# mit-han-lab/pvcnn

Hardware: AMD Instinct MI355X
Metric: point-clouds/sec fwd+bwd, PVCNN S3DIS N=4096 R=32 (higher is better)
Workload: dtype f32 (fp32 tensors, fp32 accumulate; Conv3d fwd / bwd-data / bwd-weight and the large SharedMLP fwd / bwd-data / bwd-weight products as power-of-two scaled fp16 hi+lo splits, 3 partial products on fp16 MFMA, max rel err vs fp64 1e-6 <= the fp32-MFMA kernels'; PVCNN_CONV_MATH=fp32 PVCNN_PW_MATH=fp32 s; 1 GPU; PVCNN (1xC) S3DIS fwd+bwd+Adam, B=16/GPU N=4096 R=32/16 fp32; global_batch=16, points=4096, parallelism=dp1, gradient_bytes=10289972, step_mode=graph, rccl_ranks=0, gradient_buckets=2

## Files before the change

include/pvcnn_hip.h:

```cpp
#ifndef PVCNN_HIP_H_
#define PVCNN_HIP_H_

#include <stddef.h>
#include <stdint.h>

#ifdef __cplusplus
extern "C" {
#endif

#if defined(__GNUC__)
#define PVCNN_API __attribute__((visibility("default")))
#else
#define PVCNN_API
#endif

#define PVCNN_ABI_VERSION 17
#define PVCNN_OK 0
#define PVCNN_ERR_INVALID_ARGUMENT (-1)

PVCNN_API int pvcnn_version(void);
PVCNN_API const char *pvcnn_last_error_string(void);

PVCNN_API int pvcnn_voxel_coords(const float *coords, int B, int N, int R, int normalize, float eps, float *norm_coords,
                       int32_t *vox_coords, void *stream);

PVCNN_API int pvcnn_voxel_coords_tail(const float *coords, long coords_batch_stride, const float *mean, const float *radius,
                            int B, int N, int R, float eps, float *norm_coords, int32_t *vox_coords, void *stream);

PVCNN_API size_t pvcnn_avg_voxelize_fwd_workspace_bytes(int B, int C, int N, int R);
PVCNN_API int pvcnn_avg_voxelize_fwd(const float *feat, const int32_t *coords, int B, int C, int N, int R,
                           float *out, int32_t *ind, int32_t *cnt, void *workspace,
                           size_t workspace_bytes, void *stream);
PVCNN_API int pvcnn_avg_voxelize_bwd(const float *grad_y, const int32_t *ind, const int32_t *cnt, int B,
                           int C, int N, int S, float *grad_x, void *stream);

PVCNN_API int pvcnn_trilinear_devox_fwd(const float *coords, const float *feat, int B, int C, int N, int R,
                              int is_training, int32_t *inds, float *wgts, float *outs,
                              void *stream);
PVCNN_API size_t pvcnn_trilinear_devox_bwd_workspace_bytes(int B, int C, int N, int R);
PVCNN_API int pvcnn_trilinear_devox_bwd(const float *grad_y, const int32_t *inds, const float *wgts, int B,
                              int C, int N, int R, float *grad_x, void *workspace,
                              size_t workspace_bytes, void *stream);

PVCNN_API size_t pvcnn_avg_voxelize_plan_bytes(int B, int N, int R);
PVCNN_API size_t pvcnn_avg_voxelize_plan_scratch_bytes(int B, int N, int R);
PVCNN_API int pvcnn_avg_voxelize_plan(const int32_t *coords, int B, int N, int R, int32_t *ind, int32_t *cnt, void *plan,
                            size_t plan_bytes, void *scratch, size_t scratch_bytes, void *stream);
PVCNN_API size_t pvcnn_pvconv_plans_scratch_bytes(int B, int N, int R);
PVCNN_API int pvcnn_pvconv_plans(const int32_t *vox_coords, const float *norm_coords, int B, int N, int R, int32_t *ind, int32_t *cnt,
                                 void *vox_plan, size_t vox_plan_bytes, void *devox_bwd_plan, size_t devox_bwd_plan_bytes,
                                 void *scratch, size_t scratch_bytes, void *stream);
PVCNN_API int pvcnn_avg_voxelize_apply(const float *feat, const void *plan, size_t plan_bytes, int B, int C, int N, int R,
                             float *out, void *stream);
PVCNN_API size_t pvcnn_trilinear_devox_bwd_plan_bytes(int B, int N, int R);
PVCNN_API size_t pvcnn_trilinear_devox_bwd_plan_scratch_bytes(int B, int N, int R);
PVCNN_API int pvcnn_trilinear_devox_bwd_plan(const int32_t *inds, const float *wgts, int B, int N, int R, void *plan,
                                   size_t plan_bytes, void *scratch, size_t scratch_bytes, void *stream);
PVCNN_API int pvcnn_trilinear_devox_bwd_apply(const float *grad_y, long grad_y_batch_stride, const void *plan, size_t plan_bytes,
                                    int B, int C, int N, int R, float *grad_x, void *stream);

PVCNN_API int pvcnn_ball_query(const float *centers, const float *points, int B, int N, int M, float radius,
                     int U, int32_t *out, void *stream);

PVCNN_API int pvcnn_grouping_fwd(const float *features, const int32_t *indices, int B, int C, int N, int M,
                       int U, float *out, void *stream);
PVCNN_API size_t pvcnn_grouping_bwd_workspace_bytes(int B, int C, int N, int M, int U);
PVCNN_API int pvcnn_grouping_bwd(const float *grad_y, const int32_t *indices, int B, int C, int N, int M,
                       int U, float *grad_x, void *workspace, size_t workspace_bytes, void *stream);
PVCNN_API int pvcnn_gather_fwd(const float *features, const int32_t *indices, int B, int C, int N, int M,
                     float *out, void *stream);
PVCNN_API size_t pvcnn_gather_bwd_workspace_bytes(int B, int C, int N, int M);
PVCNN_API int pvcnn_gather_bwd(const float *grad_y, const int32_t *indices, int B, int C, int N, int M,
                     float *grad_x, void *workspace, size_t workspace_bytes, void *stream);

#define PVCNN_FPS_MAX_RESIDENT_POINTS 16384
PVCNN_API int pvcnn_fps(const float *coords, int B, int N, int M, float *distances, int32_t *indices,
              void *stream);

PVCNN_API int pvcnn_mask_select(const uint8_t *mask, int B, int N, int M, const int32_t *choices, const int64_t *seed,
                      int32_t *selected, int32_t *count, void *stream);

PVCNN_API size_t pvcnn_batch_lds_bytes(int N, int max_n);
PVCNN_API int pvcnn_batch_s3dis(const float *rows, const void *labels, int label_bytes, const int64_t *offsets, long long W, int max_n,
                      const int64_t *order, long long order_len, const int64_t *cursor, int B, int N, int C_out,
                      const int32_t *choices, const int64_t *seed, float *features, int64_t *targets, void *stream);
PVCNN_API int pvcnn_batch_shapenet(const float *rows, const void *labels, int label_bytes, const int64_t *offsets, long long W,
                         const int32_t *shape_ids, const int64_t *order, long long order_len, const int64_t *cursor, int B, int N,
                         int with_normal, int num_shapes, int jitter_on, const int32_t *choices, const double *jitter,
                         const int64_t *seed, float *features, int64_t *targets, void *stream);
PVCNN_API int pvcnn_batch_frustum(const float *rows, const void *labels, int label_bytes, const int64_t *offsets, long long W,
                        const double *item_f64, const float *item_f32, const int64_t *item_i64, int K, int random_flip,
                        int random_shift, const int64_t *order, long long order_len, const int64_t *cursor, int B, int N,
                        const int32_t *choices, const double *flip, const double *shift, const int64_t *seed, float *features,
                        float *one_hot_vectors, int64_t *mask_logits, float *center, int64_t *heading_bin_id,
                        float *heading_residual, int64_t *size_template_id, float *size_residual, int64_t *class_id, void *stream);
PVCNN_API int pvcnn_batch_frustum_rgb(const float *rows, const int64_t *offsets, long long W, const double *item_f64,
                            const float *item_f32, int K, const int64_t *order, long long order_len, const int64_t *cursor, int B,
                            int N, const int32_t *choices, const int64_t *seed, float *features, float *one_hot_vectors,
                            float *rotation_angle, double *rgb_score, void *stream);

PVCNN_API int pvcnn_three_nn_interp_fwd(const float *points_coords, const float *centers_coords,
                              const float *centers_features, int B, int C, int M, int N,
                              int32_t *indices, float *weights, float *out, void *stream);
PVCNN_API size_t pvcnn_three_nn_interp_bwd_workspace_bytes(int B, int C, int N, int M);
PVCNN_API int pvcnn_three_nn_interp_bwd(const float *grad_y, const int32_t *indices, const float *weights,
                              int B, int C, int N, int M, float *grad_x, void *workspace,
                              size_t workspace_bytes, void *stream);

PVCNN_API int pvcnn_conv3d_weight_transform(const float *w, int Co, int Ci, int for_bwd_data, float *wt,
                                            void *stream);
PVCNN_API int pvcnn_conv3d_fwd(const float *x, const float *wt, const float *bias, int B, int Ci, int Co,
                               int R, float *y, void *stream);
PVCNN_API size_t pvcnn_conv3d_bwd_weight_workspace_bytes(int B, int Ci, int Co, int R);
PVCNN_API int pvcnn_conv3d_bwd_weight(const float *x, const float *grad_y, int B, int Ci, int Co, int R,
                                      float *grad_w, float *grad_bias, void *workspace, size_t workspace_bytes,
                                      void *stream);

PVCNN_API size_t pvcnn_conv3d_weight_split_bytes(int Co, int Ci, int for_bwd_data, int nsplit);
PVCNN_API int pvcnn_conv3d_weight_split(const float *w, int Co, int Ci, int for_bwd_data, int nsplit, void *wts, void *stream);
PVCNN_API int pvcnn_conv3d_weight_split_pair(const float *w, int Co, int Ci, void *wts_fwd, void *wts_bwd, void *stream);
PVCNN_API size_t pvcnn_conv3d_fwd_split_stats_parts(int B, int Co, int R, int nsplit);
PVCNN_API int pvcnn_conv3d_fwd_split_route(int B, int Ci, int Co, int R, int nsplit);
PVCNN_API int pvcnn_absmax_bits(const float *x, size_t n, void *out, void *stream);
PVCNN_API size_t pvcnn_absmax_tiles_count(int B, long L, int seg);
#define PVCNN_TABLE_ONLY ((void *)1)
PVCNN_API int pvcnn_absmax_tiles(const float *x, int B, int C, long L, int seg, void *out, void *ticket, void *stream);
PVCNN_API int pvcnn_conv3d_fwd_split(const float *x, const void *wts, const float *bias, int B, int Ci, int Co, int R, int nsplit,
                           const void *x_absmax, int amax_seg , float *y, float *stats_part, void *stream);
PVCNN_API int pvcnn_conv3d_fwd_split_act(const float *x, const void *wts, const float *bias, int B, int Ci, int Co, int R, int nsplit,
                           const void *x_absmax, int amax_seg , float *y, float *stats_part, float slope, void *y_amax,
                           int y_amax_seg , void *stream);
PVCNN_API int pvcnn_conv3d_fwd_act(const float *x, const float *wt, const float *bias, int B, int Ci, int Co, int R, float *y,
                           float slope, void *y_amax, int y_amax_seg , void *stream);

PVCNN_API size_t pvcnn_conv3d_bwd_weight_f16_workspace_bytes(int B, int Ci, int Co, int R);
PVCNN_API int pvcnn_conv3d_bwd_weight_f16(const float *x, const float *grad_y, const void *x_absmax, int x_amax_seg, const void *gy_absmax,
                                int gy_amax_seg, int B, int Ci, int Co, int R, float *grad_w, float *grad_bias, void *workspace,
                                size_t workspace_bytes, void *stream);

PVCNN_API int pvcnn_pwconv_transpose(const float *w, int M, int K, float *wt, void *stream);
PVCNN_API int pvcnn_pwconv_fwd(const float *x, const float *wt, int wt_rows, const float *bias, int B, int K, int M,
                     int N, float *y, void *stream);
PVCNN_API size_t pvcnn_pwconv_bwd_weight_workspace_bytes(int B, int K, int M, int N);
PVCNN_API int pvcnn_pwconv_bwd_weight(const float *x, const float *grad_y, int B, int K, int M, int N,
                            float *grad_w, float *grad_bias, void *workspace, size_t workspace_bytes,
                            void *stream);

PVCNN_API size_t pvcnn_pwconv_weight_split_bytes(int Co, int Ci, int for_bwd_data, int nsplit);
PVCNN_API int pvcnn_pwconv_weight_split(const float *w, int Co, int Ci, int for_bwd_data, int nsplit, void *wts, void *stream);
PVCNN_API int pvcnn_pwconv_weight_split_pair(const float *w, int Co, int Ci, void *wts_fwd, void *wts_bwd, void *stream);
PVCNN_API size_t pvcnn_pwconv_fwd_split_stats_parts(int B, int N);
PVCNN_API int pvcnn_pwconv_fwd_split_route(int B, int K, int M, int N, int nsplit);
PVCNN_API int pvcnn_pwconv_fwd_split(const float *x, const void *wts, const float *bias, int B, int K, int M, int N, int nsplit,
                           const void *x_absmax, int amax_seg , float *y, float *stats_part, void *stream);
PVCNN_API int pvcnn_pwconv_fwd_split_act(const float *x, const void *wts, const float *bias, int B, int K, int M, int N, int nsplit,
                           const void *x_absmax, int amax_seg , float *y, float *stats_part, float slope, void *y_amax,
                           int y_amax_seg , void *stream);
PVCNN_API int pvcnn_pwconv_fwd_act(const float *x, const float *wt, int wt_rows, const float *bias, int B, int K, int M, int N,
                           float *y, float slope, void *y_amax, int y_amax_seg , void *stream);
PVCNN_API size_t pvcnn_pwconv_bwd_weight_f16_workspace_bytes(int B, int K, int M, int N);
PVCNN_API int pvcnn_pwconv_bwd_weight_f16(const float *x, const float *grad_y, const void *x_absmax, int x_amax_seg, const void *gy_absmax,
                                int gy_amax_seg, int B, int K, int M, int N, float *grad_w, float *grad_bias, void *workspace,
                                size_t workspace_bytes, void *stream);

PVCNN_API int pvcnn_dropout_keep_mask(const void *drop_seed, float drop_p, long numel, unsigned char *keep, void *stream);
PVCNN_API size_t pvcnn_bnact_workspace_bytes(int B, int C, int S);
PVCNN_API int pvcnn_bnact_fwd(const float *x, const float *gamma, const float *beta, float *running_mean,
                              float *running_var, int B, int C, int S, float eps, float momentum, float slope,
                              int training, float *mean, float *rstd, float *y, void *y_amax, int amax_seg, int amax_zeroed,
                              void *workspace, size_t workspace_bytes, const void *drop_seed, float drop_p, void *stream);
PVCNN_API size_t pvcnn_conv3d_fwd_stats_parts(int B, int Co, int R);
PVCNN_API int pvcnn_conv3d_fwd_stats(const float *x, const float *wt, const float *bias, int B, int Ci, int Co, int R,
                           float *y, float *stats_part, void *stream);
PVCNN_API size_t pvcnn_pwconv_fwd_stats_parts(int B, int N);
PVCNN_API int pvcnn_pwconv_fwd_stats(const float *x, const float *wt, int wt_rows, const float *bias, int B, int K, int M,
                           int N, float *y, float *stats_part, void *stream);
PVCNN_API int pvcnn_bn_finalize(const float *part, int C, long nparts, double count, float eps, float momentum, const float *shift,
                      float *running_mean, float *running_var, float *mean, float *rstd,
                      void *zero_words , long zero_count ,
                      void *num_batches_tracked , void *stream);
PVCNN_API int pvcnn_bn_stats(const float *x, float *running_mean, float *running_var, int B, int C, int S,
                   float eps, float momentum, float *mean, float *rstd, void *workspace,
                   size_t workspace_bytes, void *stream);
PVCNN_API int pvcnn_trilinear_devox_bnact_fwd(const float *coords, const float *feat, const float *gamma,
                                    const float *beta, const float *mean, const float *rstd, float slope,
                                    int B, int C, int N, int R, int is_training, int32_t *inds, float *wgts,
                                    const float *addend, const float *se_scale, float *outs, void *stream);
PVCNN_API int pvcnn_trilinear_devox_bnact_addbn_fwd(const float *coords, const float *feat, const float *gamma,
                                    const float *beta, const float *mean, const float *rstd, float slope,
                                    int B, int C, int N, int R, int is_training, int32_t *inds, float *wgts,
                                    const float *addend, const float *add_gamma, const float *add_beta,
                                    const float *add_mean, const float *add_rstd, float add_slope, float *outs, void *stream);
PVCNN_API int pvcnn_bnact_bwd(const float *x, const float *grad_y, const float *gamma, const float *beta,
                              const float *mean, const float *rstd, int B, int C, int S, float slope, int training,
                              float *grad_x, float *grad_gamma, float *grad_beta, void *workspace,
                              size_t workspace_bytes, void *stream);
PVCNN_API int pvcnn_bnact_bwd_strided(const float *x, const float *grad_y, long grad_y_batch_stride, const float *gamma,
                            const float *beta, const float *mean, const float *rstd, int B, int C, int S,
                            float slope, int training, float *grad_x, float *grad_gamma, float *grad_beta,
                            void *gx_amax, int amax_seg, void *workspace, size_t workspace_bytes, const void *drop_seed,
                            float drop_p, void *tickets, void *stream);
PVCNN_API int pvcnn_bnact_slices(int S);
PVCNN_API long pvcnn_conv3d_weight_split_pair_entry(const float *w, int Co, int Ci, void *wts_fwd, void *wts_bwd, long long *entry);
PVCNN_API int pvcnn_conv3d_weight_split_pair_batch(const void *table, int n, long total_rows, void *stream);
PVCNN_API long pvcnn_pwconv_weight_split_pair_entry(const float *w, int Co, int Ci, void *wts_fwd, void *wts_bwd, long long *entry);
PVCNN_API int pvcnn_pwconv_weight_split_pair_batch(const void *table, int n, long total_rows, void *stream);
PVCNN_API long pvcnn_conv3d_weight_split_pair_entry_bf16(const float *w, int Co, int Ci, void *wts_fwd, void *wts_bwd, long long *entry);
PVCNN_API int pvcnn_conv3d_weight_split_pair_batch_bf16(const void *table, int n, long total_rows, void *stream);
PVCNN_API long pvcnn_pwconv_weight_split_pair_entry_bf16(const float *w, int Co, int Ci, void *wts_fwd, void *wts_bwd, long long *entry);
PVCNN_API int pvcnn_pwconv_weight_split_pair_batch_bf16(const void *table, int n, long total_rows, void *stream);

PVCNN_API int pvcnn_neighbor_max_supported(int K);
PVCNN_API int pvcnn_neighbor_max_fwd(const float *x, long rows, int K, float *out, unsigned char *winners, void *stream);
PVCNN_API int pvcnn_neighbor_max_bwd(const float *grad_out, const unsigned char *winners, long rows, int K, float *grad_x, void *stream);

PVCNN_API int pvcnn_row_argmax(const float *x, long rows, int K, long long *winners, float *values, void *stream);

PVCNN_API int pvcnn_bnact_apply_rowmax(const float *x, const float *gamma, const float *beta, const float *mean, const float *rstd, int B,
                                       int C, int S, float slope, float *y, long y_batch_stride, void *y_amax, int amax_seg,
                                       void *row_keys, void *stream);
PVCNN_API int pvcnn_row_keys_decode(const void *row_keys, const float *y, long rows, int S, long long *winners, float *values,
                                    int C, long y_batch_stride, void *stream);

PVCNN_API size_t pvcnn_frustum_box_loss_grad_floats(int B, int NH, int NS);
PVCNN_API int pvcnn_frustum_box_loss(const float *center, const float *center_reg, const float *heading_scores, const float *size_scores,
                                     const float *heading_residuals_normalized, const float *size_residuals_normalized,
                                     const float *heading_residuals, const float *size_residuals, const long long *heading_bin_id,
                                     const long long *size_template_id, const float *heading_residual_t, const float *size_residual_t,
                                     const float *center_t, const float *size_templates, const float *heading_bin_centers, int B, int NH,
                                     int NS, float heading_bin_width, float w_heading_residual, float w_size_residual, float w_corners,
                                     float *loss, float *grads, void *stream);

PVCNN_API int pvcnn_se_excite_fwd(const float *part, int slices, const float *gamma, const float *beta, const float *w1, const float *w2,
                        int B, int C, int H, float inv_s, float *a_sum, float *ax_sum, float *squeezed, float *hidden, float *excite,
                        void *stream);
PVCNN_API int pvcnn_se_excite_bwd(const float *part, int slices, const float *a_sum, const float *ax_sum, const float *gamma,
                        const float *beta, const float *squeezed, const float *hidden, const float *excite, const float *w1,
                        const float *w2, int B, int C, int H, float inv_s, float *g_w1, float *g_w2, float *g_mean, float *sum_beta,
                        float *sum_gamma, float *workspace, void *stream);
PVCNN_API int pvcnn_bnact_partial_sums(const float *x, const float *grad_y, long grad_y_batch_stride, const float *gamma, const float *beta,
                             const float *mean, const float *rstd, int B, int C, int S, float slope, float *part, void *stream);
PVCNN_API int pvcnn_bnact_bwd_apply(const float *x, const float *grad_y, long grad_y_batch_stride, const float *gamma, const float *beta,
                          const float *mean, const float *rstd, const float *sum_gamma, const float *sum_beta, const float *bc_mul,
                          const float *bc_add, int B, int C, int S, float slope, int training, float *grad_x, void *gx_amax,
                          int amax_seg, void *stream);
PVCNN_API int pvcnn_trilinear_devox_bwd_strided(const float *grad_y, long grad_y_batch_stride, const int32_t *inds,
                                      const float *wgts, int B, int C, int N, int R, float *grad_x,
                                      void *workspace, size_t workspace_bytes, void *stream);

PVCNN_API int pvcnn_concat_points(const float *const *srcs, const long *bstrides, const int *channels, const int *pstrides,
                        const void *const *src_amax ,
                        int nsrc, int B, int N, float *out, void *out_amax,
                        void *ticket , void *stream);

PVCNN_API int pvcnn_dense_bn_relu_supported(int rows, int Cin, int Cout);
PVCNN_API int pvcnn_dense_bn_relu_fwd(const float *x, const float *weight, const float *bias, const float *gamma, const float *beta,
                                      float *running_mean, float *running_var, void *num_batches_tracked, int rows, int Cin, int Cout,
                                      float eps, float momentum, float *z, float *y, float *mean, float *rstd, void *stream);
PVCNN_API int pvcnn_dense_bn_relu_bwd(const float *x, const float *grad_y, const float *z, const float *mean, const float *rstd,
                                      const float *gamma, const float *beta, int rows, int Cin, int Cout, float *grad_z,
                                      float *grad_weight, float *grad_bias, float *grad_gamma, float *grad_beta, void *stream);

PVCNN_API int pvcnn_adam_step(float *p, const float *g, float *m, float *v, size_t n, float *step, const float *hyper, int inc_step,
                    void *stream);
PVCNN_API int pvcnn_grad_sqsum(const float *g, size_t n, float *partials, int nparts, void *stream);
PVCNN_API int pvcnn_grad_norm_finalize(const float *partials, int nparts, float *status, void *stream);
PVCNN_API int pvcnn_adam_step_grouped(float *p, const float *g, float *m, float *v, float *vmax, size_t n, float *step,
                                      const float *hyper, int ngroups, const int *runs, int nruns, const float *status,
                                      int decoupled, int inc_step, void *stream);

PVCNN_API int pvcnn_eval_tile(const float *src, long long batch_stride, long long point_stride, long long chan_stride, long long src_points,
                              const long long *shuffled, int B, int V, int num_points, int C, float *out, void *stream);
PVCNN_API int pvcnn_vote_confidence(const float *logits, int B, int C, int N, int c0, int c1, const int *ranges, float *conf, int *pred,
                                    void *stream);
PVCNN_API size_t pvcnn_vote_merge_workspace_bytes(long long P);
PVCNN_API int pvcnn_vote_merge(const float *conf, const int *pred, const long long *shuffled, const long long *mapping, long long map_stride,
                               int B, int V, long long P, float *scene_conf, long long *scene_pred, void *workspace, size_t workspace_bytes,
                               void *stream);
PVCNN_API int pvcnn_seg_counts(const long long *gt, const long long *pred, long long P, int C, int wrap_negative, long long *counts,
                               void *stream);
PVCNN_API int pvcnn_seg_meter_update(const float *logits, const long long *targets, int B, int C, int N, const int *part_ranges,
                                     int num_part_classes, int max_parts, long long *counts, int *rows, const long long *row_cursor,
                                     long long row_capacity, void *stream);

// ... 102 lines not shown
```

pvcnn_amd/_lib.py:

```python
import ctypes
import functools
import os

import torch

_CSRC = os.path.join(os.path.dirname(os.path.abspath(__file__)), 'csrc')
LIB_PATH = os.path.join(_CSRC, 'libpvcnn_hip.so')
ABI_VERSION = 17

_vp, _i, _f, _sz, _l = ctypes.c_void_p, ctypes.c_int, ctypes.c_float, ctypes.c_size_t, ctypes.c_long
_ll = ctypes.c_longlong
_d = ctypes.c_double

SIGNATURES = {
    'pvcnn_version': (_i, []),
    'pvcnn_last_error_string': (ctypes.c_char_p, []),
    'pvcnn_voxel_coords': (_i, [_vp, _i, _i, _i, _i, _f, _vp, _vp, _vp]),
    'pvcnn_voxel_coords_tail': (_i, [_vp, ctypes.c_long, _vp, _vp, _i, _i, _i, _f, _vp, _vp, _vp]),
    'pvcnn_avg_voxelize_fwd_workspace_bytes': (_sz, [_i, _i, _i, _i]),
    'pvcnn_avg_voxelize_fwd': (_i, [_vp, _vp, _i, _i, _i, _i, _vp, _vp, _vp, _vp, _sz, _vp]),
    'pvcnn_avg_voxelize_bwd': (_i, [_vp, _vp, _vp, _i, _i, _i, _i, _vp, _vp]),
    'pvcnn_trilinear_devox_fwd': (_i, [_vp, _vp, _i, _i, _i, _i, _i, _vp, _vp, _vp, _vp]),
    'pvcnn_trilinear_devox_bwd_workspace_bytes': (_sz, [_i, _i, _i, _i]),
    'pvcnn_trilinear_devox_bwd': (_i, [_vp, _vp, _vp, _i, _i, _i, _i, _vp, _vp, _sz, _vp]),
    'pvcnn_avg_voxelize_plan_bytes': (_sz, [_i, _i, _i]),
    'pvcnn_avg_voxelize_plan_scratch_bytes': (_sz, [_i, _i, _i]),
    'pvcnn_avg_voxelize_plan': (_i, [_vp, _i, _i, _i, _vp, _vp, _vp, _sz, _vp, _sz, _vp]),
    'pvcnn_avg_voxelize_apply': (_i, [_vp, _vp, _sz, _i, _i, _i, _i, _vp, _vp]),
    'pvcnn_pvconv_plans_scratch_bytes': (_sz, [_i, _i, _i]),
    'pvcnn_pvconv_plans': (_i, [_vp, _vp, _i, _i, _i, _vp, _vp, _vp, _sz, _vp, _sz, _vp, _sz, _vp]),
    'pvcnn_trilinear_devox_bwd_plan_bytes': (_sz, [_i, _i, _i]),
    'pvcnn_trilinear_devox_bwd_plan_scratch_bytes': (_sz, [_i, _i, _i]),
    'pvcnn_trilinear_devox_bwd_plan': (_i, [_vp, _vp, _i, _i, _i, _vp, _sz, _vp, _sz, _vp]),
    'pvcnn_trilinear_devox_bwd_apply': (_i, [_vp, ctypes.c_long, _vp, _sz, _i, _i, _i, _i, _vp, _vp]),
    'pvcnn_ball_query': (_i, [_vp, _vp, _i, _i, _i, _f, _i, _vp, _vp]),
    'pvcnn_grouping_fwd': (_i, [_vp, _vp, _i, _i, _i, _i, _i, _vp, _vp]),
    'pvcnn_grouping_bwd_workspace_bytes': (_sz, [_i, _i, _i, _i, _i]),
    'pvcnn_grouping_bwd': (_i, [_vp, _vp, _i, _i, _i, _i, _i, _vp, _vp, _sz, _vp]),
    'pvcnn_gather_fwd': (_i, [_vp, _vp, _i, _i, _i, _i, _vp, _vp]),
    'pvcnn_gather_bwd_workspace_bytes': (_sz, [_i, _i, _i, _i]),
    'pvcnn_gather_bwd': (_i, [_vp, _vp, _i, _i, _i, _i, _vp, _vp, _sz, _vp]),
    'pvcnn_fps': (_i, [_vp, _i, _i, _i, _vp, _vp, _vp]),
    'pvcnn_mask_select': (_i, [_vp, _i, _i, _i, _vp, _vp, _vp, _vp, _vp]),
    'pvcnn_three_nn_interp_fwd': (_i, [_vp, _vp, _vp, _i, _i, _i, _i, _vp, _vp, _vp, _vp]),
    'pvcnn_three_nn_interp_bwd_workspace_bytes': (_sz, [_i, _i, _i, _i]),
    'pvcnn_three_nn_interp_bwd': (_i, [_vp, _vp, _vp, _i, _i, _i, _i, _vp, _vp, _sz, _vp]),
    'pvcnn_conv3d_weight_transform': (_i, [_vp, _i, _i, _i, _vp, _vp]),
    'pvcnn_conv3d_fwd': (_i, [_vp, _vp, _vp, _i, _i, _i, _i, _vp, _vp]),
    'pvcnn_conv3d_bwd_weight_workspace_bytes': (_sz, [_i, _i, _i, _i]),
    'pvcnn_conv3d_bwd_weight': (_i, [_vp, _vp, _i, _i, _i, _i, _vp, _vp, _vp, _sz, _vp]),
    'pvcnn_conv3d_weight_split_bytes': (_sz, [_i, _i, _i, _i]),
    'pvcnn_conv3d_weight_split': (_i, [_vp, _i, _i, _i, _i, _vp, _vp]),
    'pvcnn_conv3d_weight_split_pair': (_i, [_vp, _i, _i, _vp, _vp, _vp]),
    'pvcnn_conv3d_fwd_split_stats_parts': (_sz, [_i, _i, _i, _i]),
    'pvcnn_conv3d_fwd_split_route': (_i, [_i, _i, _i, _i, _i]),
    'pvcnn_absmax_bits': (_i, [_vp, _sz, _vp, _vp]),
    'pvcnn_absmax_tiles_count': (_sz, [_i, ctypes.c_long, _i]),
    'pvcnn_absmax_tiles': (_i, [_vp, _i, _i, ctypes.c_long, _i, _vp, _vp, _vp]),
    'pvcnn_conv3d_bwd_weight_f16_workspace_bytes': (_sz, [_i, _i, _i, _i]),
    'pvcnn_conv3d_bwd_weight_f16': (_i, [_vp, _vp, _vp, _i, _vp, _i, _i, _i, _i, _i, _vp, _vp, _vp, _sz, _vp]),
    'pvcnn_conv3d_fwd_split': (_i, [_vp, _vp, _vp, _i, _i, _i, _i, _i, _vp, _i, _vp, _vp, _vp]),
    'pvcnn_pwconv_transpose': (_i, [_vp, _i, _i, _vp, _vp]),
    'pvcnn_pwconv_fwd': (_i, [_vp, _vp, _i, _vp, _i, _i, _i, _i, _vp, _vp]),
    'pvcnn_pwconv_weight_split_bytes': (_sz, [_i, _i, _i, _i]),
    'pvcnn_pwconv_weight_split': (_i, [_vp, _i, _i, _i, _i, _vp, _vp]),
    'pvcnn_pwconv_weight_split_pair': (_i, [_vp, _i, _i, _vp, _vp, _vp]),
    'pvcnn_pwconv_fwd_split_stats_parts': (_sz, [_i, _i]),
    'pvcnn_pwconv_fwd_split_route': (_i, [_i, _i, _i, _i, _i]),
    'pvcnn_pwconv_fwd_split': (_i, [_vp, _vp, _vp, _i, _i, _i, _i, _i, _vp, _i, _vp, _vp, _vp]),
    'pvcnn_pwconv_bwd_weight_f16_workspace_bytes': (_sz, [_i, _i, _i, _i]),
    'pvcnn_pwconv_bwd_weight_f16': (_i, [_vp, _vp, _vp, _i, _vp, _i, _i, _i, _i, _i, _vp, _vp, _vp, _sz, _vp]),
    'pvcnn_pwconv_bwd_weight_workspace_bytes': (_sz, [_i, _i, _i, _i]),
    'pvcnn_pwconv_bwd_weight': (_i, [_vp, _vp, _i, _i, _i, _i, _vp, _vp, _vp, _sz, _vp]),
    'pvcnn_bnact_workspace_bytes': (_sz, [_i, _i, _i]),
    'pvcnn_bnact_fwd': (_i, [_vp, _vp, _vp, _vp, _vp, _i, _i, _i, _f, _f, _f, _i, _vp, _vp, _vp, _vp, _i, _i, _vp, _sz, _vp, _f, _vp]),
    'pvcnn_dropout_keep_mask': (_i, [_vp, _f, _l, _vp, _vp]),
    'pvcnn_conv3d_fwd_stats_parts': (_sz, [_i, _i, _i]),
    'pvcnn_conv3d_fwd_stats': (_i, [_vp, _vp, _vp, _i, _i, _i, _i, _vp, _vp, _vp]),
    'pvcnn_pwconv_fwd_stats_parts': (_sz, [_i, _i]),
    'pvcnn_pwconv_fwd_stats': (_i, [_vp, _vp, _i, _vp, _i, _i, _i, _i, _vp, _vp, _vp]),
    'pvcnn_bn_finalize': (_i, [_vp, _i, ctypes.c_long, ctypes.c_double, _f, _f, _vp, _vp, _vp, _vp, _vp, _vp, ctypes.c_long, _vp, _vp]),
    'pvcnn_bn_stats': (_i, [_vp, _vp, _vp, _i, _i, _i, _f, _f, _vp, _vp, _vp, _sz, _vp]),
    'pvcnn_trilinear_devox_bnact_fwd': (_i, [_vp, _vp, _vp, _vp, _vp, _vp, _f, _i, _i, _i, _i, _i, _vp, _vp, _vp, _vp, _vp, _vp]),
    'pvcnn_trilinear_devox_bnact_addbn_fwd': (_i, [_vp, _vp, _vp, _vp, _vp, _vp, _f, _i, _i, _i, _i, _i, _vp, _vp, _vp, _vp, _vp, _vp, _vp, _f, _vp, _vp]),
    'pvcnn_bnact_slices': (_i, [_i]),
    'pvcnn_conv3d_weight_split_pair_entry': (_l, [_vp, _i, _i, _vp, _vp, _vp]),
    'pvcnn_conv3d_weight_split_pair_batch': (_i, [_vp, _i, _l, _vp]),
    'pvcnn_pwconv_weight_split_pair_entry': (_l, [_vp, _i, _i, _vp, _vp, _vp]),
    'pvcnn_pwconv_weight_split_pair_batch': (_i, [_vp, _i, _l, _vp]),
    'pvcnn_conv3d_weight_split_pair_entry_bf16': (_l, [_vp, _i, _i, _vp, _vp, _vp]),
    'pvcnn_conv3d_weight_split_pair_batch_bf16': (_i, [_vp, _i, _l, _vp]),
    'pvcnn_pwconv_weight_split_pair_entry_bf16': (_l, [_vp, _i, _i, _vp, _vp, _vp]),
    'pvcnn_pwconv_weight_split_pair_batch_bf16': (_i, [_vp, _i, _l, _vp]),
    'pvcnn_neighbor_max_supported': (_i, [_i]),
    'pvcnn_neighbor_max_fwd': (_i, [_vp, _l, _i, _vp, _vp, _vp]),
    'pvcnn_neighbor_max_bwd': (_i, [_vp, _vp, _l, _i, _vp, _vp]),
    'pvcnn_row_argmax': (_i, [_vp, _l, _i, _vp, _vp, _vp]),
    'pvcnn_bnact_apply_rowmax': (_i, [_vp, _vp, _vp, _vp, _vp, _i, _i, _i, _f, _vp, _l, _vp, _i, _vp, _vp]),
    'pvcnn_row_keys_decode': (_i, [_vp, _vp, _l, _i, _vp, _vp, _i, _l, _vp]),
    'pvcnn_frustum_box_loss_grad_floats': (_sz, [_i, _i, _i]),
    'pvcnn_frustum_box_loss': (_i, [_vp] * 15 + [_i, _i, _i, _f, _f, _f, _f, _vp, _vp, _vp]),
    'pvcnn_se_excite_fwd': (_i, [_vp, _i, _vp, _vp, _vp, _vp, _i, _i, _i, _f, _vp, _vp, _vp, _vp, _vp, _vp]),
    'pvcnn_se_excite_bwd': (_i, [_vp, _i] + [_vp] * 9 + [_i, _i, _i, _f] + [_vp] * 7),
    'pvcnn_bnact_partial_sums': (_i, [_vp, _vp, ctypes.c_long, _vp, _vp, _vp, _vp, _i, _i, _i, _f, _vp, _vp]),
    'pvcnn_bnact_bwd_apply': (_i, [_vp, _vp, ctypes.c_long, _vp, _vp, _vp, _vp, _vp, _vp, _vp, _vp, _i, _i, _i, _f, _i, _vp, _vp, _i, _vp]),
    'pvcnn_bnact_bwd': (_i, [_vp, _vp, _vp, _vp, _vp, _vp, _i, _i, _i, _f, _i, _vp, _vp, _vp, _vp, _sz, _vp]),
    'pvcnn_bnact_bwd_strided': (_i, [_vp, _vp, ctypes.c_long, _vp, _vp, _vp, _vp, _i, _i, _i, _f, _i, _vp, _vp, _vp, _vp, _i, _vp, _sz, _vp, _f, _vp, _vp]),
    'pvcnn_concat_points': (_i, [_vp, _vp, _vp, _vp, _vp, _i, _i, _i, _vp, _vp, _vp, _vp]),
    'pvcnn_dense_bn_relu_supported': (_i, [_i, _i, _i]),
    'pvcnn_dense_bn_relu_fwd': (_i, [_vp] * 8 + [_i, _i, _i, _f, _f, _vp, _vp, _vp, _vp, _vp]),
    'pvcnn_dense_bn_relu_bwd': (_i, [_vp] * 7 + [_i, _i, _i] + [_vp] * 6),
    'pvcnn_adam_step': (_i, [_vp, _vp, _vp, _vp, _sz, _vp, _vp, _i, _vp]),
    'pvcnn_grad_sqsum': (_i, [_vp, _sz, _vp, _i, _vp]),
    'pvcnn_grad_norm_finalize': (_i, [_vp, _i, _vp, _vp]),
    'pvcnn_adam_step_grouped': (_i, [_vp, _vp, _vp, _vp, _vp, _sz, _vp, _vp, _i, _vp, _i, _vp, _i, _i, _vp]),
    'pvcnn_trilinear_devox_bwd_strided': (_i, [_vp, ctypes.c_long, _vp, _vp, _i, _i, _i, _i, _vp, _vp, _sz, _vp]),
    'pvcnn_eval_tile': (_i, [_vp, _ll, _ll, _ll, _ll, _vp, _i, _i, _i, _i, _vp, _vp]),
    'pvcnn_vote_confidence': (_i, [_vp, _i, _i, _i, _i, _i, _vp, _vp, _vp, _vp]),
    'pvcnn_vote_merge_workspace_bytes': (_sz, [_ll]),
    'pvcnn_vote_merge': (_i, [_vp, _vp, _vp, _vp, _ll, _i, _i, _ll, _vp, _vp, _vp, _sz, _vp]),
    'pvcnn_seg_counts': (_i, [_vp, _vp, _ll, _i, _i, _vp, _vp]),
    'pvcnn_seg_meter_update': (_i, [_vp, _vp, _i, _i, _i, _vp, _i, _i, _vp, _vp, _vp, _ll, _vp]),
    'pvcnn_frustum_meter_update': (_i, [_vp] * 11 + [_i, _i, _i, _vp, _vp, _vp, _vp, _i, _vp, _vp, _i, _i, _vp, _vp, _vp]),
    'pvcnn_box_iou_3d': (_i, [_vp, _vp, _i, _vp, _vp, _vp]),
    'pvcnn_rotate_iou': (_i, [_vp, _ll, _vp, _ll, _i, _vp, _vp]),
    'pvcnn_box3d_overlap': (_i, [_vp, _vp, _ll, _vp, _vp, _ll, _i, _i, ctypes.c_double, _vp, _vp]),
    'pvcnn_batch_lds_bytes': (_sz, [_i, _i]),
    'pvcnn_batch_s3dis': (_i, [_vp, _vp, _i, _vp, _ll, _i, _vp, _ll, _vp, _i, _i, _i, _vp, _vp, _vp, _vp, _vp]),
    'pvcnn_batch_shapenet': (_i, [_vp, _vp, _i, _vp, _ll, _vp, _vp, _ll, _vp, _i, _i, _i, _i, _i, _vp, _vp, _vp, _vp, _vp, _vp]),
    'pvcnn_batch_frustum': (_i, [_vp, _vp, _i, _vp, _ll, _vp, _vp, _vp, _i, _i, _i, _vp, _ll, _vp, _i, _i] + [_vp] * 14),
    'pvcnn_batch_frustum_rgb': (_i, [_vp, _vp, _ll, _vp, _vp, _i, _vp, _ll, _vp, _i, _i] + [_vp] * 7),
    'pvcnn_frustum_predictions': (_i, [_vp] * 5 + [_i, _i, _i] + [_vp] * 5 + [_ll, _ll, _vp]),
    'pvcnn_room_workspace_bytes': (_sz, [_ll, _ll]),
    'pvcnn_room_extent': (_i, [_vp, _ll, _vp, _vp, _sz, _vp]),
    'pvcnn_room_blocks': (_i, [_vp, _ll, _vp, _d, _d, _i, _i, _i, _vp, _vp, _vp, _vp, _vp, _vp, _sz, _vp]),
    'pvcnn_room_cells': (_i, [_vp, _ll, _vp, _d, _ll, _vp, _vp, _vp, _vp, _vp, _vp]),
    'pvcnn_room_plan': (_i, [_vp, _vp, _ll, _ll, _i] + [_vp] * 6 + [_vp, _sz, _vp]),
    'pvcnn_room_fill': (_i, [_vp] * 7 + [_ll, _ll, _ll] + [_vp] * 5),
    'pvcnn_room_pack': (_i, [_vp, _vp, _ll, _vp, _d, _vp, _vp, _ll, _ll, _i, _ll] + [_vp] * 9),
    'pvcnn_image_box_overlap': (_i, [_vp, _ll, _vp, _ll, _i, _vp, _vp]),
    'pvcnn_kitti_ap_bbox_overlaps': (_i, [_vp] * 5 + [_ll, _ll, _vp, _vp]),
    'pvcnn_kitti_ap_box_overlaps': (_i, [_vp] * 7 + [_ll, _ll, _i, _i, _d, _vp, _vp]),
    'pvcnn_kitti_ap_clean': (_i, [_vp, _vp, _vp, _vp, _ll, _vp, _vp, _ll, _vp, _vp, _ll, _vp, _i, _vp, _i] + [_vp] * 5),
    'pvcnn_kitti_ap_match': (_i, [_vp] * 5 + [_ll, _ll, _ll, _i, _i] + [_vp] * 9 + [_i, _i, _i] + [_vp, _vp]),
    'pvcnn_kitti_ap_thresholds': (_i, [_vp, _ll, _vp, _i, _i, _vp, _vp, _vp]),
    'pvcnn_kitti_ap_workspace_bytes': (_sz, [_ll, _i]),
    'pvcnn_conv3d_fwd_split_act': (_i, [_vp, _vp, _vp, _i, _i, _i, _i, _i, _vp, _i, _vp, _vp, _f, _vp, _i, _vp]),
    'pvcnn_conv3d_fwd_act': (_i, [_vp, _vp, _vp, _i, _i, _i, _i, _vp, _f, _vp, _i, _vp]),
    'pvcnn_pwconv_fwd_split_act': (_i, [_vp, _vp, _vp, _i, _i, _i, _i, _i, _vp, _i, _vp, _vp, _f, _vp, _i, _vp]),
    'pvcnn_pwconv_fwd_act': (_i, [_vp, _vp, _i, _vp, _i, _i, _i, _i, _vp, _f, _vp, _i, _vp]),
    'pvcnn_kitti_ap_stats': (_i, [_vp] * 5 + [_ll, _ll, _ll, _i, _i] + [_vp] * 9 + [_i, _i, _i] + [_vp, _vp, _i, _i, _vp, _vp, _sz, _vp]),
    'pvcnn_xent_parts': (_sz, [_ll, _ll]),
    'pvcnn_xent_workspace_bytes': (_sz, [_ll, _ll]),
    'pvcnn_xent_partials': (_i, [_vp, _ll, _vp, _ll, _vp, _ll, _i, _ll, _ll, _i, _vp, _vp]),
    'pvcnn_xent_finalize': (_i, [_vp, _ll, _i, _ll, _d, _i, _vp, _vp, _vp, _vp]),
    'pvcnn_xent_bwd': (_i, [_vp, _ll, _vp, _ll, _vp, _vp, _ll, _i, _ll, _ll, _f, _i, _vp, _vp, _vp]),
    'pvcnn_kl_workspace_bytes': (_sz, [_ll, _ll]),
    'pvcnn_kl_partials': (_i, [_vp, _ll, _vp, _ll, _ll, _i, _ll, _vp, _vp]),
    'pvcnn_kl_finalize': (_i, [_ll, _i, _ll, _vp, _vp, _vp]),
    'pvcnn_kl_bwd': (_i, [_vp, _ll, _vp, _ll, _vp, _ll, _i, _ll, _vp, _vp, _vp]),
    'pvcnn_dml_pair_workspace_bytes': (_sz, [_ll, _ll]),
    'pvcnn_dml_pair_partials': (_i, [_vp, _ll, _vp, _ll, _vp, _ll, _vp, _ll, _i, _ll, _ll, _vp, _vp]),
    'pvcnn_dml_pair_finalize': (_i, [_ll, _i, _ll, _vp, _vp, _vp, _vp]),
    'pvcnn_dml_pair_bwd': (_i, [_vp, _ll, _vp, _ll, _vp, _ll, _vp, _vp, _ll, _i, _ll, _ll, _i, _vp, _vp, _vp]),
}

_lib = None


class PvcnnHipError(RuntimeError):
    pass


def load():
    global _lib
    if _lib is not None:
        return _lib
    if not os.path.exists(LIB_PATH):
        raise PvcnnHipError(
            f'{LIB_PATH} not found: build it with `python -c "import __graft_entry__ as g; g.build()"` '
            f'or `make -C {_CSRC}`.  There is no CPU fallback for the PVConv hot path.')
    lib = ctypes.CDLL(LIB_PATH)
    for name, (res, args) in SIGNATURES.items():
        fn = getattr(lib, name)
        fn.restype, fn.argtypes = res, args
    got = lib.pvcnn_version()
    if got != ABI_VERSION:
        raise PvcnnHipError(f'libpvcnn_hip.so ABI version {got}, binding expects {ABI_VERSION}: rebuild')
    for name, (res, _args) in SIGNATURES.items():
        if res is _sz:
# ... 23 lines not shown
```

pvcnn_amd/csrc/bnact.hip:

```cpp
#include <algorithm>

#include "common.h"

namespace pvcnn {

constexpr int kBnThreads = 256;
constexpr int kBnSlice = 8192;

__device__ __forceinline__ float wave_sum(float v) {
#pragma unroll
  for (int d = 32; d >= 1; d >>= 1) v += __shfl_xor(v, d);
  return v;
}

__device__ __forceinline__ void block_sum2(float &a, float &b, float *sm) {
  a = wave_sum(a);
  b = wave_sum(b);
  const int wave = threadIdx.x >> 6, lane = threadIdx.x & 63;
  if (lane == 0) { sm[wave] = a; sm[8 + wave] = b; }
  __syncthreads();
  if (threadIdx.x == 0) {
    a = sm[0] + sm[1] + sm[2] + sm[3];
    b = sm[8] + sm[9] + sm[10] + sm[11];
  }
// ... 32 lines not shown
                                                        float *__restrict__ running_var, uint32_t *__restrict__ zero_word,
                                                        long zero_count, long long *__restrict__ counter) {
  const int c = blockIdx.x;
  if (zero_word != nullptr)
    for (long i = (long)c * 64 + threadIdx.x; i < zero_count; i += (long)gridDim.x * 64) zero_word[i] = 0u;
  if (counter != nullptr && c == 0 && threadIdx.x == 0) *counter += 1;
  double s = 0.0, q = 0.0;
  for (int i = threadIdx.x; i < nparts; i += 64) { const float2 p = part[(size_t)c * nparts + i]; s += p.x; q += p.y; }
#pragma unroll
  for (int d = 32; d >= 1; d >>= 1) { s += __shfl_xor(s, d); q += __shfl_xor(q, d); }
  if (threadIdx.x == 0) {
    const double ms = s / count;
    const double m = ms + (shift ? (double)shift[c] : 0.0);
    double var = q / count - ms * ms;
    var = var < 0.0 ? 0.0 : var;
    mean[c] = (float)m;
    rstd[c] = (float)(1.0 / sqrt(var + (double)eps));
    if (running_mean) {
      const double unbiased = count > 1.0 ? var * count / (count - 1.0) : var;
      running_mean[c] = (float)((1.0 - momentum) * running_mean[c] + momentum * m);
      running_var[c] = (float)((1.0 - momentum) * running_var[c] + momentum * unbiased);
    }
  }
}

__global__ __launch_bounds__(kBnThreads) void bnact_apply_kernel(const float *__restrict__ x, const float *__restrict__ mean,
                                                                const float *__restrict__ rstd,
                                                                const float *__restrict__ gamma,
                                                                const float *__restrict__ beta, float slope, int C, int S,
                                                                float *__restrict__ y) {
  const int sl = blockIdx.x, b = blockIdx.y, c = blockIdx.z;
  const float scale = (gamma ? gamma[c] : 1.0f) * rstd[c];
  const float shift = (beta ? beta[c] : 0.0f) - mean[c] * scale;
  const size_t off = ((size_t)b * C + c) * S;
  const int lo = sl * kBnSlice, hi = min(S, lo + kBnSlice);
  if ((S & 3) == 0 && aligned16(x + off) && aligned16(y + off)) {
    for (int i = lo + threadIdx.x * 4; i < hi; i += kBnThreads * 4) {
      float4 v = *reinterpret_cast<const float4 *>(x + off + i);
      v.x = fmaf(v.x, scale, shift); v.y = fmaf(v.y, scale, shift); v.z = fmaf(v.z, scale, shift); v.w = fmaf(v.w, scale, shift);
      v.x = v.x > 0.f ? v.x : v.x * slope; v.y = v.y > 0.f ? v.y : v.y * slope;
      v.z = v.z > 0.f ? v.z : v.z * slope; v.w = v.w > 0.f ? v.w : v.w * slope;
      using v4f = __attribute__((ext_vector_type(4))) float;
      v4f o = {v.x, v.y, v.z, v.w};
      __builtin_nontemporal_store(o, reinterpret_cast<v4f *>(y + off + i));
    }
  } else {
    for (int i = lo + threadIdx.x; i < hi; i += kBnThreads) {
      const float v = fmaf(x[off + i], scale, shift);
      y[off + i] = v > 0.f ? v : v * slope;
    }
  }
}

struct Drop { const unsigned long long *key; uint32_t thr; float scale; };

__device__ __forceinline__ uint32_t drop_mix(uint32_t pair, uint32_t k0, uint32_t k1) {
  uint32_t x = pair ^ k0;
  x ^= x >> 16; x *= 0x7feb352dU; x ^= x >> 15; x += k1; x *= 0x846ca68bU; x ^= x >> 16;
  return x;
}
__device__ __forceinline__ void drop_factors4(size_t e0, uint32_t k0, uint32_t k1, uint32_t thr, float scale, float (&f)[4]) {
  const uint32_t h0 = drop_mix((uint32_t)(e0 >> 1), k0, k1), h1 = drop_mix((uint32_t)(e0 >> 1) + 1u, k0, k1);
  f[0] = (h0 & 0xffffu) >= thr ? scale : 0.0f; f[1] = (h0 >> 16) >= thr ? scale : 0.0f;
  f[2] = (h1 & 0xffffu) >= thr ? scale : 0.0f; f[3] = (h1 >> 16) >= thr ? scale : 0.0f;
}
__device__ __forceinline__ float drop_factor1(size_t e, uint32_t k0, uint32_t k1, uint32_t thr, float scale) {
  const uint32_t h = drop_mix((uint32_t)(e >> 1), k0, k1);
  return ((e & 1) ? (h >> 16) : (h & 0xffffu)) >= thr ? scale : 0.0f;
}

__global__ __launch_bounds__(256) void dropout_keep_mask_kernel(Drop d, long numel, unsigned char *__restrict__ keep) {
  const long e = (long)blockIdx.x * 256 + threadIdx.x;
  const unsigned long long key = *d.key;
  if (e < numel) keep[e] = drop_factor1((size_t)e, (uint32_t)key, (uint32_t)(key >> 32), d.thr, 1.0f) != 0.0f;
}

struct BwdFold {
  unsigned *tickets;
  float *dgamma, *dbeta;
  uint32_t *zero_word;
  long zero_count;
};

template <bool DROP = false>
__global__ __launch_bounds__(kBnThreads) void bnact_bwd_reduce_kernel(const float *__restrict__ x, const float *__restrict__ gy,
                                                                     const float *__restrict__ mean,
                                                                     const float *__restrict__ rstd,
                                                                     const float *__restrict__ gamma,
                                                                     const float *__restrict__ beta, float slope, int C,
                                                                     int S, int slices, float2 *__restrict__ part,
                                                                     long gy_bstride, Drop drop = Drop{nullptr, 0u, 1.0f},
                                                                     BwdFold fold = BwdFold{nullptr, nullptr, nullptr, nullptr, 0L}) {
  __shared__ float sm[16];
  uint32_t k0 = 0u, k1 = 0u;
  if constexpr (DROP) { const unsigned long long key = *drop.key; k0 = (uint32_t)key; k1 = (uint32_t)(key >> 32); }
  int lin = blockIdx.x + (int)gridDim.x * (blockIdx.y + (int)gridDim.y * blockIdx.z);
  const int sl = lin % (int)gridDim.x; lin /= (int)gridDim.x;
  const int c = lin % (int)gridDim.z, b = lin / (int)gridDim.z;
  const float m = mean[c], r = rstd[c];
  const float scale = (gamma ? gamma[c] : 1.0f) * r;
  const float shift = (beta ? beta[c] : 0.0f) - m * scale;
  const size_t off = ((size_t)b * C + c) * S;
  const size_t goff = (size_t)b * gy_bstride + (size_t)c * S;
  const int lo = sl * kBnSlice, hi = min(S, lo + kBnSlice);
  float s = 0.f, q = 0.f;
  auto quad = [&](int i, const float4 xv, const float4 gv) {
    const float xs_[4] = {xv.x, xv.y, xv.z, xv.w};
    float gs_[4] = {gv.x, gv.y, gv.z, gv.w};
    if constexpr (DROP) {
      float f[4];
      drop_factors4(off + i, k0, k1, drop.thr, drop.scale, f);
#pragma unroll
      for (int u = 0; u < 4; ++u) gs_[u] *= f[u];
    }
#pragma unroll
    for (int u = 0; u < 4; ++u) {
      const float z = fmaf(xs_[u], scale, shift);
      const float g = gs_[u] * (z > 0.f ? 1.0f : slope);
      s += g;
      q += g * ((xs_[u] - m) * r);
    }
  };
  const float4 ones = make_float4(1.0f, 1.0f, 1.0f, 1.0f);
  if ((S & 3) == 0 && aligned16(x + off) && (!gy || aligned16(gy + goff))) {
    for (int i = lo + threadIdx.x * 4; i < hi; i += kBnThreads * 4)
      quad(i, *reinterpret_cast<const float4 *>(x + off + i), gy ? *reinterpret_cast<const float4 *>(gy + goff + i) : ones);
  } else if ((S & 3) == 0) {
    for (int i = lo + threadIdx.x * 4; i < hi; i += kBnThreads * 4)
      quad(i, ld4_unaligned(x + off + i), gy ? ld4_unaligned(gy + goff + i) : ones);
  } else {
    for (int i = lo + threadIdx.x; i < hi; i += kBnThreads) {
      const float xv = x[off + i];
      const float z = fmaf(xv, scale, shift);
      float gin = gy ? gy[goff + i] : 1.0f;
      if constexpr (DROP) gin *= drop_factor1(off + i, k0, k1, drop.thr, drop.scale);
      const float g = gin * (z > 0.f ? 1.0f : slope);
      s += g;
      q += g * ((xv - m) * r);
    }
  }
  block_sum2(s, q, sm);
  float2 *mine = part + ((size_t)c * gridDim.y + b) * slices + sl;
  if (fold.tickets == nullptr) {
    if (threadIdx.x == 0) *mine = make_float2(s, q);
    return;
  }
  if (fold.zero_word != nullptr) {
    const long wgs = (long)gridDim.x * gridDim.y * gridDim.z;
    const long me = blockIdx.x + (long)gridDim.x * (blockIdx.y + (long)gridDim.y * blockIdx.z);
    for (long i = me * kBnThreads + threadIdx.x; i < fold.zero_count; i += wgs * kBnThreads) fold.zero_word[i] = 0u;
  }
  if (threadIdx.x >= 64) return;
  if (threadIdx.x == 0)
    publish64(reinterpret_cast<unsigned long long *>(mine), ((unsigned long long)__float_as_uint(q) << 32) | __float_as_uint(s));
  if (!ticket_take_wave(fold.tickets + c, (unsigned)(gridDim.x * gridDim.y))) return;
  {
    const int nparts = (int)(gridDim.x * gridDim.y);
    double ds = 0.0, dq = 0.0;
    for (int i = threadIdx.x; i < nparts; i += 64) {
      const unsigned long long w = peek64(reinterpret_cast<const unsigned long long *>(part + (size_t)c * nparts + i));
      ds += __uint_as_float((uint32_t)w); dq += __uint_as_float((uint32_t)(w >> 32));
    }
#pragma unroll
    for (int d = 32; d >= 1; d >>= 1) { ds += __shfl_xor(ds, d); dq += __shfl_xor(dq, d); }
    if (threadIdx.x == 0) { fold.dbeta[c] = (float)ds; fold.dgamma[c] = (float)dq; }
  }
}

__global__ __launch_bounds__(64) void bnact_bwd_finalize_kernel(const float2 *__restrict__ part, int nparts,
                                                               float *__restrict__ dgamma, float *__restrict__ dbeta,
                                                               uint32_t *__restrict__ zero_word, long zero_count) {
  const int c = blockIdx.x;
  if (zero_word != nullptr)
    for (long i = (long)c * 64 + threadIdx.x; i < zero_count; i += (long)gridDim.x * 64) zero_word[i] = 0u;
  double s = 0.0, q = 0.0;
  for (int i = threadIdx.x; i < nparts; i += 64) { const float2 p = part[(size_t)c * nparts + i]; s += p.x; q += p.y; }
#pragma unroll
  for (int d = 32; d >= 1; d >>= 1) { s += __shfl_xor(s, d); q += __shfl_xor(q, d); }
  if (threadIdx.x == 0) { dbeta[c] = (float)s; dgamma[c] = (float)q; }
}

__global__ __launch_bounds__(kBnThreads) void bnact_bwd_apply_kernel(const float *__restrict__ x, const float *__restrict__ gy,
                                                                    const float *__restrict__ mean,
                                                                    const float *__restrict__ rstd,
                                                                    const float *__restrict__ gamma,
                                                                    const float *__restrict__ beta,
                                                                    const float *__restrict__ dgamma,
                                                                    const float *__restrict__ dbeta, float slope,
                                                                    float inv_count, int training, int C, int S,
                                                                    float *__restrict__ gx, long gy_bstride) {
  const int sl = blockIdx.x, b = blockIdx.y, c = blockIdx.z;
  const float m = mean[c], r = rstd[c];
  const float gmm = gamma ? gamma[c] : 1.0f;
  const float scale = gmm * r;
  const float shift = (beta ? beta[c] : 0.0f) - m * scale;
  const float db = training ? dbeta[c] * inv_count : 0.0f, dg = training ? dgamma[c] * inv_count : 0.0f;
  const size_t off = ((size_t)b * C + c) * S;
  const size_t goff = (size_t)b * gy_bstride + (size_t)c * S;
  const int lo = sl * kBnSlice, hi = min(S, lo + kBnSlice);
  if ((S & 3) == 0 && aligned16(x + off) && aligned16(gy + goff) && aligned16(gx + off)) {
    for (int i = lo + threadIdx.x * 4; i < hi; i += kBnThreads * 4) {
      const float4 xv = *reinterpret_cast<const float4 *>(x + off + i);
      const float4 gv = *reinterpret_cast<const float4 *>(gy + goff + i);
      const float xs_[4] = {xv.x, xv.y, xv.z, xv.w}, gs_[4] = {gv.x, gv.y, gv.z, gv.w};
      float o[4];
#pragma unroll
      for (int u = 0; u < 4; ++u) {
        const float z = fmaf(xs_[u], scale, shift);
        const float g = gs_[u] * (z > 0.f ? 1.0f : slope);
        o[u] = scale * (g - db - ((xs_[u] - m) * r) * dg);
      }
      using v4f = __attribute__((ext_vector_type(4))) float;
      v4f ov = {o[0], o[1], o[2], o[3]};
      __builtin_nontemporal_store(ov, reinterpret_cast<v4f *>(gx + off + i));
    }
  } else {
    for (int i = lo + threadIdx.x; i < hi; i += kBnThreads) {
      const float xv = x[off + i];
      const float z = fmaf(xv, scale, shift);
      const float g = gy[goff + i] * (z > 0.f ? 1.0f : slope);
      const float xhat = (xv - m) * r;
      gx[off + i] = scale * (g - db - xhat * dg);
    }
  }
}

__device__ __forceinline__ uint32_t max_order_bits(float v) {
  uint32_t u = __float_as_uint(v);
  if (u == 0x80000000u) u = 0u;
  return v != v ? 0xffffffffu : (u ^ ((uint32_t)((int32_t)u >> 31) | 0x80000000u));
}

__global__ __launch_bounds__(256) void row_keys_decode_kernel(const unsigned long long *__restrict__ keys, const float *__restrict__ y, long rows,
                                                              int S, long long *__restrict__ winners, float *__restrict__ values, int C,
                                                              long y_bstride) {
  const long row = (long)blockIdx.x * 256 + threadIdx.x;
  if (row >= rows) return;
  const uint32_t k = ~(uint32_t)keys[row];
  winners[row] = (long long)k;
  if (values) values[row] = y[(size_t)(row / C) * y_bstride + (size_t)(row % C) * S + k];
}

template <bool BWD, bool DROP = false, bool ROWMAX = false>
__global__ __launch_bounds__(256) void bnact_apply_pb_kernel(const float *__restrict__ x, const float *__restrict__ gy, long gy_bstride,
                                                             const float *__restrict__ mean, const float *__restrict__ rstd,
                                                             const float *__restrict__ gamma, const float *__restrict__ beta,
                                                             const float *__restrict__ dgamma, const float *__restrict__ dbeta,
                                                             float slope, float inv_count, int training, int C, int S, int seg,
                                                             int nseg, int vec, float *__restrict__ out, uint32_t *__restrict__ amax,
                                                             int global_by_atomic, const float *__restrict__ bc_mul = nullptr,
                                                             const float *__restrict__ bc_add = nullptr, int cgroup = 0x7fffffff,
                                                             int table_by_atomic = 0, Drop drop = Drop{nullptr, 0u, 1.0f},
                                                             unsigned long long *__restrict__ row_keys = nullptr, long out_bstride = 0) {
  static_assert(!ROWMAX || (!BWD && !DROP), "row maxima: plain forward pass only");
  __shared__ uint32_t seg_max[256];
  int lin = blockIdx.x + (int)gridDim.x * (blockIdx.y + (int)gridDim.y * blockIdx.z);
  const int bz = lin % (int)gridDim.z; lin /= (int)gridDim.z;
  const int bx = lin % (int)gridDim.x, by = lin / (int)gridDim.x;
  uint32_t k0 = 0u, k1 = 0u;
  if constexpr (DROP) { const unsigned long long key = *drop.key; k0 = (uint32_t)key; k1 = (uint32_t)(key >> 32); }
  const int spb = seg >= 256 ? 1 : 256 / seg;
  const int b = by, s0 = bx * spb;
  const int p0 = s0 * seg, span = min(spb * seg, S - p0);
  const int tid = threadIdx.x, wave = __builtin_amdgcn_readfirstlane(tid >> 6), lane = tid & 63, pos = 4 * lane;
  const int cbeg = bz * min(cgroup, C), cend = min(C, cbeg + min(cgroup, C));
  if (tid < spb) seg_max[tid] = 0u;
  __syncthreads();
  const float *xb = x + (size_t)b * C * S + p0;
  const float *gb = BWD ? gy + (size_t)b * gy_bstride + p0 : nullptr;
  float *ob = out + (size_t)b * (out_bstride > 0 ? (size_t)out_bstride : (size_t)C * S) + p0;
  uint32_t mx[4] = {0u, 0u, 0u, 0u};
  struct Par { float scale, shift, m, r, db, dg, gmul, gadd; };
  auto par_of = [&](int c) {
    Par p;
    p.m = mean[c]; p.r = rstd[c];
    p.gmul = (BWD && bc_mul) ? bc_mul[(size_t)b * C + c] : 1.0f;
    p.gadd = (BWD && bc_add) ? bc_add[(size_t)b * C + c] : 0.0f;
    p.scale = (gamma ? gamma[c] : 1.0f) * p.r;
    p.shift = (beta ? beta[c] : 0.0f) - p.m * p.scale;
    p.db = (BWD && training) ? dbeta[c] * inv_count : 0.0f;
    p.dg = (BWD && training) ? dgamma[c] * inv_count : 0.0f;
    return p;
  };
  auto one = [&](float xv, float gv, const Par &p, float kf) {
    if constexpr (BWD) {
      const float z = fmaf(xv, p.scale, p.shift);
      float gin = (bc_mul || bc_add) ? fmaf(gv, p.gmul, p.gadd) : gv;
      if constexpr (DROP) gin *= kf;
      const float g = gin * (z > 0.f ? 1.0f : slope);
      return p.scale * (g - p.db - ((xv - p.m) * p.r) * p.dg);
    } else {
      const float v = fmaf(xv, p.scale, p.shift);
      const float a = v > 0.f ? v : v * slope;
      if constexpr (DROP) return a * kf; else return a;
    }
  };
  const size_t ebase = (size_t)b * C * S + p0;
  if (pos < span) {
    if (vec) {
      using v4f = __attribute__((ext_vector_type(4))) float;
      constexpr int RF = 8;
      for (int c0 = cbeg + wave; c0 < cend; c0 += 4 * RF) {
        float4 xv[RF], gv[RF];
#pragma unroll
        for (int u = 0; u < RF; ++u) {
          const int c = c0 + 4 * u;
          xv[u] = gv[u] = make_float4(0.f, 0.f, 0.f, 0.f);
          if (c < cend) {
            xv[u] = *reinterpret_cast<const float4 *>(xb + (size_t)c * S + pos);
            if constexpr (BWD) gv[u] = *reinterpret_cast<const float4 *>(gb + (size_t)c * S + pos);
          }
        }
#pragma unroll
        for (int u = 0; u < RF; ++u) {
          const int c = c0 + 4 * u;
          if (c < cend) {
            const Par p = par_of(c);
            float kf[4] = {1.0f, 1.0f, 1.0f, 1.0f};
            if constexpr (DROP) drop_factors4(ebase + (size_t)c * S + pos, k0, k1, drop.thr, drop.scale, kf);
            const float o0 = one(xv[u].x, gv[u].x, p, kf[0]), o1 = one(xv[u].y, gv[u].y, p, kf[1]), o2 = one(xv[u].z, gv[u].z, p, kf[2]),
                        o3 = one(xv[u].w, gv[u].w, p, kf[3]);
            mx[0] = max(mx[0], __float_as_uint(fabsf(o0))); mx[1] = max(mx[1], __float_as_uint(fabsf(o1)));
            mx[2] = max(mx[2], __float_as_uint(fabsf(o2))); mx[3] = max(mx[3], __float_as_uint(fabsf(o3)));
            v4f ov = {o0, o1, o2, o3};
            __builtin_nontemporal_store(ov, reinterpret_cast<v4f *>(ob + (size_t)c * S + pos));
            if constexpr (ROWMAX) {
              const uint32_t e0 = max_order_bits(o0), e1 = max_order_bits(o1), e2 = max_order_bits(o2), e3 = max_order_bits(o3);
              uint32_t bv = e0;
              int bi = 0;
              if (e1 > bv) { bv = e1; bi = 1; }
              if (e2 > bv) { bv = e2; bi = 2; }
              if (e3 > bv) { bv = e3; bi = 3; }
              uint32_t wv = bv;
#pragma unroll
              for (int o = 32; o > 0; o >>= 1) wv = max(wv, (uint32_t)__shfl_xor((int)wv, o));
              const unsigned long long holders = __ballot(bv == wv);
              if (lane == __ffsll((long long)holders) - 1)
                atomicMax(&row_keys[(size_t)b * C + c], ((unsigned long long)wv << 32) | (unsigned long long)(~(uint32_t)(p0 + pos + bi)));
            }
          }
        }
      }
    } else {
      for (int c = cbeg + wave; c < cend; c += 4) {
        const Par p = par_of(c);
#pragma unroll
        for (int i = 0; i < 4; ++i)
          if (pos + i < span) {
            const float kf = DROP ? drop_factor1(ebase + (size_t)c * S + pos + i, k0, k1, drop.thr, drop.scale) : 1.0f;
            const float o = one(xb[(size_t)c * S + pos + i], BWD ? gb[(size_t)c * S + pos + i] : 0.0f, p, kf);
            ob[(size_t)c * S + pos + i] = o;
            mx[i] = max(mx[i], __float_as_uint(fabsf(o)));
          }
      }
    }
#pragma unroll
    for (int i = 0; i < 4; ++i)
      if (pos + i < span) atomicMax(&seg_max[(pos + i) / seg], mx[i]);
  }
  lds_barrier();
  if (tid < spb && s0 + tid < nseg) {
    if (table_by_atomic) { if (seg_max[tid] != 0u) atomicMax(&amax[1 + (size_t)b * nseg + s0 + tid], seg_max[tid]); }
    else amax[1 + (size_t)b * nseg + s0 + tid] = seg_max[tid];
  }
  if (global_by_atomic && tid == 0) {
    uint32_t m = 0;
    for (int i = 0; i < spb; ++i) m = max(m, seg_max[i]);
    if (m != 0) atomicMax(amax, m);
  }
}

}

using namespace pvcnn;

static const char kAmaxSegRange[] = "amax_seg must be in 1..256";
static bool amax_seg_in_range(int seg) { return seg > 0 && seg <= 256; }

static int pb_channel_groups(long position_blocks, int C) {
  int g = 1;
  while (position_blocks * g < 4 * kNumCU && C / (2 * g) >= 32) g *= 2;
  return g;
}

static bool make_drop(const void *drop_seed, float drop_p, Drop *d) {
  if (drop_seed == nullptr || !(drop_p > 0.0f)) return false;
  long t = lrintf(drop_p * 65536.0f);
  d->key = static_cast<const unsigned long long *>(drop_seed);
  d->thr = (uint32_t)(t < 0 ? 0 : t > 65536 ? 65536 : t);
  d->scale = 1.0f / (1.0f - drop_p);
  return true;
}

// ... 38 lines not shown
    amax_zeroed = 1;
  }
  if (y_amax != nullptr) {
    const int nseg = ceil_div(S, amax_seg), spb = amax_seg >= 256 ? 1 : 256 / amax_seg;
    const int vec = (S % 4 == 0) && (amax_seg % 4 == 0) && aligned16(x) && aligned16(y);
    uint32_t *am = static_cast<uint32_t *>(y_amax);
    const int groups = amax_zeroed ? pb_channel_groups((long)ceil_div(nseg, spb) * B, C) : 1;
    if (dropping)
      hipLaunchKernelGGL((bnact_apply_pb_kernel<false, true>), dim3(ceil_div(nseg, spb), B, groups), dim3(256), 0, s, x, nullptr, 0L, mean, rstd,
                         gamma, beta, nullptr, nullptr, slope, 0.0f, 0, C, S, amax_seg, nseg, vec, y, am, amax_zeroed ? 1 : 0, nullptr, nullptr,
                         ceil_div(C, groups), groups > 1 ? 1 : 0, drop);
    else
      hipLaunchKernelGGL(bnact_apply_pb_kernel<false>, dim3(ceil_div(nseg, spb), B, groups), dim3(256), 0, s, x, nullptr, 0L, mean, rstd, gamma,
                         beta, nullptr, nullptr, slope, 0.0f, 0, C, S, amax_seg, nseg, vec, y, am, amax_zeroed ? 1 : 0, nullptr, nullptr,
                         ceil_div(C, groups), groups > 1 ? 1 : 0);
    if (int e = check_launch("bnact_apply_pb")) return e;
    return amax_zeroed ? 0 : launch_amax_reduce(am, (long)B * nseg, s);
  }
  hipLaunchKernelGGL(bnact_apply_kernel, grid, dim3(kBnThreads), 0, s, x, mean, rstd, gamma, beta, slope, C, S, y);
  return check_launch("bnact_apply");
}

extern "C" int pvcnn_bnact_apply_rowmax(const float *x, const float *gamma, const float *beta, const float *mean, const float *rstd, int B,
                                        int C, int S, float slope, float *y, long y_batch_stride, void *y_amax, int amax_seg, void *row_keys,
                                        void *stream) {
  PVCNN_REQUIRE(B > 0 && C > 0 && S > 0 && x && y && mean && rstd && y_amax && row_keys, "bad argument");
  PVCNN_REQUIRE(y_batch_stride == 0 || (y_batch_stride >= (long)C * S && y_batch_stride % 4 == 0), "y_batch_stride: 0, or >= C * S and a multiple of 4");
  PVCNN_REQUIRE(B <= 65535 && C <= 65535, "batch or channel count > 65535");
  PVCNN_REQUIRE(amax_seg_in_range(amax_seg), kAmaxSegRange);
  PVCNN_REQUIRE(amax_seg % 4 == 0 && 256 % amax_seg == 0 && S % 256 == 0,
                "the row-maximum pass additionally needs S % 256 == 0 and amax_seg a multiple of 4 that divides 256");
  PVCNN_REQUIRE(aligned16(x) && aligned16(y) && ((uintptr_t)row_keys & 7) == 0, "x / y must be 16-byte aligned, row_keys 8-byte aligned");
  hipStream_t s = static_cast<hipStream_t>(stream);
  const int nseg = ceil_div(S, amax_seg), spb = amax_seg >= 256 ? 1 : 256 / amax_seg;
  const int groups = pb_channel_groups((long)ceil_div(nseg, spb) * B, C);
  hipLaunchKernelGGL((bnact_apply_pb_kernel<false, false, true>), dim3(ceil_div(nseg, spb), B, groups), dim3(256), 0, s, x, nullptr, 0L, mean, rstd,
                     gamma, beta, nullptr, nullptr, slope, 0.0f, 0, C, S, amax_seg, nseg, 1, y, static_cast<uint32_t *>(y_amax), 1, nullptr, nullptr,
                     ceil_div(C, groups), groups > 1 ? 1 : 0, Drop{nullptr, 0u, 1.0f}, static_cast<unsigned long long *>(row_keys), y_batch_stride);
  return check_launch("bnact_apply_rowmax");
}

extern "C" int pvcnn_row_keys_decode(const void *row_keys, const float *y, long rows, int S, long long *winners, float *values, int C,
                                     long y_batch_stride, void *stream) {
  PVCNN_REQUIRE(rows >= 0 && S > 0, "negative size");
  if (rows == 0) return 0;
  PVCNN_REQUIRE(row_keys && y && winners, "null pointer");
  if (C <= 0 || y_batch_stride <= 0) { C = 1; y_batch_stride = S; }
  hipLaunchKernelGGL(row_keys_decode_kernel, dim3((unsigned)((rows + 255) / 256)), dim3(256), 0, static_cast<hipStream_t>(stream),
                     static_cast<const unsigned long long *>(row_keys), y, rows, S, winners, values, C, y_batch_stride);
  return check_launch("row_keys_decode");
}

extern "C" int pvcnn_bn_finalize(const float *part, int C, long nparts, double count, float eps, float momentum, const float *shift,
                                 float *running_mean, float *running_var, float *mean, float *rstd, void *zero_words, long zero_count,
                                 void *num_batches_tracked, void *stream) {
  PVCNN_REQUIRE(C > 0 && nparts > 0 && nparts <= 0x7fffffffL && count > 0 && part && mean && rstd, "bad argument");
  hipLaunchKernelGGL(bn_finalize_kernel, dim3(C), dim3(64), 0, static_cast<hipStream_t>(stream),
                     reinterpret_cast<const float2 *>(part), (int)nparts, count, eps, momentum, shift, mean, rstd, running_mean,
                     running_var, static_cast<uint32_t *>(zero_words), zero_words ? zero_count : 0L,
                     static_cast<long long *>(num_batches_tracked));
  return check_launch("bn_finalize");
}

extern "C" int pvcnn_bn_stats(const float *x, float *running_mean, float *running_var, int B, int C, int S, float eps,
                              float momentum, float *mean, float *rstd, void *workspace, size_t workspace_bytes, void *stream) {
  PVCNN_REQUIRE(B > 0 && C > 0 && S > 0 && x && mean && rstd, "bad argument");
  PVCNN_REQUIRE(B <= 65535 && C <= 65535, "batch or channel count > 65535");
  PVCNN_REQUIRE(workspace && workspace_bytes >= pvcnn_bnact_workspace_bytes(B, C, S), "workspace too small");
  hipStream_t s = static_cast<hipStream_t>(stream);
  const int slices = ceil_div(S, kBnSlice);
  float2 *part = static_cast<float2 *>(workspace);
  float *shift = reinterpret_cast<float *>(part + (size_t)C * B * slices);
  hipLaunchKernelGGL(bn_stats_kernel, dim3(slices, B, C), dim3(kBnThreads), 0, s, x, C, S, slices, part, shift);
  if (int e = check_launch("bn_stats")) return e;
  hipLaunchKernelGGL(bn_finalize_kernel, dim3(C), dim3(64), 0, s, part, B * slices, (double)B * S, eps, momentum, shift, mean, rstd,
                     running_mean, running_var, static_cast<uint32_t *>(nullptr), 0L, static_cast<long long *>(nullptr));
  return check_launch("bn_finalize");
}

static int bnact_bwd_impl(const float *x, const float *grad_y, long gy_bstride, const float *gamma, const float *beta,
                          const float *mean, const float *rstd, int B, int C, int S, float slope, int training, float *grad_x,
                          float *grad_gamma, float *grad_beta, void *workspace, size_t workspace_bytes, void *stream,
                          void *gx_amax = nullptr, int amax_seg = 0, const void *drop_seed = nullptr, float drop_p = 0.0f,
                          void *tickets = nullptr) {
  PVCNN_REQUIRE(drop_p >= 0.0f && drop_p < 1.0f, "drop_p must be in [0, 1)");
  Drop drop{nullptr, 0u, 1.0f};
  const bool dropping = make_drop(drop_seed, drop_p, &drop);
  PVCNN_REQUIRE(!dropping || (gx_amax && (size_t)B * C * S < ((size_t)1 << 33)), "fused dropout needs the amax-emitting pass (gx_amax) and < 2^33 elements");
  PVCNN_REQUIRE(B > 0 && C > 0 && S > 0 && x && grad_y && mean && rstd && grad_x && grad_gamma && grad_beta, "bad argument");
  PVCNN_REQUIRE(B <= 65535 && C <= 65535, "batch or channel count > 65535");
  PVCNN_REQUIRE(gy_bstride >= (long)C * S, "grad_y batch stride smaller than one sample");
  PVCNN_REQUIRE(workspace && workspace_bytes >= pvcnn_bnact_workspace_bytes(B, C, S), "workspace too small");
  PVCNN_REQUIRE(!gx_amax || amax_seg_in_range(amax_seg), kAmaxSegRange);
  hipStream_t s = static_cast<hipStream_t>(stream);
  const int slices = ceil_div(S, kBnSlice);
  const dim3 grid(slices, B, C);
  float2 *part = static_cast<float2 *>(workspace);
  const long zero_count = gx_amax ? 1 + (long)B * ceil_div(S, amax_seg) : 0L;
  PVCNN_REQUIRE(!tickets || (reinterpret_cast<uintptr_t>(tickets) & 3) == 0, "tickets must be 4-byte aligned");
  const BwdFold fold{static_cast<unsigned *>(tickets), grad_gamma, grad_beta, static_cast<uint32_t *>(gx_amax), zero_count};
  if (dropping)
    hipLaunchKernelGGL(bnact_bwd_reduce_kernel<true>, grid, dim3(kBnThreads), 0, s, x, grad_y, mean, rstd, gamma, beta, slope, C, S, slices, part,
                       gy_bstride, drop, fold);
  else
    hipLaunchKernelGGL(bnact_bwd_reduce_kernel<false>, grid, dim3(kBnThreads), 0, s, x, grad_y, mean, rstd, gamma, beta, slope, C, S, slices, part,
                       gy_bstride, Drop{nullptr, 0u, 1.0f}, fold);
  if (int e = check_launch("bnact_bwd_reduce")) return e;
  if (tickets == nullptr) {
    hipLaunchKernelGGL(bnact_bwd_finalize_kernel, dim3(C), dim3(64), 0, s, part, B * slices, grad_gamma, grad_beta,
                       static_cast<uint32_t *>(gx_amax), zero_count);
    if (int e = check_launch("bnact_bwd_finalize")) return e;
  }
  const float inv_count = (float)(1.0 / ((double)B * S));
  if (gx_amax != nullptr) {
    const int nseg = ceil_div(S, amax_seg), spb = amax_seg >= 256 ? 1 : 256 / amax_seg;
    const int vec = (S % 4 == 0) && (amax_seg % 4 == 0) && (gy_bstride % 4 == 0) && aligned16(x) && aligned16(grad_y) && aligned16(grad_x);
    uint32_t *am = static_cast<uint32_t *>(gx_amax);
    const int groups = pb_channel_groups((long)ceil_div(nseg, spb) * B, C);
    if (dropping)
      hipLaunchKernelGGL((bnact_apply_pb_kernel<true, true>), dim3(ceil_div(nseg, spb), B, groups), dim3(256), 0, s, x, grad_y, gy_bstride, mean,
                         rstd, gamma, beta, grad_gamma, grad_beta, slope, inv_count, training, C, S, amax_seg, nseg, vec, grad_x, am, 1, nullptr,
                         nullptr, ceil_div(C, groups), groups > 1 ? 1 : 0, drop);
    else
      hipLaunchKernelGGL(bnact_apply_pb_kernel<true>, dim3(ceil_div(nseg, spb), B, groups), dim3(256), 0, s, x, grad_y, gy_bstride, mean, rstd,
                         gamma, beta, grad_gamma, grad_beta, slope, inv_count, training, C, S, amax_seg, nseg, vec, grad_x, am, 1, nullptr,
                         nullptr, ceil_div(C, groups), groups > 1 ? 1 : 0);
    return check_launch("bnact_bwd_apply_pb");
  }
  hipLaunchKernelGGL(bnact_bwd_apply_kernel, grid, dim3(kBnThreads), 0, s, x, grad_y, mean, rstd, gamma, beta, grad_gamma,
                     grad_beta, slope, inv_count, training, C, S, grad_x, gy_bstride);
  return check_launch("bnact_bwd_apply");
}

extern "C" int pvcnn_bnact_bwd(const float *x, const float *grad_y, const float *gamma, const float *beta, const float *mean,
                               const float *rstd, int B, int C, int S, float slope, int training, float *grad_x,
                               float *grad_gamma, float *grad_beta, void *workspace, size_t workspace_bytes, void *stream) {
  return bnact_bwd_impl(x, grad_y, (long)C * S, gamma, beta, mean, rstd, B, C, S, slope, training, grad_x, grad_gamma, grad_beta,
                        workspace, workspace_bytes, stream);
}

extern "C" int pvcnn_bnact_bwd_strided(const float *x, const float *grad_y, long grad_y_batch_stride, const float *gamma,
                                       const float *beta, const float *mean, const float *rstd, int B, int C, int S, float slope,
                                       int training, float *grad_x, float *grad_gamma, float *grad_beta, void *gx_amax, int amax_seg,
                                       void *workspace, size_t workspace_bytes, const void *drop_seed, float drop_p, void *tickets,
                                       void *stream) {
  return bnact_bwd_impl(x, grad_y, grad_y_batch_stride, gamma, beta, mean, rstd, B, C, S, slope, training, grad_x, grad_gamma,
                        grad_beta, workspace, workspace_bytes, stream, gx_amax, amax_seg, drop_seed, drop_p, tickets);
}

extern "C" int pvcnn_bnact_slices(int S) { return S > 0 ? ceil_div(S, kBnSlice) : 0; }

extern "C" int pvcnn_bnact_partial_sums(const float *x, const float *grad_y, long grad_y_batch_stride, const float *gamma, const float *beta,
                                        const float *mean, const float *rstd, int B, int C, int S, float slope, float *part, void *stream) {
  PVCNN_REQUIRE(B > 0 && C > 0 && S > 0 && x && mean && rstd && part, "bad argument");
  PVCNN_REQUIRE(B <= 65535 && C <= 65535, "batch or channel count > 65535");
  PVCNN_REQUIRE(!grad_y || grad_y_batch_stride >= (long)C * S, "grad_y batch stride smaller than one sample");
  PVCNN_REQUIRE((reinterpret_cast<uintptr_t>(part) & 7) == 0, "part must be 8-byte aligned");
  const int slices = ceil_div(S, kBnSlice);
  hipLaunchKernelGGL(bnact_bwd_reduce_kernel<false>, dim3(slices, B, C), dim3(kBnThreads), 0, static_cast<hipStream_t>(stream), x, grad_y, mean,
                     rstd, gamma, beta, slope, C, S, slices, reinterpret_cast<float2 *>(part), grad_y ? grad_y_batch_stride : (long)C * S);
  return check_launch("bnact_partial_sums");
}

extern "C" int pvcnn_bnact_bwd_apply(const float *x, const float *grad_y, long grad_y_batch_stride, const float *gamma, const float *beta,
                                     const float *mean, const float *rstd, const float *sum_gamma, const float *sum_beta, const float *bc_mul,
                                     const float *bc_add, int B, int C, int S, float slope, int training, float *grad_x, void *gx_amax,
                                     int amax_seg, void *stream) {
  PVCNN_REQUIRE(B > 0 && C > 0 && S > 0 && x && grad_y && mean && rstd && grad_x, "bad argument");
  PVCNN_REQUIRE(!training || (sum_gamma && sum_beta), "training mode needs the two per-channel sums");
  PVCNN_REQUIRE(B <= 65535 && C <= 65535, "batch or channel count > 65535");
  PVCNN_REQUIRE(grad_y_batch_stride >= (long)C * S, "grad_y batch stride smaller than one sample");
  PVCNN_REQUIRE(!gx_amax || amax_seg_in_range(amax_seg), kAmaxSegRange);
  hipStream_t s = static_cast<hipStream_t>(stream);
  PVCNN_REQUIRE(gx_amax, "pvcnn_bnact_bwd_apply needs an amax buffer (pvcnn_absmax_tiles_count words)");
  const int nseg = ceil_div(S, amax_seg), spb = amax_seg >= 256 ? 1 : 256 / amax_seg;
  const int vec = (S % 4 == 0) && (amax_seg % 4 == 0) && (grad_y_batch_stride % 4 == 0) && aligned16(x) && aligned16(grad_y) && aligned16(grad_x);
  uint32_t *am = static_cast<uint32_t *>(gx_amax);
  hipLaunchKernelGGL(bnact_apply_pb_kernel<true>, dim3(ceil_div(nseg, spb), B), dim3(256), 0, s, x, grad_y, grad_y_batch_stride, mean, rstd, gamma,
                     beta, sum_gamma, sum_beta, slope, (float)(1.0 / ((double)B * S)), training, C, S, amax_seg, nseg, vec, grad_x, am, 0, bc_mul,
                     bc_add);
  if (int e = check_launch("bnact_bwd_apply_pb")) return e;
  return launch_amax_reduce(am, (long)B * nseg, s);
}

namespace pvcnn {
constexpr int kCatMaxSrc = 8;
struct CatSources {
  const float *p[kCatMaxSrc];
  long bstride[kCatMaxSrc];
  int c0[kCatMaxSrc + 1];
  int pstride[kCatMaxSrc];
  const uint32_t *pre[kCatMaxSrc];
  int n;
};

__global__ __launch_bounds__(256) void concat_points_kernel(CatSources src, int N, int vec, float *__restrict__ out,
                                                            uint32_t *__restrict__ amax, unsigned *__restrict__ ticket) {
  __shared__ uint32_t wave_max[4];
  const int b = blockIdx.y, p0 = blockIdx.x * 256;
  const int tid = threadIdx.x, wave = __builtin_amdgcn_readfirstlane(tid >> 6), lane = tid & 63, pos = p0 + 4 * lane;
  const int Ctot = src.c0[src.n];
  const int cgroup = ceil_div(Ctot, (int)gridDim.z), gbeg = (int)blockIdx.z * cgroup, gend = min(Ctot, gbeg + cgroup);
  float *ob = out + (size_t)b * Ctot * N;
  uint32_t m = 0;
  using v4f = __attribute__((ext_vector_type(4))) float;
  for (int s = 0; s < src.n; ++s) {
    const int cb = src.c0[s], lo = max(gbeg, cb) - cb, cn = min(gend, src.c0[s + 1]) - cb;
    if (lo >= cn) continue;
    if (src.pre[s] != nullptr) {
      if (tid == 0 && amax != nullptr) m = max(m, src.pre[s][1 + (size_t)b * gridDim.x + blockIdx.x]);
      continue;
    }
    const float *sp = src.p[s] + (size_t)b * src.bstride[s];
    if (src.pstride[s] == 0) {
      for (int c = lo + wave; c < cn; c += 4) {
        const float v = sp[c];
        m = max(m, __float_as_uint(fabsf(v)));
        if (vec && pos < N) { v4f o = {v, v, v, v}; __builtin_nontemporal_store(o, reinterpret_cast<v4f *>(ob + (size_t)(cb + c) * N + pos)); }
        else for (int i = 0; i < 4; ++i) if (pos + i < N) ob[(size_t)(cb + c) * N + pos + i] = v;
      }
    } else if (vec) {
      if (pos < N)
        for (int c0 = lo + wave; c0 < cn; c0 += 32) {
          float4 v[8];
#pragma unroll
          for (int u = 0; u < 8; ++u)
            if (c0 + 4 * u < cn) v[u] = *reinterpret_cast<const float4 *>(sp + (size_t)(c0 + 4 * u) * N + pos);
#pragma unroll
          for (int u = 0; u < 8; ++u)
            if (c0 + 4 * u < cn) {
// ... 74 lines not shown
```

pvcnn_amd/csrc/common.h:

```cpp
#pragma once
#include <hip/hip_runtime.h>
#include <stdint.h>
#include <stddef.h>

#include "../../include/pvcnn_hip.h"
#include "switches.h"

namespace pvcnn {

constexpr int kWave = 64;
constexpr int kLdsBytesPerCU = 160 * 1024;
constexpr int kNumCU = 256;

void set_error(const char *fmt, ...);
int check_launch(const char *what);

__host__ __device__ inline int ceil_div(int a, int b) { return (a + b - 1) / b; }
inline int grid_pad_shift(int R) { int s = 0; while ((1 << s) < R) ++s; return ((1 << s) == R && R >= 4) ? s : 0; }
__host__ __device__ inline bool aligned16(const void *p) { return (reinterpret_cast<uintptr_t>(p) & 15) == 0; }

constexpr long kFoldTableMax = 1024;
int launch_amax_reduce(uint32_t *out, long T, hipStream_t s);

struct SplitEntry {
  const float *w;
  uint16_t *wts_f;
  int *wexp_f;
  uint16_t *wts_b;
  int *wexp_b;
  long long Co, Ci, rows_f, tm , row_begin;
};
static_assert(sizeof(SplitEntry) == 80, "ten 8-byte words");

#ifdef __HIPCC__
__device__ __forceinline__ SplitEntry split_entry_of(const SplitEntry *__restrict__ tab, int n, long long blk) {
  int i = 0;
  while (i + 1 < n && tab[i + 1].row_begin <= blk) ++i;
  return tab[i];
}

__device__ __forceinline__ void lds_barrier() { asm volatile("s_waitcnt lgkmcnt(0)\n\ts_barrier" ::: "memory"); }

__device__ __forceinline__ void publish32(uint32_t *p, uint32_t v) {
  const uint32_t old = atomicExch(p, v);
  asm volatile("" ::"v"(old) : "memory");
}
__device__ __forceinline__ void publish64(unsigned long long *p, unsigned long long v) {
  const unsigned long long old = atomicExch(p, v);
  asm volatile("" ::"v"(old) : "memory");
}
__device__ __forceinline__ uint32_t peek32(const uint32_t *p) {
  return __hip_atomic_load(p, __ATOMIC_RELAXED, __HIP_MEMORY_SCOPE_AGENT);
}
__device__ __forceinline__ unsigned long long peek64(const unsigned long long *p) {
  return __hip_atomic_load(p, __ATOMIC_RELAXED, __HIP_MEMORY_SCOPE_AGENT);
}
__device__ __forceinline__ bool ticket_take_wave(unsigned *ticket, unsigned total) {
  unsigned t = 0u;
  if ((threadIdx.x & 63) == 0) {
    t = atomicAdd(ticket, 1u);
    if (t == total - 1u) atomicExch(ticket, 0u);
  }
  return (unsigned)__builtin_amdgcn_readfirstlane((int)t) == total - 1u;
}
__device__ __forceinline__ bool ticket_take(unsigned *ticket, unsigned total) {
  __shared__ int s_last_workgroup;
  __syncthreads();
  if (threadIdx.x == 0) {
    const unsigned t = atomicAdd(ticket, 1u);
    s_last_workgroup = (t == total - 1u) ? 1 : 0;
    if (t == total - 1u) atomicExch(ticket, 0u);
  }
  __syncthreads();
  return s_last_workgroup != 0;
}

__device__ __forceinline__ void amax_table_max_wave(uint32_t *out, long T) {
  uint32_t m = 0;
  for (long i = threadIdx.x & 63; i < T; i += 64) m = max(m, peek32(out + 1 + i));
#pragma unroll
  for (int o = 32; o > 0; o >>= 1) m = max(m, (uint32_t)__shfl_xor((int)m, o));
  if ((threadIdx.x & 63) == 0) out[0] = m;
}
__device__ __forceinline__ void amax_table_max(uint32_t *out, long T) {
  __shared__ uint32_t s_amax_red[16];
  uint32_t m = 0;
  for (long i = threadIdx.x; i < T; i += blockDim.x) m = max(m, peek32(out + 1 + i));
#pragma unroll
  for (int o = 32; o > 0; o >>= 1) m = max(m, (uint32_t)__shfl_xor((int)m, o));
  if ((threadIdx.x & 63) == 0) s_amax_red[threadIdx.x >> 6] = m;
  __syncthreads();
  if (threadIdx.x == 0) {
    for (int w = 1; w < (int)((blockDim.x + 63) >> 6); ++w) m = max(m, s_amax_red[w]);
    out[0] = m;
  }
}

__device__ __forceinline__ uint32_t amax_table_value(const uint32_t *__restrict__ buf, long T) {
  if (T <= 0) return buf[0];
  __shared__ uint32_t s_amax_val[17];
  uint32_t m = 0;
  for (long i = threadIdx.x; i < T; i += blockDim.x) m = max(m, buf[1 + i]);
// ... 80 lines not shown
```

pvcnn_amd/csrc/csr.h:

```cpp
#pragma once
#include <algorithm>

#include "slab.h"

namespace pvcnn {

constexpr int kCsrThreads = 1024;
constexpr int kCsrMaxTargets = 1 << 20;
constexpr int kCsrMaxRange = 14336;

__host__ __device__ __forceinline__ int pad32(int v) { return v + (v >> 5); }
__host__ __device__ __forceinline__ int start_stride(int L) { return (L + 1 + 3) & ~3; }

constexpr int kTileTargets = 4096;
constexpr int kTileThreads = 1024;
__host__ __device__ inline int order_stride(int L) { return ceil_div(L, kTileTargets) * kTileTargets; }

constexpr int kGroupSlack = 256;
__host__ __device__ inline long entw_range_base(int start_t0, int r) { return 2L * start_t0 + (long)r * (kTileTargets / kWave) * kGroupSlack; }
__host__ __device__ inline long entw_stride(int L, long E) { return 2L * E + (long)ceil_div(L, kTileTargets) * (kTileTargets / kWave) * kGroupSlack; }

struct CsrPlan {
  int32_t *start;
  int2 *ent;
// ... 462 lines not shown
  int2 sg[kSlots];
#pragma unroll
  for (int k = 0; k < kSlots; ++k) {
    const int pos = k * kTileThreads + tid;
    sg[k] = l_seg[pos];
    out[pos] = l_lt[pos];
    sout[pos] = sg[k];
    int m = sg[k].y - sg[k].x, sum = m;
#pragma unroll
    for (int d = 32; d >= 1; d >>= 1) { m = max(m, __shfl_xor(m, d)); sum += __shfl_xor(sum, d); }
    if (lane == 0) gsz[pos >> 6] = (m > 0 && 64L * m <= 2L * sum + kGroupSlack) ? 64 * m : 0;
  }
  __syncthreads();
  if (tid < kGroups) {
    const int sz = gsz[tid];
    int inc = sz;
#pragma unroll
    for (int d = 1; d < kWave; d <<= 1) {
      const int up = __shfl_up(inc, d);
      if (lane >= d) inc += up;
    }
    const long base = entw_range_base(st[0], r) + (inc - sz);
    const int ofs = sz > 0 ? (int)base : -1;
    gsz[tid] = ofs;
    gofs[(size_t)b * (order_stride(L) / kWave) + (size_t)r * kGroups + tid] = ofs;
  }
}

static __global__ __launch_bounds__(kTileThreads) void csr_order_kernel(const int32_t *__restrict__ start, const int2 *__restrict__ ent,
                                                                        int L, int E, uint16_t *__restrict__ order,
                                                                        int2 *__restrict__ seg, int32_t *__restrict__ gofs,
                                                                        int2 *__restrict__ entw) {
  csr_order_body(start, ent, L, E, order, seg, gofs, entw, (int)blockIdx.x, (int)blockIdx.y);
}

struct CsrPlanRef {
  const int32_t *start;
  const int2 *ent;
  uint16_t *order;
  int2 *seg;
  int32_t *gofs;
  int2 *entw;
  int E;
};

[[maybe_unused]] static __global__ __launch_bounds__(kTileThreads) void csr_order_pair_kernel(CsrPlanRef a, CsrPlanRef c, int L, int nr) {
  const int r = (int)blockIdx.x;
  const bool f = r < nr;
  csr_order_body(f ? a.start : c.start, f ? a.ent : c.ent, L, f ? a.E : c.E, f ? a.order : c.order, f ? a.seg : c.seg,
                 f ? a.gofs : c.gofs, f ? a.entw : c.entw, f ? r : r - nr, (int)blockIdx.y);
}

static __device__ __forceinline__ void csr_interleave_body(const int2 *__restrict__ ent, const int2 *__restrict__ seg,
                                                           const int32_t *__restrict__ gofs, int L, int E, int2 *__restrict__ entw,
                                                           int blk, int b) {
  const int pos = blk * 256 + threadIdx.x, lane = threadIdx.x & 63;
  const int ofs = gofs[(size_t)b * (order_stride(L) / kWave) + (pos >> 6)];
  if (ofs < 0) return;
  const int2 sg = seg[(size_t)b * order_stride(L) + pos];
  const int2 *en = ent + (size_t)b * E + sg.x;
  int2 *ew = entw + (size_t)b * entw_stride(L, E) + ofs + lane;
  const int n = sg.y - sg.x;
  int i = 0;
  for (; i + 4 <= n; i += 4) {
    const int2 a = en[i], c = en[i + 1], d = en[i + 2], f = en[i + 3];
    ew[(size_t)i * 64] = a; ew[(size_t)(i + 1) * 64] = c; ew[(size_t)(i + 2) * 64] = d; ew[(size_t)(i + 3) * 64] = f;
  }
  for (; i < n; ++i) ew[(size_t)i * 64] = en[i];
}

static __global__ __launch_bounds__(256) void csr_interleave_kernel(const int2 *__restrict__ ent, const int2 *__restrict__ seg,
                                                                    const int32_t *__restrict__ gofs, int L, int E,
                                                                    int2 *__restrict__ entw) {
  csr_interleave_body(ent, seg, gofs, L, E, entw, (int)blockIdx.x, (int)blockIdx.y);
}

[[maybe_unused]] static __global__ __launch_bounds__(256) void csr_interleave_pair_kernel(CsrPlanRef a, CsrPlanRef c, int L, int nblk) {
  const int k = (int)blockIdx.x;
  const bool f = k < nblk;
  csr_interleave_body(f ? a.ent : c.ent, f ? a.seg : c.seg, f ? a.gofs : c.gofs, L, f ? a.E : c.E, f ? a.entw : c.entw, f ? k : k - nblk,
                      (int)blockIdx.y);
}

template <int G>
__global__ __launch_bounds__(kTileThreads) void segsum_tile_kernel(const float *__restrict__ src, const int2 *__restrict__ seg,
                                                                   const int2 *__restrict__ ent, const uint16_t *__restrict__ order,
                                                                   const int32_t *__restrict__ gofs, const int2 *__restrict__ entw,
                                                                   float *__restrict__ dst, int C, int L, int J, int E,
                                                                   long src_bstride, int nsplit, int JP) {
  extern __shared__ __attribute__((aligned(16))) float lds[];
  using vecG = __attribute__((ext_vector_type(G))) float;
  const int b = blockIdx.z, split = blockIdx.y, c0 = blockIdx.x * G, tid = threadIdx.x;
  const int g = min(G, C - c0);
  float *srcI = lds;
  float *tile = lds + (size_t)JP * G;
  const float *rows = src + (size_t)b * src_bstride + (size_t)c0 * J;
  if ((J & 3) == 0 && aligned16(rows) && ((src_bstride & 3) == 0)) {
    for (int j0 = tid * 4; j0 < J; j0 += kTileThreads * 4) {
      float4 v[G];
#pragma unroll
      for (int c = 0; c < G; ++c) v[c] = ld4(rows + (size_t)min(c, g - 1) * J + j0);
#pragma unroll
      for (int u = 0; u < 4; ++u) {
        vecG o;
#pragma unroll
        for (int c = 0; c < G; ++c) o[c] = (u == 0) ? v[c].x : (u == 1) ? v[c].y : (u == 2) ? v[c].z : v[c].w;
        *reinterpret_cast<vecG *>(srcI + (size_t)(j0 + u) * G) = o;
      }
    }
  } else {
    for (int j = tid; j < J; j += kTileThreads) {
      vecG o;
#pragma unroll
      for (int c = 0; c < G; ++c) o[c] = rows[(size_t)min(c, g - 1) * J + j];
      *reinterpret_cast<vecG *>(srcI + (size_t)j * G) = o;
    }
  }
  __syncthreads();
  const int2 *en = ent + (size_t)b * E;
  const int2 *ew = entw + (size_t)b * entw_stride(L, E) + (tid & 63);
  const uint16_t *ord = order + (size_t)b * order_stride(L);
  const int2 *sg = seg + (size_t)b * order_stride(L);
  const int32_t *go = gofs + (size_t)b * (order_stride(L) / kWave);
  const int nr = ceil_div(L, kTileTargets);
  constexpr int kSlots = kTileTargets / kTileThreads;
  int lt[kSlots], gb[kSlots];
  int2 sq[kSlots];
  auto fetch = [&](int r) {
#pragma unroll
    for (int k = 0; k < kSlots; ++k) {
      const int pos = r * kTileTargets + k * kTileThreads + tid;
      lt[k] = ord[pos];
      sq[k] = sg[pos];
      gb[k] = go[pos >> 6];
    }
  };
  if (split < nr) fetch(split);
  for (int r = split; r < nr; r += nsplit) {
    const int t0 = r * kTileTargets, nt = min(kTileTargets, L - t0);
    int clt[kSlots], cgb[kSlots];
    int2 csq[kSlots];
#pragma unroll
    for (int k = 0; k < kSlots; ++k) { clt[k] = lt[k]; csq[k] = sq[k]; cgb[k] = gb[k]; }
    if (r + nsplit < nr) fetch(r + nsplit);
#pragma unroll
    for (int k = 0; k < kSlots; ++k) {
      if (clt[k] == 0xFFFF) continue;
      const int n = csq[k].y - csq[k].x;
      const int2 *ep = cgb[k] >= 0 ? ew + cgb[k] : en + csq[k].x;
      const int estep = cgb[k] >= 0 ? 64 : 1;
      vecG acc;
#pragma unroll
      for (int c = 0; c < G; ++c) acc[c] = 0.0f;
      int i = 0;
      for (; i + 8 <= n; i += 8) {
        int2 t[8];
        vecG x[8];
#pragma unroll
        for (int u = 0; u < 8; ++u) t[u] = ep[(size_t)(i + u) * estep];
#pragma unroll
        for (int u = 0; u < 8; ++u) x[u] = *reinterpret_cast<const vecG *>(srcI + (size_t)t[u].x * G);
#pragma unroll
        for (int u = 0; u < 8; ++u) {
          const float w = __int_as_float(t[u].y);
#pragma unroll
          for (int c = 0; c < G; ++c) acc[c] = acc[c] + w * x[u][c];
        }
      }
#define PVCNN_TAIL(U)                                                                              \
      if ((n - i) & U) {                                                                           \
        int2 t[U];                                                                                 \
        vecG x[U];                                                                                 \
        _Pragma("unroll") for (int u = 0; u < U; ++u) t[u] = ep[(size_t)(i + u) * estep];          \
        _Pragma("unroll") for (int u = 0; u < U; ++u) x[u] = *reinterpret_cast<const vecG *>(srcI + (size_t)t[u].x * G); \
        _Pragma("unroll") for (int u = 0; u < U; ++u) {                                            \
          const float w = __int_as_float(t[u].y);                                                  \
          _Pragma("unroll") for (int c = 0; c < G; ++c) acc[c] = acc[c] + w * x[u][c];             \
        }                                                                                          \
        i += U;                                                                                    \
      }
      PVCNN_TAIL(4)
      PVCNN_TAIL(2)
      PVCNN_TAIL(1)
#undef PVCNN_TAIL
#pragma unroll
      for (int c = 0; c < G; ++c) tile[c * kTileTargets + clt[k]] = acc[c];
    }
    lds_barrier();
    float *out = dst + ((size_t)b * C + c0) * L + t0;
    if ((L & 3) == 0 && aligned16(dst)) {
      const int q_per_row = nt >> 2;
      for (int q = tid; q < g * q_per_row; q += kTileThreads) {
        const int c = q / q_per_row, i = (q - c * q_per_row) * 4;
        const float4 v = *reinterpret_cast<const float4 *>(tile + c * kTileTargets + i);
        using v4f = __attribute__((ext_vector_type(4))) float;
        v4f o = {v.x, v.y, v.z, v.w};
        __builtin_nontemporal_store(o, reinterpret_cast<v4f *>(out + (size_t)c * L + i));
      }
    } else {
      for (int q = tid; q < g * nt; q += kTileThreads) {
        const int c = q / nt, i = q - c * nt;
        out[(size_t)c * L + i] = tile[c * kTileTargets + i];
      }
    }
    lds_barrier();
  }
}

inline bool csr_supported(int L, long E) { return L <= kCsrMaxTargets && E <= 0x7fffffffL / 8; }

template <int G, bool STAGE>
int launch_segsum_g(const float *src, const CsrPlan &ws, float *dst, int B, int C, int L, int J, int E,
                    bool vec, int threads, hipStream_t s, const char *what, long src_bstride) {
  const size_t lds = STAGE ? (size_t)G * J * sizeof(float) : 0;
  const dim3 grid(ceil_div(C, G), B);
#define PVCNN_SEGSUM(VEC, T)                                                                          \
  do {                                                                                                \
    auto k = segsum_kernel<G, VEC, T, STAGE>;                                                         \
    if (int e = enable_big_lds(k, lds)) { set_error("%s: LDS attribute: %d", what, e); return e; }    \
    hipLaunchKernelGGL(k, grid, dim3(T), lds, s, src, ws.start, ws.ent, dst, C, L, J, E, src_bstride); \
  } while (0)
  if (threads == 1024) { if (vec) PVCNN_SEGSUM(4, 1024); else PVCNN_SEGSUM(1, 1024); }
  else                 { if (vec) PVCNN_SEGSUM(4, 256);  else PVCNN_SEGSUM(1, 256); }
#undef PVCNN_SEGSUM
  return check_launch(what);
}

template <class EP>
int launch_csr_prep(const EP &ep, int B, int L, long E_, int32_t *cnt_out, void *plan, size_t plan_bytes, void *scratch,
                    size_t scratch_bytes, hipStream_t s, const char *what) {
  const int E = (int)E_;
  if (B == 0) return 0;
  if (!plan || plan_bytes < CsrPlan::bytes(B, L, E) || !aligned16(plan) || !scratch || !aligned16(scratch) ||
      scratch_bytes < csr_prep_scratch_bytes(B, E)) {
    set_error("%s: plan / scratch missing, misaligned or too small (%zu + %zu bytes needed)", what, CsrPlan::bytes(B, L, E),
              csr_prep_scratch_bytes(B, E));
    return PVCNN_ERR_INVALID_ARGUMENT;
  }
  CsrPlan pl;
  pl.carve(plan, B, L, E);
  const CsrSplit sp = csr_split(B, L, E);
  const size_t prep_lds = ((size_t)kCsrCoarse * 2 + 4 + 32 + 4 + 3 * kCsrList + sp.HP) * sizeof(int);
  auto k = csr_prep_kernel<EP>;
  if (int e = enable_big_lds(k, prep_lds)) { set_error("%s: LDS attribute: %d", what, e); return e; }
  hipLaunchKernelGGL(k, dim3(sp.P, B), dim3(kCsrThreads), prep_lds, s, ep, E, L, sp, cnt_out, pl.start,
                     static_cast<int32_t *>(scratch), pl.ent);
  if (int e = check_launch(what)) return e;
  hipLaunchKernelGGL(csr_order_kernel, dim3(ceil_div(L, kTileTargets), B), dim3(kTileThreads), 0, s, pl.start, pl.ent, L, E, pl.order, pl.seg,
                     pl.gofs, pl.entw);
  if (int e = check_launch(what)) return e;
  hipLaunchKernelGGL(csr_interleave_kernel, dim3(order_stride(L) / 256, B), dim3(256), 0, s, pl.ent, pl.seg, pl.gofs, L, E, pl.entw);
  return check_launch(what);
}

template <class EP1, class EP2>
int launch_csr_prep_pair(const EP1 &ep1, long E1_, int32_t *cnt1, void *plan1, size_t plan1_bytes, const EP2 &ep2, long E2_, void *plan2,
                         size_t plan2_bytes, int B, int L, void *scratch, size_t scratch_bytes, hipStream_t s, const char *what) {
  const int E1 = (int)E1_, E2 = (int)E2_;
  if (B == 0) return 0;
  const size_t s1 = csr_prep_scratch_bytes(B, E1), s2 = csr_prep_scratch_bytes(B, E2);
  if (!plan1 || !plan2 || plan1_bytes < CsrPlan::bytes(B, L, E1) || plan2_bytes < CsrPlan::bytes(B, L, E2) || !aligned16(plan1) ||
      !aligned16(plan2) || !scratch || !aligned16(scratch) || scratch_bytes < s1 + s2) {
    set_error("%s: plans / scratch missing, misaligned or too small (%zu, %zu, %zu bytes needed)", what, CsrPlan::bytes(B, L, E1),
              CsrPlan::bytes(B, L, E2), s1 + s2);
    return PVCNN_ERR_INVALID_ARGUMENT;
  }
  CsrPlan p1, p2;
  p1.carve(plan1, B, L, E1);
  p2.carve(plan2, B, L, E2);
  const int total = std::max(2, std::min(16, kNumCU / std::max(B, 1)));
  const int cap1 = std::max(1, total / 4);
  const CsrSplit sp1 = csr_split(B, L, E1, cap1), sp2 = csr_split(B, L, E2, std::max(1, total - cap1));
  const size_t prep_lds = ((size_t)kCsrCoarse * 2 + 4 + 32 + 4 + 3 * kCsrList + std::max(sp1.HP, sp2.HP)) * sizeof(int);
  auto k = csr_prep_pair_kernel<EP1, EP2>;
  if (int e = enable_big_lds(k, prep_lds)) { set_error("%s: LDS attribute: %d", what, e); return e; }
  char *sc = static_cast<char *>(scratch);
  hipLaunchKernelGGL(k, dim3(sp1.P + sp2.P, B), dim3(kCsrThreads), prep_lds, s, ep1, E1, sp1, cnt1, p1.start, reinterpret_cast<int32_t *>(sc),
                     p1.ent, ep2, E2, sp2, p2.start, reinterpret_cast<int32_t *>(sc + s1), p2.ent, L);
  if (int e = check_launch(what)) return e;
  const CsrPlanRef r1{p1.start, p1.ent, p1.order, p1.seg, p1.gofs, p1.entw, E1}, r2{p2.start, p2.ent, p2.order, p2.seg, p2.gofs, p2.entw, E2};
  const int nr = ceil_div(L, kTileTargets), nblk = order_stride(L) / 256;
  hipLaunchKernelGGL(csr_order_pair_kernel, dim3(2 * nr, B), dim3(kTileThreads), 0, s, r1, r2, L, nr);
  if (int e = check_launch(what)) return e;
  hipLaunchKernelGGL(csr_interleave_pair_kernel, dim3(2 * nblk, B), dim3(256), 0, s, r1, r2, L, nblk);
  return check_launch(what);
}

inline int launch_csr_apply(const float *src, const void *plan, size_t plan_bytes, float *dst, int B, int C, int L, int J, long E_,
                            hipStream_t s, const char *what, long src_bstride = 0) {
  if (src_bstride <= 0) src_bstride = (long)C * J;
  const int E = (int)E_;
  if (B == 0 || C == 0) return 0;
  if (!plan || plan_bytes < CsrPlan::bytes(B, L, E) || !aligned16(plan)) {
    set_error("%s: plan missing, misaligned or too small (%zu bytes needed)", what, CsrPlan::bytes(B, L, E));
    return PVCNN_ERR_INVALID_ARGUMENT;
  }
  CsrPlan pl;
  pl.carve(const_cast<void *>(plan), B, L, E);
  const int JP = (J + 3) & ~3;
  int G = 0;
  for (int cand = 4; cand >= 1; cand >>= 1)
    if ((size_t)cand * (JP + kTileTargets) * sizeof(float) <= (size_t)kLdsBytesPerCU) { G = cand; break; }
  const size_t row = (size_t)J * sizeof(float);
  int GS = 1;
  if (row > 0 && row <= 64 * 1024) {
    GS = (int)std::min<size_t>(8, (64 * 1024) / row);
    while (GS > 1 && (long)B * ceil_div(C, GS) < 2L * kNumCU) GS >>= 1;
    if (GS >= 8) GS = 8; else if (GS >= 4) GS = 4; else if (GS >= 2) GS = 2; else GS = 1;
  }
  const bool very_sparse = (long)E * 4 <= (long)L && row > 0 && row <= (size_t)kLdsBytesPerCU && (long)B * ceil_div(C, GS) >= kNumCU;
  if (G > 0 && J > 0 && !very_sparse) {
    while (G > 1 && G / 2 >= C) G >>= 1;
    const int nr = ceil_div(L, kTileTargets), slabs = ceil_div(C, G);
    int nsplit = 1;
    while (nsplit < nr && (long)B * slabs * nsplit < kNumCU) nsplit <<= 1;
    nsplit = std::min(nsplit, nr);
    const size_t lds = (size_t)G * (JP + kTileTargets) * sizeof(float);
    const dim3 grid(slabs, nsplit, B);
#define PVCNN_TILE(GV)                                                                                                   \
  do {                                                                                                                   \
    auto k = segsum_tile_kernel<GV>;                                                                                     \
    if (int e = enable_big_lds(k, lds)) { set_error("%s: LDS attribute: %d", what, e); return e; }                       \
    hipLaunchKernelGGL(k, grid, dim3(kTileThreads), lds, s, src, pl.seg, pl.ent, pl.order, pl.gofs, pl.entw, dst, C, L, J, E,  \
                       src_bstride, nsplit, JP);                                                                                      \
  } while (0)
    if (G == 4) PVCNN_TILE(4); else if (G == 2) PVCNN_TILE(2); else PVCNN_TILE(1);
#undef PVCNN_TILE
    return check_launch(what);
  }
  const bool stage = row > 0 && row <= (size_t)kLdsBytesPerCU;
  const bool vec = (L % 4 == 0) && aligned16(dst);
  const int threads = (L >= 8192 || (size_t)GS * row > 48 * 1024) ? 1024 : 256;
  if (!stage) return launch_segsum_g<1, false>(src, pl, dst, B, C, L, J, E, vec, threads, s, what, src_bstride);
  switch (GS) {
    case 8: return launch_segsum_g<8, true>(src, pl, dst, B, C, L, J, E, vec, threads, s, what, src_bstride);
    case 4: return launch_segsum_g<4, true>(src, pl, dst, B, C, L, J, E, vec, threads, s, what, src_bstride);
    case 2: return launch_segsum_g<2, true>(src, pl, dst, B, C, L, J, E, vec, threads, s, what, src_bstride);
    default: return launch_segsum_g<1, true>(src, pl, dst, B, C, L, J, E, vec, threads, s, what, src_bstride);
  }
}

template <class EP>
int launch_csr_scatter(const EP &ep, const float *src, float *dst, int B, int C, int L, int J, long E,
                       int32_t *cnt_out, void *workspace, size_t workspace_bytes, hipStream_t s, const char *what,
                       long src_bstride = 0) {
  if (B == 0) return 0;
  const size_t pb = CsrPlan::bytes(B, L, E);
  if (!workspace || workspace_bytes < pb + csr_prep_scratch_bytes(B, E) || !aligned16(workspace)) {
    set_error("%s: workspace missing, misaligned or too small (%zu bytes needed)", what, pb + csr_prep_scratch_bytes(B, E));
    return PVCNN_ERR_INVALID_ARGUMENT;
  }
  char *w = static_cast<char *>(workspace);
  if (int e = launch_csr_prep(ep, B, L, E, cnt_out, w, pb, w + pb, workspace_bytes - pb, s, what)) return e;
  return launch_csr_apply(src, w, pb, dst, B, C, L, J, E, s, what, src_bstride);
}

}
```

pvcnn_amd/csrc/devoxelize.hip:

```cpp
#include "csr.h"

using namespace pvcnn;

__global__ __launch_bounds__(256) void trilinear_taps_only_kernel(TrilinearFromCoords p, int N) {
  const int b = blockIdx.y, j = blockIdx.x * 256 + threadIdx.x;
  if (j >= N) return;
  Taps<8> t;
  p.load1(b, j, t);
  p.post1(b, j, t);
}

extern "C" int pvcnn_trilinear_devox_fwd(const float *coords, const float *feat, int B, int C, int N, int R,
                                         int is_training, int32_t *inds, float *wgts, float *outs,
                                         void *stream) {
  PVCNN_REQUIRE(B >= 0 && C >= 0 && N >= 0 && R > 0, "negative size");
  PVCNN_REQUIRE((long)R * R * R <= 0x7fffffffL / 4, "resolution too large");
  if (B == 0 || N == 0) return 0;
  PVCNN_REQUIRE(coords && (outs || C == 0) && (feat || C == 0), "null pointer");
  PVCNN_REQUIRE(!is_training || (inds && wgts), "training mode needs inds and wgts");
  PVCNN_REQUIRE(B <= 65535, "batch > 65535");
  hipStream_t s = static_cast<hipStream_t>(stream);
  TrilinearFromCoords p{coords, is_training ? inds : nullptr, is_training ? wgts : nullptr, N, R, R * R};
  bool vec = (N % 4 == 0) && aligned16(coords) && aligned16(outs);
  if (is_training) vec = vec && aligned16(inds) && aligned16(wgts);
// ... 42 lines not shown
  if (is_training) vec = vec && aligned16(inds) && aligned16(wgts);
  const XfBnAct xf{gamma, beta, mean, rstd, slope, nullptr};
  const AddBnAct ax{add_gamma, add_beta, add_mean, add_rstd, add_slope};
  return launch_gather(p, feat, outs, B, C, R * R * R, N, vec, s, "trilinear_devox_bnact_addbn_fwd", xf, grid_pad_shift(R), addend, ax);
}

extern "C" size_t pvcnn_trilinear_devox_bwd_workspace_bytes(int B, int C, int N, int R) {
  if (B <= 0 || C < 0 || N < 0 || R <= 0) return 0;
  const long S = (long)R * R * R;
  if (S > 0x7fffffffL || !csr_supported((int)S, 8L * N)) return 16;
  return CsrWorkspace::bytes(B, C, (int)S, N, 8L * N);
}

static int devox_bwd_impl(const float *grad_y, long gy_bstride, const int32_t *inds, const float *wgts, int B, int C, int N,
                          int R, float *grad_x, void *workspace, size_t workspace_bytes, void *stream) {
  PVCNN_REQUIRE(B >= 0 && C >= 0 && N >= 0 && R > 0, "negative size");
  PVCNN_REQUIRE((long)R * R * R <= 0x7fffffffL / 4, "resolution too large");
  if (B == 0 || C == 0) return 0;
  PVCNN_REQUIRE(grad_x && (N == 0 || (grad_y && inds && wgts)), "null pointer");
  PVCNN_REQUIRE(B <= 65535, "batch > 65535");
  PVCNN_REQUIRE(gy_bstride >= (long)C * N, "grad_y batch stride smaller than one cloud");
  const int S = R * R * R;
  hipStream_t s = static_cast<hipStream_t>(stream);
  if (!csr_supported(S, 8L * N)) {
    PVCNN_REQUIRE(gy_bstride == (long)C * N, "the atomic fallback needs a contiguous grad_y");
    SavedTaps<8> p{inds, wgts, N};
    return launch_scatter_direct(p, grad_y, grad_x, B, C, S, N, s, "trilinear_devox_bwd(atomic)");
  }
  TapEntries<8> ep{inds, wgts, N, S};
  return launch_csr_scatter(ep, grad_y, grad_x, B, C, S, N, 8L * N, nullptr, workspace,
                            workspace_bytes, s, "trilinear_devox_bwd", gy_bstride);
}

extern "C" int pvcnn_trilinear_devox_bwd(const float *grad_y, const int32_t *inds, const float *wgts, int B,
                                         int C, int N, int R, float *grad_x, void *workspace,
                                         size_t workspace_bytes, void *stream) {
  return devox_bwd_impl(grad_y, (long)C * N, inds, wgts, B, C, N, R, grad_x, workspace, workspace_bytes, stream);
}

extern "C" int pvcnn_trilinear_devox_bwd_strided(const float *grad_y, long grad_y_batch_stride, const int32_t *inds,
                                                 const float *wgts, int B, int C, int N, int R, float *grad_x,
                                                 void *workspace, size_t workspace_bytes, void *stream) {
  return devox_bwd_impl(grad_y, grad_y_batch_stride, inds, wgts, B, C, N, R, grad_x, workspace, workspace_bytes, stream);
}

extern "C" size_t pvcnn_trilinear_devox_bwd_plan_bytes(int B, int N, int R) {
  if (B <= 0 || N < 0 || R <= 0) return 0;
  const long S = (long)R * R * R;
  if (S > 0x7fffffffL / 4 || !csr_supported((int)S, 8L * N)) return 0;
  return CsrPlan::bytes(B, (int)S, 8L * N);
}

extern "C" size_t pvcnn_trilinear_devox_bwd_plan_scratch_bytes(int B, int N, int R) {
  if (B <= 0 || N < 0 || R <= 0) return 0;
  return csr_prep_scratch_bytes(B, 8L * N);
}

extern "C" int pvcnn_trilinear_devox_bwd_plan(const int32_t *inds, const float *wgts, int B, int N, int R, void *plan,
                                              size_t plan_bytes, void *scratch, size_t scratch_bytes, void *stream) {
  PVCNN_REQUIRE(B >= 0 && N >= 0 && R > 0, "negative size");
  PVCNN_REQUIRE((long)R * R * R <= 0x7fffffffL / 4, "resolution too large");
  if (B == 0) return 0;
  const int S = R * R * R;
  PVCNN_REQUIRE(csr_supported(S, 8L * N), "grid too large for a plan: use pvcnn_trilinear_devox_bwd");
  PVCNN_REQUIRE(N == 0 || (inds && wgts), "null pointer");
  PVCNN_REQUIRE(B <= 65535, "batch > 65535");
  TapEntries<8> ep{inds, wgts, N, S};
  return launch_csr_prep(ep, B, S, 8L * N, nullptr, plan, plan_bytes, scratch, scratch_bytes,
                         static_cast<hipStream_t>(stream), "trilinear_devox_bwd_plan");
}

extern "C" int pvcnn_trilinear_devox_bwd_apply(const float *grad_y, long grad_y_batch_stride, const void *plan, size_t plan_bytes,
                                               int B, int C, int N, int R, float *grad_x, void *stream) {
  PVCNN_REQUIRE(B >= 0 && C >= 0 && N >= 0 && R > 0, "negative size");
  PVCNN_REQUIRE((long)R * R * R <= 0x7fffffffL / 4, "resolution too large");
  if (B == 0 || C == 0) return 0;
  PVCNN_REQUIRE(grad_x && (N == 0 || grad_y), "null pointer");
  PVCNN_REQUIRE(B <= 65535, "batch > 65535");
  PVCNN_REQUIRE(grad_y_batch_stride >= (long)C * N, "grad_y batch stride smaller than one cloud");
  const int S = R * R * R;
  return launch_csr_apply(grad_y, plan, plan_bytes, grad_x, B, C, S, N, 8L * N, static_cast<hipStream_t>(stream),
                          "trilinear_devox_bwd_apply", grad_y_batch_stride);
}
```

pvcnn_amd/modules/functional/backend.py:

```python
import ctypes
import os

import torch

from ... import _lib
from . import _cache
from ._align import aligned as _aligned
from ._product import CONV, PW

__all__ = ['_backend']


def _dev(t, name):
    if not t.is_cuda:
        raise RuntimeError(f'{name} must be a CUDA (HIP) tensor -- the PVConv hot path has no CPU implementation')


def _f32(t, name):
    _dev(t, name)
    if not t.is_contiguous():
        raise RuntimeError(f'{name} must be a contiguous tensor')
    if t.dtype != torch.float32:
        raise RuntimeError(f'{name} must be a float tensor')

# ... 313 lines not shown
    def _stamped_voxel_plan(self, coords, r):
        vp = self.avg_voxelize_plan(coords, r)
        return None if vp is None else (vp, (vp.ind._version, vp.cnt._version))

    def avg_voxelize_backward(self, grad_y, indices, cnt):
        _f32(grad_y, 'grad_y'); _i32(indices, 'indices'); _i32(cnt, 'cnt')
        _shape(grad_y.dim() == 3 and indices.dim() == 2 and tuple(cnt.shape) == (grad_y.shape[0], grad_y.shape[2])
               and indices.shape[0] == grad_y.shape[0],
               'avg_voxelize backward: grad_y (B,C,S), indices (B,N), cnt (B,S) expected')
        b, c, s3 = grad_y.shape
        n = indices.shape[1]
        grad_x = torch.empty((b, c, n), dtype=torch.float32, device=grad_y.device)
        _run(self.lib.pvcnn_avg_voxelize_bwd, 'avg_voxelize_backward', grad_y, grad_y, indices, cnt, b, c, n, s3, grad_x)
        return grad_x

    has_scatter_plans = True

    class VoxelPlan:
        __slots__ = ('ind', 'cnt', 'plan', 'r', 'n', 'b')

    def _voxel_plan(self, b, n, r, nbytes, dev):
        vp = self.VoxelPlan()
        vp.r, vp.n, vp.b = r, n, b
        vp.ind = torch.empty((b, n), dtype=torch.int32, device=dev)
        vp.cnt = torch.empty((b, r * r * r), dtype=torch.int32, device=dev)
        vp.plan = torch.empty((nbytes,), dtype=torch.uint8, device=dev)
        return vp

    def avg_voxelize_plan(self, coords, resolution):
        _i32(coords, 'coords')
        _shape(coords.dim() == 3 and coords.shape[1] == 3, 'avg_voxelize: coords (B,3,N) expected')
        b, _, n = coords.shape
        r = int(resolution)
        nbytes = self.lib.pvcnn_avg_voxelize_plan_bytes(b, n, r)
        if nbytes == 0:
            return None
        vp = self._voxel_plan(b, n, r, nbytes, coords.device)
        scratch = self._scratch(self.lib.pvcnn_avg_voxelize_plan_scratch_bytes(b, n, r), coords.device)
        _run(self.lib.pvcnn_avg_voxelize_plan, 'avg_voxelize_plan', coords, coords, b, n, r, vp.ind, vp.cnt, vp.plan, vp.plan.numel(),
             scratch, scratch.numel())
        return vp

    has_pvconv_plans = os.environ.get('PVCNN_PAIR_PLANS', '1') != '0'

    def pvconv_plans(self, vox_coords, norm_coords, resolution):
        _i32(vox_coords, 'vox_coords'); _f32(norm_coords, 'norm_coords')
        _shape(vox_coords.dim() == 3 and vox_coords.shape[1] == 3 and tuple(norm_coords.shape) == tuple(vox_coords.shape),
               'pvconv_plans: vox_coords / norm_coords (B,3,N) expected')
        b, _, n = vox_coords.shape
        r = int(resolution)
        vbytes, dbytes = self.lib.pvcnn_avg_voxelize_plan_bytes(b, n, r), self.lib.pvcnn_trilinear_devox_bwd_plan_bytes(b, n, r)
        if vbytes == 0 or dbytes == 0 or n == 0:
            return None
        dev = vox_coords.device
        vp = self._voxel_plan(b, n, r, vbytes, dev)
        dplan = torch.empty((dbytes,), dtype=torch.uint8, device=dev)
        scratch = self._scratch(self.lib.pvcnn_pvconv_plans_scratch_bytes(b, n, r), dev)
        _run(self.lib.pvcnn_pvconv_plans, 'pvconv_plans', vox_coords, vox_coords, norm_coords, b, n, r, vp.ind, vp.cnt, vp.plan, vp.plan.numel(),
             dplan, dplan.numel(), scratch, scratch.numel())
        return vp, dplan

    def avg_voxelize_apply(self, features, vp):
        _f32(features, 'features')
        _shape(features.dim() == 3 and features.shape[0] == vp.b and features.shape[2] == vp.n, 'avg_voxelize: features do not match the plan')
        b, c, n = features.shape
        out = torch.empty((b, c, vp.r ** 3), dtype=torch.float32, device=features.device)
        _run(self.lib.pvcnn_avg_voxelize_apply, 'avg_voxelize_apply', features, features, vp.plan, vp.plan.numel(), b, c, n, vp.r, out)
        return out

    def trilinear_devoxelize_backward_plan(self, indices, weights, r):
        _i32(indices, 'indices'); _f32(weights, 'weights')
        _shape(indices.dim() == 3 and indices.shape[1] == 8 and indices.shape == weights.shape, 'inds / wgts (B,8,N) expected')
        b, _, n = indices.shape
        r = int(r)
        nbytes = self.lib.pvcnn_trilinear_devox_bwd_plan_bytes(b, n, r)
        if nbytes == 0:
            return None
        plan = torch.empty((nbytes,), dtype=torch.uint8, device=indices.device)
        scratch = self._scratch(self.lib.pvcnn_trilinear_devox_bwd_plan_scratch_bytes(b, n, r), indices.device)
        _run(self.lib.pvcnn_trilinear_devox_bwd_plan, 'trilinear_devoxelize_backward_plan', indices, indices, weights, b, n, r,
             plan, plan.numel(), scratch, scratch.numel())
        return plan

    def trilinear_devoxelize_backward_apply(self, grad_y, plan, r):
        gy_bstride = _f32_rows(grad_y, 'grad_y')
        b, c, n = grad_y.shape
        r = int(r)
        grad_x = torch.empty((b, c, r * r * r), dtype=torch.float32, device=grad_y.device)
        _run(self.lib.pvcnn_trilinear_devox_bwd_apply, 'trilinear_devoxelize_backward_apply', grad_y, grad_y, gy_bstride, plan, plan.numel(),
             b, c, n, r, grad_x)
        return grad_x

    has_conv3d = True

    def _conv_wt(self, weight, for_bwd_data):
        co, ci = weight.shape[0], weight.shape[1]
        wt = torch.empty((ci * 27 * co,), dtype=torch.float32, device=weight.device)
        _run(self.lib.pvcnn_conv3d_weight_transform, 'conv3d_weight_transform', weight, weight, co, ci, int(for_bwd_data), wt)
        return wt

    def conv3d_forward(self, x, weight, bias, want_stats=False):
        _f32(x, 'x'); _f32(weight, 'weight')
        _shape(x.dim() == 5 and weight.dim() == 5 and tuple(weight.shape[2:]) == (3, 3, 3) and weight.shape[1] == x.shape[1]
               and x.shape[2] == x.shape[3] == x.shape[4], 'conv3d: x (B,Ci,R,R,R), weight (Co,Ci,3,3,3) expected')
        if bias is not None:
            _f32(bias, 'bias')
        b, ci, r = x.shape[0], x.shape[1], x.shape[2]
        co = weight.shape[0]
        wt = self._conv_wt(weight, False)
        y = torch.empty((b, co, r, r, r), dtype=torch.float32, device=x.device)
        if want_stats:
            part = torch.empty((co, self.lib.pvcnn_conv3d_fwd_stats_parts(b, co, r), 2), dtype=torch.float32, device=x.device)
            _run(self.lib.pvcnn_conv3d_fwd_stats, 'conv3d_forward', x, x, wt, bias, b, ci, co, r, y, part)
            return y, part
        _run(self.lib.pvcnn_conv3d_fwd, 'conv3d_forward', x, x, wt, bias, b, ci, co, r, y)
        return y

    def conv3d_backward_data(self, grad_y, weight):
        _f32(grad_y, 'grad_y'); _f32(weight, 'weight')
        b, co, r = grad_y.shape[0], grad_y.shape[1], grad_y.shape[2]
        ci = weight.shape[1]
        wt = self._conv_wt(weight, True)
        gx = torch.empty((b, ci, r, r, r), dtype=torch.float32, device=grad_y.device)
        _run(self.lib.pvcnn_conv3d_fwd, 'conv3d_backward_data', grad_y, grad_y, wt, None, b, co, ci, r, gx)
        return gx

    has_grad_out = True

    @staticmethod
    def _grad_out(dst, shape, device):
        if dst is None:
            return torch.empty(shape, dtype=torch.float32, device=device)
        _shape(tuple(dst.shape) == tuple(shape) and dst.dtype == torch.float32 and dst.is_contiguous() and dst.device == device,
               'gradient destination: contiguous float32 tensor of the gradient\'s shape expected')
        return dst

    def conv3d_backward_weight(self, x, grad_y, with_bias=False, out_w=None, out_b=None):
        _f32(x, 'x'); _f32(grad_y, 'grad_y')
        return self._backward_weight(CONV, x, grad_y, with_bias, out_w, out_b)

    has_conv3d_split = True
    conv_math = os.environ.get('PVCNN_CONV_MATH', 'f16x2')
    CONV_NSPLIT = {'f16x2': 2, 'bf16x3': 3, 'fp32': 0}

    def absmax_bits(self, x):
        _f32(x, 'x')
        x = _aligned(x)
        out = torch.empty((1,), dtype=torch.int32, device=x.device)
        _run(self.lib.pvcnn_absmax_bits, 'absmax_bits', x, x, x.numel(), out)
        return out

    PW_AMAX_SEG = 256
    _TABLE_ONLY = ctypes.c_void_p(1)
    amax_global = os.environ.get('PVCNN_AMAX_GLOBAL', '0') == '1'

    def absmax_tiles(self, x, seg, want_global=True):
        _f32(x, 'x')
        _shape(x.dim() == 3, 'absmax_tiles: x (B,C,L) expected')
        b, c, n = x.shape
        seg = int(seg)
        out = torch.empty((self.lib.pvcnn_absmax_tiles_count(b, n, seg),), dtype=torch.int32, device=x.device)
        ticket = self._tickets(1, x.device)
        want_global = want_global or self.amax_global
        _run(self.lib.pvcnn_absmax_tiles, 'absmax_tiles', x, x, b, c, n, seg, out, ticket if want_global else self._TABLE_ONLY)
        return out

    def conv_amax(self, x, want_global=True):
        return self.absmax_tiles(x.view(x.shape[0], x.shape[1], -1), x.shape[2], want_global)

    def pw_amax(self, x, want_global=True):
        return self.absmax_tiles(x, self.PW_AMAX_SEG, want_global)

    @staticmethod
    def _amax_seg(amax, tiles, seg):
# ... 446 lines not shown
        winners = torch.empty(x.shape[:-1], dtype=torch.int64, device=x.device)
        values = torch.empty(x.shape[:-1], dtype=torch.float32, device=x.device) if with_values else None
        _run(self.lib.pvcnn_row_argmax, 'row_argmax', x, x, x.numel() // k, k, winners, values)
        return (winners, values) if with_values else winners

    has_frustum_loss = True

    def frustum_box_loss(self, center, center_reg, heading_scores, size_scores, hrn, srn, hr, sr, heading_bin_id, size_template_id,
                         heading_residual, size_residual, center_t, templates, bin_centers, bin_width, w_heading, w_size, w_corners):
        outs = (center, center_reg, heading_scores, size_scores, hrn, srn, hr, sr)
        for t in outs + (heading_residual, size_residual, center_t, templates, bin_centers):
            _f32(t, 'frustum_box_loss input')
        b, nh, ns = center.shape[0], heading_scores.shape[1], size_scores.shape[1]
        _shape(tuple(center.shape) == (b, 3) and tuple(center_reg.shape) == (b, 3) and tuple(center_t.shape) == (b, 3)
               and tuple(heading_scores.shape) == (b, nh) and tuple(hrn.shape) == (b, nh) and tuple(hr.shape) == (b, nh)
               and tuple(size_scores.shape) == (b, ns) and tuple(srn.shape) == (b, ns, 3) and tuple(sr.shape) == (b, ns, 3)
               and tuple(heading_residual.shape) == (b,) and tuple(size_residual.shape) == (b, 3) and tuple(templates.shape) == (ns, 3)
               and tuple(bin_centers.shape) == (nh,) and tuple(heading_bin_id.shape) == (b,) and tuple(size_template_id.shape) == (b,)
               and heading_bin_id.dtype == torch.int64 and size_template_id.dtype == torch.int64
               and heading_bin_id.is_contiguous() and size_template_id.is_contiguous(), 'frustum_box_loss: shapes of modules/frustum.py:57-75 expected')
        loss = torch.empty((), dtype=torch.float32, device=center.device)
        grads = torch.empty((self.lib.pvcnn_frustum_box_loss_grad_floats(b, nh, ns),), dtype=torch.float32, device=center.device)
        _run(self.lib.pvcnn_frustum_box_loss, 'frustum_box_loss', center, *outs, heading_bin_id, size_template_id, heading_residual,
             size_residual, center_t, templates, bin_centers, b, nh, ns, float(bin_width), float(w_heading), float(w_size),
             float(w_corners), loss, grads)
        return loss, grads

    has_se_excite = True

    def se_excite_forward(self, part, gamma, beta, w1, w2, s3):
        c, b, slices, _ = part.shape
        h = w1.shape[0]
        _shape(tuple(w1.shape) == (h, c) and tuple(w2.shape) == (c, h) and c <= 2048 and h <= 256, 'se_excite: W1 (H,C), W2 (C,H), C <= 2048, H <= 256')
        dev = part.device
        a_sum, ax_sum, squeezed, excite = (torch.empty((b, c), dtype=torch.float32, device=dev) for _ in range(4))
        hidden = torch.empty((b, h), dtype=torch.float32, device=dev)
        _run(self.lib.pvcnn_se_excite_fwd, 'se_excite_fwd', part, part, slices, gamma, beta, w1, w2, b, c, h, 1.0 / float(s3),
             a_sum, ax_sum, squeezed, hidden, excite)
        return a_sum, ax_sum, squeezed, hidden, excite

    def se_excite_backward(self, part, a_sum, ax_sum, gamma, beta, squeezed, hidden, excite, w1, w2, s3):
        c, b, slices, _ = part.shape
        h = w1.shape[0]
        dev = part.device
        g_w1 = torch.empty((h, c), dtype=torch.float32, device=dev)
        g_w2 = torch.empty((c, h), dtype=torch.float32, device=dev)
        g_mean = torch.empty((b, c), dtype=torch.float32, device=dev)
        sum_beta = torch.empty((c,), dtype=torch.float32, device=dev)
        sum_gamma = torch.empty((c,), dtype=torch.float32, device=dev)
        ws = torch.empty((b * (3 * c + h),), dtype=torch.float32, device=dev)
        _run(self.lib.pvcnn_se_excite_bwd, 'se_excite_bwd', part, part, slices, a_sum, ax_sum, gamma, beta, squeezed, hidden, excite, w1, w2,
             b, c, h, 1.0 / float(s3), g_w1, g_w2, g_mean, sum_beta, sum_gamma, ws)
        return g_w1, g_w2, g_mean, sum_beta, sum_gamma

    def bnact_partial_sums_raw(self, x, grad_y, gamma, beta, mean, rstd, slope):
        _f32(x, 'x')
        b, c, s3 = x.shape
        gy_bstride = _f32_rows(grad_y, 'grad_y') if grad_y is not None else c * s3
        slices = self.lib.pvcnn_bnact_slices(s3)
        part = torch.empty((c, b, slices, 2), dtype=torch.float32, device=x.device)
        _run(self.lib.pvcnn_bnact_partial_sums, 'bnact_partial_sums', x, x, grad_y, gy_bstride, gamma, beta, mean, rstd, b, c, s3,
             float(slope), part)
        return part

    def bnact_partial_sums(self, x, grad_y, gamma, beta, mean, rstd, slope):
        sums = self.bnact_partial_sums_raw(x, grad_y, gamma, beta, mean, rstd, slope).sum(dim=2)
        return sums[..., 0].t().contiguous(), sums[..., 1].t().contiguous()

    def bnact_backward_apply(self, x, grad_y, gamma, beta, mean, rstd, sum_gamma, sum_beta, slope, training, bc_mul=None, bc_add=None,
                             amax_seg=256):
        _f32(x, 'x')
        gy_bstride = _f32_rows(grad_y, 'grad_y')
        b, c, s3 = x.shape
        for t, name in ((bc_mul, 'bc_mul'), (bc_add, 'bc_add')):
            if t is not None:
                _f32(t, name)
                _shape(tuple(t.shape) == (b, c), f'{name} (B,C) expected')
        gx = torch.empty_like(x)
        amax = self.amax_buffer(b, s3, amax_seg, x.device)
        _run(self.lib.pvcnn_bnact_bwd_apply, 'bnact_backward_apply', x, x, grad_y, gy_bstride, gamma, beta, mean, rstd, sum_gamma, sum_beta,
             bc_mul, bc_add, b, c, s3, float(slope), int(bool(training)), gx, amax, int(amax_seg))
        return gx, amax

    def bnact_backward(self, x, grad_y, gamma, beta, mean, rstd, slope, training, amax_seg=0, drop=None, out_w=None, out_b=None):
        _f32(x, 'x')
        gy_bstride = _f32_rows(grad_y, 'grad_y')
        b, c, s3 = x.shape
        dev = x.device
        gx = torch.empty_like(x)
        gg = self._grad_out(out_w, (c,), dev)
        gb = self._grad_out(out_b, (c,), dev)
        ws = self._scratch(self.lib.pvcnn_bnact_workspace_bytes(b, c, s3), dev)
        amax_seg = int(amax_seg)
        gx_amax = self.amax_buffer(b, s3, amax_seg, dev) if amax_seg > 0 else None
        tickets = self._tickets(c, dev)
        _run(self.lib.pvcnn_bnact_bwd_strided, 'bnact_backward', x, x, grad_y, gy_bstride, gamma, beta, mean, rstd, b, c, s3, float(slope),
             int(bool(training)), gx, gg, gb, gx_amax, amax_seg, ws, ws.numel(), drop[0] if drop else None,
             float(drop[1]) if drop else 0.0, tickets)
        return (gx, gg, gb, gx_amax) if amax_seg > 0 else (gx, gg, gb)

    def eval_tile(self, src, shuffled, num_points, channels, strides, src_points):
        _f32(src, 'src'); _dev(shuffled, 'shuffled')
        _shape(shuffled.dtype == torch.int64 and shuffled.dim() == 2 and shuffled.is_contiguous(), 'eval_tile: shuffled (B,V) int64 expected')
        b, v = shuffled.shape
        np_, c, (bs, ps, cs) = int(num_points), int(channels), (int(x) for x in strides)
        _shape(np_ > 0 and v % np_ == 0 and c > 0, 'eval_tile: V must be a multiple of num_points')
        _shape(min(bs, ps, cs) >= 0 and (b == 0 or (b - 1) * bs + (int(src_points) - 1) * ps + (c - 1) * cs < src.numel()),
               'eval_tile: strides reach beyond src')
        out = torch.empty((b * (v // np_), c, np_), dtype=torch.float32, device=src.device)
        _run(self.lib.pvcnn_eval_tile, 'eval_tile', src, src, bs, ps, cs, int(src_points), shuffled, b, v, np_, c, out)
        return out

    def vote_confidence(self, logits, class_range=None):
        _f32(logits, 'logits')
        _shape(logits.dim() == 3, 'vote_confidence: logits (B,C,N) expected')
        b, c, n = logits.shape
        table = None
        if class_range is None:
            c0, c1 = 0, c
        elif isinstance(class_range, torch.Tensor):
            _i32(class_range, 'class_range')
            _shape(tuple(class_range.shape) == (b, 2), 'vote_confidence: class_range table (B,2) expected')
            table, c0, c1 = class_range, 0, 0
        else:
            c0, c1 = int(class_range[0]), int(class_range[1])
            _shape(0 <= c0 < c1 <= c, 'vote_confidence: class range must satisfy 0 <= c0 < c1 <= C')
        conf = torch.empty((b, n), dtype=torch.float32, device=logits.device)
        pred = torch.empty((b, n), dtype=torch.int32, device=logits.device)
        _run(self.lib.pvcnn_vote_confidence, 'vote_confidence', logits, logits, b, c, n, c0, c1, table, conf, pred)
        return conf, pred

    def vote_merge(self, conf, pred, shuffled, scene_conf, scene_pred, keys, mapping=None):
        _f32(conf, 'conf'); _i32(pred, 'pred'); _f32(scene_conf, 'scene_conf')
        for t, name in ((shuffled, 'shuffled'), (scene_pred, 'scene_pred'), (keys, 'keys')):
            _dev(t, name)
            _shape(t.dtype == torch.int64 and t.is_contiguous(), f'vote_merge: {name} must be a contiguous int64 tensor')
        _shape(conf.dim() == 2 and conf.shape == pred.shape == shuffled.shape, 'vote_merge: conf, pred, shuffled (B,V) expected')
        b, v = conf.shape
        p = scene_conf.numel()
        _shape(scene_pred.numel() == p and keys.numel() == p, 'vote_merge: scene_pred (P) and a (P) key workspace expected')
        map_stride = 0
        if mapping is not None:
            _dev(mapping, 'mapping')
            _shape(mapping.dtype == torch.int64 and mapping.is_contiguous() and mapping.dim() == 2 and mapping.shape[0] >= b,
                   'vote_merge: mapping (>= B, M) contiguous int64 expected')
            map_stride = mapping.shape[1]
        _run(self.lib.pvcnn_vote_merge, 'vote_merge', conf, conf, pred, shuffled, mapping, map_stride, b, v, p, scene_conf, scene_pred,
             keys, keys.numel() * 8)

    def seg_counts(self, gt, pred, num_classes, counts=None, wrap_negative=True):
        for t, name in ((gt, 'gt'), (pred, 'pred')):
            _dev(t, name)
            _shape(t.dtype == torch.int64 and t.is_contiguous(), f'seg_counts: {name} must be a contiguous int64 tensor')
        _shape(gt.numel() == pred.numel(), 'seg_counts: gt and pred must have the same number of points')
        c = int(num_classes)
        if counts is None:
            counts = torch.zeros((3, c), dtype=torch.int64, device=gt.device)
        _shape(counts.dtype == torch.int64 and counts.is_contiguous() and counts.numel() == 3 * c, 'seg_counts: counts (3,C) int64')
        _run(self.lib.pvcnn_seg_counts, 'seg_counts', gt, gt, pred, gt.numel(), c, int(bool(wrap_negative)), counts)
        return counts

    def seg_meter_update(self, logits, targets, counts=None, part_ranges=None, max_parts=0, rows=None, row_cursor=None):
        _f32(logits, 'logits'); _dev(targets, 'targets')
        _shape(logits.dim() == 3 and targets.dtype == torch.int64 and targets.is_contiguous()
               and tuple(targets.shape) == (logits.shape[0], logits.shape[2]), 'seg_meter_update: logits (B,C,N), targets (B,N) int64')
        b, c, n = logits.shape
        if part_ranges is None:
            _shape(counts is not None and counts.dtype == torch.int64 and counts.is_contiguous() and counts.numel() == 3 * c + 2,
                   'seg_meter_update: counts (3C+2) int64 expected')
            tail = (None, 0, 0, counts, None, None, 0)
        else:
            _i32(part_ranges, 'part_ranges')
            _shape(part_ranges.dim() == 2 and part_ranges.shape[1] == 2, 'seg_meter_update: part_ranges (K,2) int32 expected')
            _i32(rows, 'rows')
            _shape(rows.dim() == 3 and rows.shape[1:] == (int(max_parts) + 1, 2), 'seg_meter_update: rows (capacity, max_parts+1, 2)')
            if row_cursor is not None:
                _dev(row_cursor, 'row_cursor')
                _shape(row_cursor.dtype == torch.int64 and row_cursor.numel() == 1, 'seg_meter_update: row_cursor: one int64')
            tail = (part_ranges, part_ranges.shape[0], int(max_parts), None, rows, row_cursor, rows.shape[0])
# ... 292 lines not shown
```

pvcnn_amd/modules/functional/bnact.py:

```python
import contextlib
import threading

import torch
import torch.nn as nn
from torch.autograd import Function

from . import _cache, _fold, _gradslots, _product
from ._align import aligned as _aligned
from ._autograd import native, amp_fwd, amp_bwd
from ._fold import folded_parameters
from .backend import batch_strided_ok
from .devoxelization import CornerTaps


def _rows(t, shape):
    if t.dim() == len(shape) and t.dim() >= 3:
        try:
            v = t.view(shape[0], shape[1], -1) if t.dim() > 3 else t
            if batch_strided_ok(v):
                return v
        except RuntimeError:
            pass
    return t.contiguous().view(shape[0], shape[1], -1)


def _servable(x):
    return x.dtype == torch.float32 or (torch.is_autocast_enabled() and x.dtype in (torch.bfloat16, torch.float16))


def _amax_seg_for(shape, is_cuda):
    be = native()
    if not is_cuda:
        return 0
    cap = getattr(be, 'BNACT_AMAX_MAX_SEG', 0)
    if len(shape) == 5 and shape[2] == shape[3] == shape[4]:
        ok = getattr(be, 'has_conv3d_split', False) and getattr(be, 'conv_math', '') == 'f16x2'
        return int(shape[2]) if ok and shape[2] <= cap else 0
    if len(shape) in (3, 4):
        ok = getattr(be, 'has_pwconv_split', False) and getattr(be, 'pw_math', '') == 'f16x2'
        seg = getattr(be, 'PW_AMAX_SEG', 0)
        return seg if ok and 0 < seg <= cap else 0
    return 0


def _bnact_backward(x3, g3, w, b, mean, rstd, slope, training, shape, drop=None):
    be = native()
    seg = _amax_seg_for(shape, x3.is_cuda)
    dst = _gradslots.destinations(be, w, b)
    if seg:
        gx, gw, gb, amax = be.bnact_backward(x3, g3, w, b, mean, rstd, slope, training, amax_seg=seg, **({'drop': drop} if drop else {}), **dst)
        return _cache.tag_amax(gx.view(shape), seg, amax), gw, gb
    assert drop is None, 'the fused dropout rides on the amax-emitting passes'
    gx, gw, gb = be.bnact_backward(x3, g3, w, b, mean, rstd, slope, training, **dst)
    return gx.view(shape), gw, gb


def _prologue(x, weight, bias):
    return (x.shape, x.contiguous().view(x.shape[0], x.shape[1], -1), weight.contiguous() if weight is not None else None,
            bias.contiguous() if bias is not None else None)


def _statistics(x3, use_batch_stats, stats_part, stats_shift, running_mean, running_var, momentum, eps, counter, zero_word=None):
    if use_batch_stats and stats_part is not None:
        return native().bn_finalize(stats_part, x3.shape[0] * x3.shape[2], running_mean, running_var, momentum, eps, stats_shift,
                                    **({'zero_word': zero_word} if zero_word is not None else {}), counter=counter)
    if use_batch_stats:
        return native().bn_stats(x3, running_mean, running_var, momentum, eps)
    return running_mean.contiguous(), torch.rsqrt(running_var + eps)


__all__ = ['batch_norm_act', 'batch_norm_act_devoxelize', 'batch_norm_act_se_devoxelize', 'batch_norm_act_devoxelize_point_bn',
           'point_bn_fusable', 'fusable_tail', 'run_layers', 'fused_dropout_ok',
           'folded_parameters', 'folded_snapshot']


class BatchNormAct(Function):
    @staticmethod
    @amp_fwd
    def forward(ctx, x, weight, bias, running_mean, running_var, training, momentum, eps, slope, stats_part=None, stats_shift=None,
                amax_seg=0, counter=None, drop_p=0.0, drop_seed=None, row_max=False):
        shape, x3, w, b = _prologue(x, weight, bias)
        stats = whole = armed = keys = None
        if training and stats_part is not None:
            if amax_seg and row_max:
                whole, armed, keys = native().amax_and_row_keys(x3.shape[0], x3.shape[1], x3.shape[2], amax_seg, x3.device)
            elif amax_seg:
                whole = armed = native().amax_buffer(x3.shape[0], x3.shape[2], amax_seg, x3.device)
            stats = _statistics(x3, True, stats_part, stats_shift, running_mean, running_var, momentum, eps, counter, zero_word=whole)
            if keys is not None:
                ctx.slope, ctx.training, ctx.shape, ctx.drop = slope, training, shape, None
                dest = getattr(_ROW_MAX, 'out', None)
                if dest is not None and not (dest.is_cuda and tuple(dest.shape) == tuple(x3.shape) and dest.dtype == torch.float32):
                    dest = None
                y, winners, values = native().bnact_apply_rowmax(x3, w, b, stats[0], stats[1], slope, amax_seg, armed, keys, out=dest)
                ctx.save_for_backward(x3, w, b, stats[0], stats[1])
                ctx.mark_non_differentiable(armed, winners, values)
                ctx.set_materialize_grads(False)
                return y.view(shape), armed, winners, values
        ctx.slope, ctx.training, ctx.shape = slope, training, shape
        ctx.drop = (drop_seed, float(drop_p)) if (drop_p and drop_seed is not None) else None
        if amax_seg:
            y, mean, rstd, amax = native().bnact_forward(x3, w, b, running_mean, running_var, training, momentum, eps, slope, stats=stats,
                                                         amax_seg=amax_seg, y_amax=armed, **({'drop': ctx.drop} if ctx.drop else {}))
            ctx.save_for_backward(x3, w, b, mean, rstd)
            ctx.mark_non_differentiable(amax)
            ctx.set_materialize_grads(False)
            return y.view(shape), amax
        y, mean, rstd = native().bnact_forward(x3, w, b, running_mean, running_var, training, momentum, eps, slope, stats=stats)
        ctx.save_for_backward(x3, w, b, mean, rstd)
        return y.view(shape)

    @staticmethod
    @amp_bwd
    def backward(ctx, grad_y, grad_amax=None, grad_winners=None, grad_values=None):
        if grad_y is None:
            return (None,) * 16
        x3, w, b, mean, rstd = ctx.saved_tensors
        g3 = _rows(grad_y, ctx.shape)
        gx, gw, gb = _bnact_backward(x3, g3, w, b, mean, rstd, ctx.slope, ctx.training, ctx.shape, drop=ctx.drop)
        return (gx, gw if w is not None else None, gb if b is not None else None) + (None,) * 13


_ROW_MAX = threading.local()


@contextlib.contextmanager
def emit_row_max(bn, out=None):
    prev = (getattr(_ROW_MAX, 'bn', None), getattr(_ROW_MAX, 'out', None))
    _ROW_MAX.bn, _ROW_MAX.out = bn, out
    try:
        yield
    finally:
        _ROW_MAX.bn, _ROW_MAX.out = prev


def _bn_mode(bn, finalize_counts=False):
    use_batch_stats = bn.training or bn.running_mean is None
    momentum = 0.0 if bn.momentum is None else bn.momentum
    counter = None
    if bn.training and bn.track_running_stats and bn.num_batches_tracked is not None:
        nbt = bn.num_batches_tracked
        if (finalize_counts and bn.momentum is not None and nbt.is_cuda and nbt.dtype == torch.int64 and nbt.numel() == 1):
            counter = nbt
        else:
            nbt.add_(1)
            if bn.momentum is None:
                momentum = 1.0 / float(nbt)
    rm = bn.running_mean if (bn.track_running_stats or not use_batch_stats) else None
    rv = bn.running_var if (bn.track_running_stats or not use_batch_stats) else None
    return use_batch_stats, momentum, rm, rv, counter


def _split(stats):
    if stats is None:
        return None, None
    part, shift = stats
    return part, (shift.detach().contiguous() if shift is not None else None)


def _module_call(bn, stats_part):
    return (*_bn_mode(bn, finalize_counts=stats_part is not None and bn.training), *_split(stats_part))


def fused_dropout_ok(x):
    return (x.is_cuda and x.dtype == torch.float32 and getattr(native(), 'has_bnact_dropout', False) and not torch.is_autocast_enabled()
            and _amax_seg_for(x.shape, True) > 0 and 0 < x.numel() < (1 << 33))


def batch_norm_act(x, bn, slope, stats_part=None, drop_p=0.0):
    use_batch_stats, momentum, rm, rv, counter, part, shift = _module_call(bn, stats_part)
    seg = _amax_seg_for(x.shape, x.is_cuda)
    if (seg and bn is getattr(_ROW_MAX, 'bn', None) and not drop_p and use_batch_stats and part is not None and x.dim() == 3
            and x.shape[2] % 256 == 0 and seg % 4 == 0 and x.dtype == torch.float32 and x.data_ptr() % 16 == 0 and x.is_contiguous()
            and getattr(native(), 'has_bnact_rowmax', False)):
        y, amax, winners, values = BatchNormAct.apply(x, bn.weight, bn.bias, rm, rv, use_batch_stats, momentum, bn.eps, slope, part, shift,
                                                      seg, counter, 0.0, None, True)
        y._pvcnn_row_max = (winners, values, y._version)
        return _cache.tag_amax(y, seg, amax)
    if seg:
        seed = torch.randint(-(1 << 62), 1 << 62, (1,), dtype=torch.int64, device=x.device) if drop_p else None
        y, amax = BatchNormAct.apply(x, bn.weight, bn.bias, rm, rv, use_batch_stats, momentum, bn.eps, slope, part, shift, seg, counter,
                                     float(drop_p), seed)
        return _cache.tag_amax(y, seg, amax)
    assert not drop_p, 'fused dropout: see fused_dropout_ok'
    return BatchNormAct.apply(x, bn.weight, bn.bias, rm, rv, use_batch_stats, momentum, bn.eps, slope, part, shift, 0, counter)


class BatchNormActDevoxelize(Function):

    @staticmethod
    @amp_fwd
    def forward(ctx, grid, coords, weight, bias, running_mean, running_var, use_batch_stats, momentum, eps, slope,
                resolution, is_training, stats_part=None, stats_shift=None, addend=None, counter=None):
        shape, x3, w, b = _prologue(grid, weight, bias)
        mean, rstd = _statistics(x3, use_batch_stats, stats_part, stats_shift, running_mean, running_var, momentum, eps, counter)
        r = int(resolution)
        pts = coords.contiguous()
        add = addend.contiguous() if addend is not None else None
        ctx.has_addend = add is not None
        if not is_training:
            return native().trilinear_devoxelize_bnact_forward(r, False, pts, x3, w, b, mean, rstd, slope, add)[0]
        taps = CornerTaps.of(coords, r)
        out = taps.forward(lambda emit: native().trilinear_devoxelize_bnact_forward(r, emit, pts, x3, w, b, mean, rstd, slope, add))
        ctx.save_for_backward(x3, w, b, mean, rstd, taps.inds, taps.wgts)
        ctx.taps = taps
        ctx.slope, ctx.use_batch_stats, ctx.shape = slope, use_batch_stats, shape
        return out

    @staticmethod
    @amp_bwd
    def backward(ctx, grad_out):
        x3, w, b, mean, rstd, _, _ = ctx.saved_tensors
        g_act = ctx.taps.backward(_rows(grad_out, grad_out.shape))
        gx, gw, gb = _bnact_backward(x3, g_act.view(x3.shape), w, b, mean, rstd, ctx.slope, ctx.use_batch_stats, ctx.shape)
        return (gx, None, gw if w is not None else None, gb if b is not None else None) + (None,) * 10 + (grad_out if ctx.has_addend else None, None)


def batch_norm_act_devoxelize(grid, coords, bn, slope, resolution, is_training, stats_part=None, addend=None):
    use_batch_stats, momentum, rm, rv, counter, part, shift = _module_call(bn, stats_part)
    return BatchNormActDevoxelize.apply(grid, coords, bn.weight, bn.bias, rm, rv, use_batch_stats, momentum, bn.eps, slope,
                                        resolution, is_training, part, shift, addend, counter)


class BatchNormActDevoxelizePointBN(Function):

    @staticmethod
    @amp_fwd
    def forward(ctx, grid, coords, weight, bias, running_mean, running_var, momentum, eps, slope, resolution, stats_part, stats_shift,
                counter, pre, p_weight, p_bias, p_running_mean, p_running_var, p_momentum, p_eps, p_slope, p_stats_part, p_stats_shift,
                p_counter):
        shape, x3, w, b = _prologue(grid, weight, bias)
        p_shape, pre3, pw, pb = _prologue(pre, p_weight, p_bias)
        p_mean, p_rstd = _statistics(pre3, True, p_stats_part, p_stats_shift, p_running_mean, p_running_var, p_momentum, p_eps, p_counter)
        mean, rstd = _statistics(x3, True, stats_part, stats_shift, running_mean, running_var, momentum, eps, counter)
        r = int(resolution)
        pts = coords.contiguous()
        taps = CornerTaps.of(coords, r)
        out = taps.forward(lambda emit: native().trilinear_devoxelize_bnact_forward(
            r, emit, pts, x3, w, b, mean, rstd, slope, pre3, addend_bn=(pw, pb, p_mean, p_rstd, p_slope)))
        ctx.save_for_backward(x3, w, b, mean, rstd, pre3, pw, pb, p_mean, p_rstd, taps.inds, taps.wgts)
        ctx.taps = taps
        ctx.slope, ctx.shape, ctx.p_slope, ctx.p_shape = slope, shape, p_slope, p_shape
        return out

    @staticmethod
    @amp_bwd
    def backward(ctx, grad_out):
        x3, w, b, mean, rstd, pre3, pw, pb, p_mean, p_rstd, _, _ = ctx.saved_tensors
        g_rows = _rows(grad_out, grad_out.shape)
        g_act = ctx.taps.backward(g_rows)
        gx, gw, gb = _bnact_backward(x3, g_act.view(x3.shape), w, b, mean, rstd, ctx.slope, True, ctx.shape)
        gp, gpw, gpb = _bnact_backward(pre3, g_rows, pw, pb, p_mean, p_rstd, ctx.p_slope, True, ctx.p_shape)
        return ((gx, None, gw if w is not None else None, gb if b is not None else None) + (None,) * 9
                + (gp, gpw if pw is not None else None, gpb if pb is not None else None) + (None,) * 8)


def point_bn_fusable(point_layers, features, training):
    be = native()
    if not (training and getattr(be, 'has_point_branch_fused', False) and getattr(be, 'has_pwconv', False)
            and getattr(be, 'has_bnact', False)):
        return None
    mods = list(point_layers)
    if len(mods) != 3 or _has_hooks(point_layers) or any(_has_hooks(m) for m in mods):
        return None
    conv, bn, act = mods
    if not (_is_pointwise(conv) and isinstance(conv, nn.Conv1d) and isinstance(bn, nn.BatchNorm1d) and _slope(act) is not None):
        return None
    if not (bn.training and conv.weight.dtype == torch.float32 and getattr(conv, _fold.ATTR, None) is None):
        return None
    if not (features.is_cuda and features.dtype == torch.float32 and features.dim() == 3 and features.numel() > 0
            and not torch.is_autocast_enabled() and torch.is_grad_enabled()):
        return None
    return conv, bn, _slope(act)


def batch_norm_act_devoxelize_point_bn(grid, coords, bn, slope, resolution, stats_part, pre, p_bn, p_slope, p_stats_part):
    _, momentum, rm, rv, counter, part, shift = _module_call(bn, stats_part)
    _, p_momentum, p_rm, p_rv, p_counter, p_part, p_shift = _module_call(p_bn, p_stats_part)
    return BatchNormActDevoxelizePointBN.apply(grid, coords, bn.weight, bn.bias, rm, rv, momentum, bn.eps, slope, resolution, part, shift,
                                               counter, pre, p_bn.weight, p_bn.bias, p_rm, p_rv, p_momentum, p_bn.eps, p_slope, p_part,
                                               p_shift, p_counter)


def _se_excite_forward(sums, gamma, beta, w1, w2, s3):
    a_sum, ax_sum = sums
    gam = gamma if gamma is not None else torch.ones_like(a_sum[0])
    bet = beta if beta is not None else torch.zeros_like(a_sum[0])
    squeezed = (gam * ax_sum + bet * a_sum) / float(s3)
    hidden = torch.relu(squeezed @ w1.t())
    excite = torch.sigmoid(hidden @ w2.t()).contiguous()
    return a_sum, ax_sum, squeezed, hidden, excite


def _se_excite_backward(sums, a_sum, ax_sum, gamma, beta, squeezed, hidden, excite, w1, w2, s3):
    p_sum, q_sum = sums
    gam = gamma if gamma is not None else torch.ones_like(p_sum[0])
    bet = beta if beta is not None else torch.zeros_like(p_sum[0])
    g_excite = gam * q_sum + bet * p_sum
    g_pre2 = g_excite * excite * (1.0 - excite)
    g_w2 = g_pre2.t() @ hidden
    g_pre1 = (g_pre2 @ w2) * (hidden > 0).to(hidden.dtype)
    g_w1 = g_pre1.t() @ squeezed
    g_mean = ((g_pre1 @ w1) / float(s3)).contiguous()
    sum_beta = (excite * p_sum + g_mean * a_sum).sum(dim=0).contiguous()
    sum_gamma = (excite * q_sum + g_mean * ax_sum).sum(dim=0).contiguous()
    return g_w1, g_w2, g_mean, sum_beta, sum_gamma


class BatchNormActSEDevoxelize(Function):

    @staticmethod
    @amp_fwd
    def forward(ctx, grid, coords, weight, bias, running_mean, running_var, use_batch_stats, momentum, eps, slope,
                resolution, is_training, stats_part, stats_shift, addend, counter, fc1, fc2):
        be = native()
        shape, x3, w, b = _prologue(grid, weight, bias)
        mean, rstd = _statistics(x3, use_batch_stats, stats_part, stats_shift, running_mean, running_var, momentum, eps, counter)
        w1, w2 = fc1.contiguous(), fc2.contiguous()
        fused = ctx.fused_se = getattr(be, 'has_se_excite', False) and x3.shape[1] <= 2048 and w1.shape[0] <= 256
        sums = (be.bnact_partial_sums_raw if fused else be.bnact_partial_sums)(x3, None, w, b, mean, rstd, slope)
        a_sum, ax_sum, squeezed, hidden, excite = (be.se_excite_forward if fused else _se_excite_forward)(sums, w, b, w1, w2, x3.shape[2])
        r = int(resolution)
        pts = coords.contiguous()
        add = addend.contiguous() if addend is not None else None
        ctx.has_addend = add is not None
        if not is_training:
            return be.trilinear_devoxelize_bnact_forward(r, False, pts, x3, w, b, mean, rstd, slope, add, se_scale=excite)[0]
        taps = CornerTaps.of(coords, r)
        out = taps.forward(lambda emit: be.trilinear_devoxelize_bnact_forward(r, emit, pts, x3, w, b, mean, rstd, slope, add, se_scale=excite))
        ctx.save_for_backward(x3, w, b, mean, rstd, a_sum, ax_sum, squeezed, hidden, excite, w1, w2, taps.inds, taps.wgts)
        ctx.taps = taps
        ctx.slope, ctx.use_batch_stats, ctx.shape = slope, use_batch_stats, shape
        return out

# ... 162 lines not shown
```

pvcnn_amd/modules/functional/devoxelization.py:

```python
from torch.autograd import Function

from . import _cache
from ._autograd import native, amp_fwd, amp_bwd

__all__ = ['trilinear_devoxelize', 'CornerTaps']


class CornerTaps:
    __slots__ = ('inds', 'wgts', 'plan', 'r')

    def __init__(self, r):
        self.inds = self.wgts = self.plan = None
        self.r = int(r)

    @staticmethod
    def of(coords, r):
        if coords.is_cuda and getattr(native(), 'has_scatter_plans', False):
            return _cache.memo(coords, ('corner_taps', int(r)), lambda: CornerTaps(r))
        return CornerTaps(r)

    def forward(self, run):
        if self.inds is None:
            outs, self.inds, self.wgts = run(True)
        else:
            outs = run(False)[0]
        return outs

    def backward(self, grad_points):
        be = native()
        if getattr(be, 'has_scatter_plans', False) and grad_points.is_cuda:
            if self.plan is None:
                made = be.trilinear_devoxelize_backward_plan(self.inds, self.wgts, self.r)
                self.plan = made if made is not None else False
            if self.plan is not False:
                return be.trilinear_devoxelize_backward_apply(grad_points, self.plan, self.r)
        return be.trilinear_devoxelize_backward(grad_points, self.inds, self.wgts, self.r)


class TrilinearDevoxelization(Function):

    @staticmethod
    @amp_fwd
    def forward(ctx, features, coords, resolution, is_training=True):
        nb, nc = features.shape[0], features.shape[1]
        grid = features.contiguous().view(nb, nc, -1)
        r = int(resolution)
        if not is_training:
            return native().trilinear_devoxelize_forward(r, False, coords.contiguous(), grid)[0]
        taps = CornerTaps.of(coords, r)
        pts = coords.contiguous()
        outs = taps.forward(lambda emit: native().trilinear_devoxelize_forward(r, emit, pts, grid))
        ctx.save_for_backward(taps.inds, taps.wgts)
        ctx.taps = taps
        return outs

    @staticmethod
    @amp_bwd
    def backward(ctx, grad_points):
        r = ctx.taps.r
        grad_grid = ctx.taps.backward(grad_points.contiguous())
        return grad_grid.view(grad_points.shape[0], grad_points.shape[1], r, r, r), None, None, None


trilinear_devoxelize = TrilinearDevoxelization.apply
```

Before: 2510 point-clouds/s.

## Skip untapped voxel rows in devoxelize backward and fused BN-act backward

Builds a per-sample bitmask of voxel rows (runs of length R along the grid) that any point's trilinear corner taps actually touch, cached alongside the scatter plan. The devoxelize backward scatter then writes only tapped rows, and the fused BN+activation backward reduce and apply kernels skip loading and processing grad_y for rows whose gradient is known to be zero. The aim is to cut memory traffic over the sparse R^3 grid at resolution 32. It adds a mask-building kernel and extra per-element mask checks, and it is restricted to aligned, non-dropout, amax-emitting paths with autocast disabled.

```diff
diff --git a/include/pvcnn_hip.h b/include/pvcnn_hip.h
--- a/include/pvcnn_hip.h
+++ b/include/pvcnn_hip.h
@@ -58,6 +58,10 @@
                                    size_t plan_bytes, void *scratch, size_t scratch_bytes, void *stream);
 PVCNN_API int pvcnn_trilinear_devox_bwd_apply(const float *grad_y, long grad_y_batch_stride, const void *plan, size_t plan_bytes,
                                     int B, int C, int N, int R, float *grad_x, void *stream);
+PVCNN_API int pvcnn_trilinear_devox_bwd_row_mask(const void *plan, size_t plan_bytes, int B, int N, int R, void *row_mask,
+                                    void *stream);
+PVCNN_API int pvcnn_trilinear_devox_bwd_apply_rows(const float *grad_y, long grad_y_batch_stride, const void *plan, size_t plan_bytes,
+                                    const void *row_mask, int B, int C, int N, int R, float *grad_x, void *stream);
 
 PVCNN_API int pvcnn_ball_query(const float *centers, const float *points, int B, int N, int M, float radius,
                      int U, int32_t *out, void *stream);
@@ -200,6 +204,11 @@
                             float slope, int training, float *grad_x, float *grad_gamma, float *grad_beta,
                             void *gx_amax, int amax_seg, void *workspace, size_t workspace_bytes, const void *drop_seed,
                             float drop_p, void *tickets, void *stream);
+PVCNN_API int pvcnn_bnact_bwd_strided_rows(const float *x, const float *grad_y, long grad_y_batch_stride, const float *gamma,
+                            const float *beta, const float *mean, const float *rstd, int B, int C, int S,
+                            float slope, int training, float *grad_x, float *grad_gamma, float *grad_beta,
+                            void *gx_amax, int amax_seg, void *workspace, size_t workspace_bytes, void *tickets,
+                            const void *row_mask, int row_len, void *stream);
 PVCNN_API int pvcnn_bnact_slices(int S);
 PVCNN_API long pvcnn_conv3d_weight_split_pair_entry(const float *w, int Co, int Ci, void *wts_fwd, void *wts_bwd, long long *entry);
 PVCNN_API int pvcnn_conv3d_weight_split_pair_batch(const void *table, int n, long total_rows, void *stream);
diff --git a/pvcnn_amd/_lib.py b/pvcnn_amd/_lib.py
--- a/pvcnn_amd/_lib.py
+++ b/pvcnn_amd/_lib.py
@@ -33,6 +33,8 @@
     'pvcnn_trilinear_devox_bwd_plan_scratch_bytes': (_sz, [_i, _i, _i]),
     'pvcnn_trilinear_devox_bwd_plan': (_i, [_vp, _vp, _i, _i, _i, _vp, _sz, _vp, _sz, _vp]),
     'pvcnn_trilinear_devox_bwd_apply': (_i, [_vp, ctypes.c_long, _vp, _sz, _i, _i, _i, _i, _vp, _vp]),
+    'pvcnn_trilinear_devox_bwd_row_mask': (_i, [_vp, _sz, _i, _i, _i, _vp, _vp]),
+    'pvcnn_trilinear_devox_bwd_apply_rows': (_i, [_vp, ctypes.c_long, _vp, _sz, _vp, _i, _i, _i, _i, _vp, _vp]),
     'pvcnn_ball_query': (_i, [_vp, _vp, _i, _i, _i, _f, _i, _vp, _vp]),
     'pvcnn_grouping_fwd': (_i, [_vp, _vp, _i, _i, _i, _i, _i, _vp, _vp]),
     'pvcnn_grouping_bwd_workspace_bytes': (_sz, [_i, _i, _i, _i, _i]),
@@ -106,6 +108,7 @@
     'pvcnn_bnact_bwd_apply': (_i, [_vp, _vp, ctypes.c_long, _vp, _vp, _vp, _vp, _vp, _vp, _vp, _vp, _i, _i, _i, _f, _i, _vp, _vp, _i, _vp]),
     'pvcnn_bnact_bwd': (_i, [_vp, _vp, _vp, _vp, _vp, _vp, _i, _i, _i, _f, _i, _vp, _vp, _vp, _vp, _sz, _vp]),
     'pvcnn_bnact_bwd_strided': (_i, [_vp, _vp, ctypes.c_long, _vp, _vp, _vp, _vp, _i, _i, _i, _f, _i, _vp, _vp, _vp, _vp, _i, _vp, _sz, _vp, _f, _vp, _vp]),
+    'pvcnn_bnact_bwd_strided_rows': (_i, [_vp, _vp, ctypes.c_long, _vp, _vp, _vp, _vp, _i, _i, _i, _f, _i, _vp, _vp, _vp, _vp, _i, _vp, _sz, _vp, _vp, _i, _vp]),
     'pvcnn_concat_points': (_i, [_vp, _vp, _vp, _vp, _vp, _i, _i, _i, _vp, _vp, _vp, _vp]),
     'pvcnn_dense_bn_relu_supported': (_i, [_i, _i, _i]),
     'pvcnn_dense_bn_relu_fwd': (_i, [_vp] * 8 + [_i, _i, _i, _f, _f, _vp, _vp, _vp, _vp, _vp]),
diff --git a/pvcnn_amd/csrc/bnact.hip b/pvcnn_amd/csrc/bnact.hip
--- a/pvcnn_amd/csrc/bnact.hip
+++ b/pvcnn_amd/csrc/bnact.hip
@@ -138,7 +138,7 @@
   long zero_count;
 };
 
-template <bool DROP = false>
+template <bool DROP = false, bool ROWS = false>
 __global__ __launch_bounds__(kBnThreads) void bnact_bwd_reduce_kernel(const float *__restrict__ x, const float *__restrict__ gy,
                                                                      const float *__restrict__ mean,
                                                                      const float *__restrict__ rstd,
@@ -146,7 +146,9 @@
                                                                      const float *__restrict__ beta, float slope, int C,
                                                                      int S, int slices, float2 *__restrict__ part,
                                                                      long gy_bstride, Drop drop = Drop{nullptr, 0u, 1.0f},
-                                                                     BwdFold fold = BwdFold{nullptr, nullptr, nullptr, nullptr, 0L}) {
+                                                                     BwdFold fold = BwdFold{nullptr, nullptr, nullptr, nullptr, 0L},
+                                                                     RowMaskArg<ROWS> rows = RowMaskArg<ROWS>{}) {
+  static_assert(!(DROP && ROWS), "rows mode: no fused dropout");
   __shared__ float sm[16];
   uint32_t k0 = 0u, k1 = 0u;
   if constexpr (DROP) { const unsigned long long key = *drop.key; k0 = (uint32_t)key; k1 = (uint32_t)(key >> 32); }
@@ -178,7 +180,18 @@
     }
   };
   const float4 ones = make_float4(1.0f, 1.0f, 1.0f, 1.0f);
-  if ((S & 3) == 0 && aligned16(x + off) && (!gy || aligned16(gy + goff))) {
+  if constexpr (ROWS) {
+    __shared__ uint32_t mw[kBnSlice / 4 / 32 + 2];
+    const int row_len = rows.row_len;
+    const int w0 = (lo / row_len) >> 5, w1 = ((hi - 1) / row_len) >> 5;
+    for (int w = w0 + (int)threadIdx.x; w <= w1; w += kBnThreads) mw[w - w0] = rows.mask[(size_t)b * rows.words + w];
+    __syncthreads();
+    for (int i = lo + threadIdx.x * 4; i < hi; i += kBnThreads * 4) {
+      const int row = i / row_len;
+      if (((mw[(row >> 5) - w0] >> (row & 31)) & 1u) == 0u) continue;
+      quad(i, *reinterpret_cast<const float4 *>(x + off + i), *reinterpret_cast<const float4 *>(gy + goff + i));
+    }
+  } else if ((S & 3) == 0 && aligned16(x + off) && (!gy || aligned16(gy + goff))) {
     for (int i = lo + threadIdx.x * 4; i < hi; i += kBnThreads * 4)
       quad(i, *reinterpret_cast<const float4 *>(x + off + i), gy ? *reinterpret_cast<const float4 *>(gy + goff + i) : ones);
   } else if ((S & 3) == 0) {
@@ -297,7 +310,7 @@
   if (values) values[row] = y[(size_t)(row / C) * y_bstride + (size_t)(row % C) * S + k];
 }
 
-template <bool BWD, bool DROP = false, bool ROWMAX = false>
+template <bool BWD, bool DROP = false, bool ROWMAX = false, bool ROWS = false>
 __global__ __launch_bounds__(256) void bnact_apply_pb_kernel(const float *__restrict__ x, const float *__restrict__ gy, long gy_bstride,
                                                              const float *__restrict__ mean, const float *__restrict__ rstd,
                                                              const float *__restrict__ gamma, const float *__restrict__ beta,
@@ -307,8 +320,10 @@
                                                              int global_by_atomic, const float *__restrict__ bc_mul = nullptr,
                                                              const float *__restrict__ bc_add = nullptr, int cgroup = 0x7fffffff,
                                                              int table_by_atomic = 0, Drop drop = Drop{nullptr, 0u, 1.0f},
-                                                             unsigned long long *__restrict__ row_keys = nullptr, long out_bstride = 0) {
+                                                             unsigned long long *__restrict__ row_keys = nullptr, long out_bstride = 0,
+                                                             RowMaskArg<ROWS> rows = RowMaskArg<ROWS>{}) {
   static_assert(!ROWMAX || (!BWD && !DROP), "row maxima: plain forward pass only");
+  static_assert(!ROWS || (BWD && !DROP), "rows mode: plain backward pass only");
   __shared__ uint32_t seg_max[256];
   int lin = blockIdx.x + (int)gridDim.x * (blockIdx.y + (int)gridDim.y * blockIdx.z);
   const int bz = lin % (int)gridDim.z; lin /= (int)gridDim.z;
@@ -353,7 +368,9 @@
   };
   const size_t ebase = (size_t)b * C * S + p0;
   if (pos < span) {
-    if (vec) {
+    [[maybe_unused]] bool tapped = true;
+    if constexpr (ROWS) tapped = rows.tapped(b, p0 + pos);
+    if (ROWS || vec) {
       using v4f = __attribute__((ext_vector_type(4))) float;
       constexpr int RF = 8;
       for (int c0 = cbeg + wave; c0 < cend; c0 += 4 * RF) {
@@ -364,7 +381,8 @@
           xv[u] = gv[u] = make_float4(0.f, 0.f, 0.f, 0.f);
           if (c < cend) {
             xv[u] = *reinterpret_cast<const float4 *>(xb + (size_t)c * S + pos);
-            if constexpr (BWD) gv[u] = *reinterpret_cast<const float4 *>(gb + (size_t)c * S + pos);
+            if constexpr (BWD && ROWS) { if (tapped) gv[u] = *reinterpret_cast<const float4 *>(gb + (size_t)c * S + pos); }
+            else if constexpr (BWD) gv[u] = *reinterpret_cast<const float4 *>(gb + (size_t)c * S + pos);
           }
         }
 #pragma unroll
@@ -569,7 +587,7 @@
                           const float *mean, const float *rstd, int B, int C, int S, float slope, int training, float *grad_x,
                           float *grad_gamma, float *grad_beta, void *workspace, size_t workspace_bytes, void *stream,
                           void *gx_amax = nullptr, int amax_seg = 0, const void *drop_seed = nullptr, float drop_p = 0.0f,
-                          void *tickets = nullptr) {
+                          void *tickets = nullptr, const uint32_t *row_mask = nullptr, int row_len = 0) {
   PVCNN_REQUIRE(drop_p >= 0.0f && drop_p < 1.0f, "drop_p must be in [0, 1)");
   Drop drop{nullptr, 0u, 1.0f};
   const bool dropping = make_drop(drop_seed, drop_p, &drop);
@@ -586,7 +604,11 @@
   const long zero_count = gx_amax ? 1 + (long)B * ceil_div(S, amax_seg) : 0L;
   PVCNN_REQUIRE(!tickets || (reinterpret_cast<uintptr_t>(tickets) & 3) == 0, "tickets must be 4-byte aligned");
   const BwdFold fold{static_cast<unsigned *>(tickets), grad_gamma, grad_beta, static_cast<uint32_t *>(gx_amax), zero_count};
-  if (dropping)
+  const int mask_words = row_mask ? ceil_div(S / row_len, 32) : 0;
+  if (row_mask)
+    hipLaunchKernelGGL((bnact_bwd_reduce_kernel<false, true>), grid, dim3(kBnThreads), 0, s, x, grad_y, mean, rstd, gamma, beta, slope, C, S, slices,
+                       part, gy_bstride, Drop{nullptr, 0u, 1.0f}, fold, RowMask{row_mask, row_len, mask_words});
+  else if (dropping)
     hipLaunchKernelGGL(bnact_bwd_reduce_kernel<true>, grid, dim3(kBnThreads), 0, s, x, grad_y, mean, rstd, gamma, beta, slope, C, S, slices, part,
                        gy_bstride, drop, fold);
   else
@@ -604,7 +626,12 @@
     const int vec = (S % 4 == 0) && (amax_seg % 4 == 0) && (gy_bstride % 4 == 0) && aligned16(x) && aligned16(grad_y) && aligned16(grad_x);
     uint32_t *am = static_cast<uint32_t *>(gx_amax);
     const int groups = pb_channel_groups((long)ceil_div(nseg, spb) * B, C);
-    if (dropping)
+    if (row_mask)
+      hipLaunchKernelGGL((bnact_apply_pb_kernel<true, false, false, true>), dim3(ceil_div(nseg, spb), B, groups), dim3(256), 0, s, x, grad_y,
+                         gy_bstride, mean, rstd, gamma, beta, grad_gamma, grad_beta, slope, inv_count, training, C, S, amax_seg, nseg, vec, grad_x,
+                         am, 1, nullptr, nullptr, ceil_div(C, groups), groups > 1 ? 1 : 0, Drop{nullptr, 0u, 1.0f}, nullptr, 0L,
+                         RowMask{row_mask, row_len, mask_words});
+    else if (dropping)
       hipLaunchKernelGGL((bnact_apply_pb_kernel<true, true>), dim3(ceil_div(nseg, spb), B, groups), dim3(256), 0, s, x, grad_y, gy_bstride, mean,
                          rstd, gamma, beta, grad_gamma, grad_beta, slope, inv_count, training, C, S, amax_seg, nseg, vec, grad_x, am, 1, nullptr,
                          nullptr, ceil_div(C, groups), groups > 1 ? 1 : 0, drop);
@@ -633,6 +660,21 @@
                                        void *stream) {
   return bnact_bwd_impl(x, grad_y, grad_y_batch_stride, gamma, beta, mean, rstd, B, C, S, slope, training, grad_x, grad_gamma,
                         grad_beta, workspace, workspace_bytes, stream, gx_amax, amax_seg, drop_seed, drop_p, tickets);
+}
+
+extern "C" int pvcnn_bnact_bwd_strided_rows(const float *x, const float *grad_y, long grad_y_batch_stride, const float *gamma,
+                                            const float *beta, const float *mean, const float *rstd, int B, int C, int S, float slope,
+                                            int training, float *grad_x, float *grad_gamma, float *grad_beta, void *gx_amax,
+                                            int amax_seg, void *workspace, size_t workspace_bytes, void *tickets, const void *row_mask,
+                                            int row_len, void *stream) {
+  PVCNN_REQUIRE(row_mask && (reinterpret_cast<uintptr_t>(row_mask) & 3) == 0, "rows mode: row_mask missing or not 4-byte aligned");
+  PVCNN_REQUIRE(row_len > 0 && row_len % 4 == 0 && S > 0 && S % row_len == 0, "rows mode: row_len must be a multiple of 4 that divides S");
+  PVCNN_REQUIRE(gx_amax && amax_seg % 4 == 0, "rows mode: the amax-emitting apply pass only (gx_amax given, amax_seg a multiple of 4)");
+  PVCNN_REQUIRE(aligned16(x) && aligned16(grad_y) && aligned16(grad_x) && grad_y_batch_stride % 4 == 0,
+                "rows mode: x, grad_y and grad_x must be 16-byte aligned, grad_y_batch_stride a multiple of 4");
+  return bnact_bwd_impl(x, grad_y, grad_y_batch_stride, gamma, beta, mean, rstd, B, C, S, slope, training, grad_x, grad_gamma, grad_beta,
+                        workspace, workspace_bytes, stream, gx_amax, amax_seg, nullptr, 0.0f, tickets,
+                        static_cast<const uint32_t *>(row_mask), row_len);
 }
 
 extern "C" int pvcnn_bnact_slices(int S) { return S > 0 ? ceil_div(S, kBnSlice) : 0; }
diff --git a/pvcnn_amd/csrc/common.h b/pvcnn_amd/csrc/common.h
--- a/pvcnn_amd/csrc/common.h
+++ b/pvcnn_amd/csrc/common.h
@@ -2,6 +2,8 @@
 #include <hip/hip_runtime.h>
 #include <stdint.h>
 #include <stddef.h>
+
+#include <type_traits>
 
 #include "../../include/pvcnn_hip.h"
 #include "switches.h"
@@ -18,6 +20,17 @@
 __host__ __device__ inline int ceil_div(int a, int b) { return (a + b - 1) / b; }
 inline int grid_pad_shift(int R) { int s = 0; while ((1 << s) < R) ++s; return ((1 << s) == R && R >= 4) ? s : 0; }
 __host__ __device__ inline bool aligned16(const void *p) { return (reinterpret_cast<uintptr_t>(p) & 15) == 0; }
+
+struct RowMask {
+  const uint32_t *mask;
+  int row_len, words;
+  __device__ __forceinline__ bool tapped(int sample, int position) const {
+    const int row = position / row_len;
+    return ((mask[(size_t)sample * words + (row >> 5)] >> (row & 31)) & 1u) != 0u;
+  }
+};
+struct NoRowMask {};
+template <bool ROWS> using RowMaskArg = typename std::conditional<ROWS, RowMask, NoRowMask>::type;
 
 constexpr long kFoldTableMax = 1024;
 int launch_amax_reduce(uint32_t *out, long T, hipStream_t s);
diff --git a/pvcnn_amd/csrc/csr.h b/pvcnn_amd/csrc/csr.h
--- a/pvcnn_amd/csrc/csr.h
+++ b/pvcnn_amd/csrc/csr.h
@@ -568,12 +568,12 @@
                       (int)blockIdx.y);
 }
 
-template <int G>
+template <int G, bool ROWS = false>
 __global__ __launch_bounds__(kTileThreads) void segsum_tile_kernel(const float *__restrict__ src, const int2 *__restrict__ seg,
                                                                    const int2 *__restrict__ ent, const uint16_t *__restrict__ order,
                                                                    const int32_t *__restrict__ gofs, const int2 *__restrict__ entw,
                                                                    float *__restrict__ dst, int C, int L, int J, int E,
-                                                                   long src_bstride, int nsplit, int JP) {
+                                                                   long src_bstride, int nsplit, int JP, RowMaskArg<ROWS> rmask) {
   extern __shared__ __attribute__((aligned(16))) float lds[];
   using vecG = __attribute__((ext_vector_type(G))) float;
   const int b = blockIdx.z, split = blockIdx.y, c0 = blockIdx.x * G, tid = threadIdx.x;
@@ -674,10 +674,13 @@
     }
     lds_barrier();
     float *out = dst + ((size_t)b * C + c0) * L + t0;
-    if ((L & 3) == 0 && aligned16(dst)) {
+    if (ROWS || ((L & 3) == 0 && aligned16(dst))) {
       const int q_per_row = nt >> 2;
       for (int q = tid; q < g * q_per_row; q += kTileThreads) {
         const int c = q / q_per_row, i = (q - c * q_per_row) * 4;
+        if constexpr (ROWS) {
+          if (!rmask.tapped(b, t0 + i)) continue;
+        }
         const float4 v = *reinterpret_cast<const float4 *>(tile + c * kTileTargets + i);
         using v4f = __attribute__((ext_vector_type(4))) float;
         v4f o = {v.x, v.y, v.z, v.w};
@@ -691,6 +694,16 @@
     }
     lds_barrier();
   }
+}
+
+static __global__ __launch_bounds__(256) void csr_row_mask_kernel(const int32_t *__restrict__ start, int L, int row_len, int rows,
+                                                                  uint32_t *__restrict__ mask, int mask_words) {
+  const int b = blockIdx.y, row = blockIdx.x * 256 + threadIdx.x, lane = threadIdx.x & 63;
+  const int32_t *st = start + (size_t)b * start_stride(L);
+  const bool any = row < rows && st[(size_t)(row + 1) * row_len] > st[(size_t)row * row_len];
+  const unsigned long long bits = __ballot(any);
+  const int word = row >> 5;
+  if ((lane & 31) == 0 && word < mask_words) mask[(size_t)b * mask_words + word] = (uint32_t)(bits >> (lane & 32));
 }
 
 inline bool csr_supported(int L, long E) { return L <= kCsrMaxTargets && E <= 0x7fffffffL / 8; }
@@ -773,7 +786,7 @@
 }
 
 inline int launch_csr_apply(const float *src, const void *plan, size_t plan_bytes, float *dst, int B, int C, int L, int J, long E_,
-                            hipStream_t s, const char *what, long src_bstride = 0) {
+                            hipStream_t s, const char *what, long src_bstride = 0, const uint32_t *row_mask = nullptr, int row_len = 0) {
   if (src_bstride <= 0) src_bstride = (long)C * J;
   const int E = (int)E_;
   if (B == 0 || C == 0) return 0;
@@ -794,7 +807,7 @@
     while (GS > 1 && (long)B * ceil_div(C, GS) < 2L * kNumCU) GS >>= 1;
     if (GS >= 8) GS = 8; else if (GS >= 4) GS = 4; else if (GS >= 2) GS = 2; else GS = 1;
   }
-  const bool very_sparse = (long)E * 4 <= (long)L && row > 0 && row <= (size_t)kLdsBytesPerCU && (long)B * ceil_div(C, GS) >= kNumCU;
+  const bool very_sparse = !row_mask && (long)E * 4 <= (long)L && row > 0 && row <= (size_t)kLdsBytesPerCU && (long)B * ceil_div(C, GS) >= kNumCU;
   if (G > 0 && J > 0 && !very_sparse) {
     while (G > 1 && G / 2 >= C) G >>= 1;
     const int nr = ceil_div(L, kTileTargets), slabs = ceil_div(C, G);
@@ -808,9 +821,18 @@
     auto k = segsum_tile_kernel<GV>;                                                                                     \
     if (int e = enable_big_lds(k, lds)) { set_error("%s: LDS attribute: %d", what, e); return e; }                       \
     hipLaunchKernelGGL(k, grid, dim3(kTileThreads), lds, s, src, pl.seg, pl.ent, pl.order, pl.gofs, pl.entw, dst, C, L, J, E,  \
-                       src_bstride, nsplit, JP);                                                                                      \
+                       src_bstride, nsplit, JP, NoRowMask{});                                                                         \
   } while (0)
-    if (G == 4) PVCNN_TILE(4); else if (G == 2) PVCNN_TILE(2); else PVCNN_TILE(1);
+#define PVCNN_TILE_ROWS(GV)                                                                                             \
+  do {                                                                                                                   \
+    auto k = segsum_tile_kernel<GV, true>;                                                                               \
+    if (int e = enable_big_lds(k, lds)) { set_error("%s: LDS attribute: %d", what, e); return e; }                       \
+    hipLaunchKernelGGL(k, grid, dim3(kTileThreads), lds, s, src, pl.seg, pl.ent, pl.order, pl.gofs, pl.entw, dst, C, L, J, E,  \
+                       src_bstride, nsplit, JP, RowMask{row_mask, row_len, ceil_div(L / row_len, 32)});                        \
+  } while (0)
+    if (row_mask) { if (G == 4) PVCNN_TILE_ROWS(4); else if (G == 2) PVCNN_TILE_ROWS(2); else PVCNN_TILE_ROWS(1); }
+    else if (G == 4) PVCNN_TILE(4); else if (G == 2) PVCNN_TILE(2); else PVCNN_TILE(1);
+#undef PVCNN_TILE_ROWS
 #undef PVCNN_TILE
     return check_launch(what);
   }
@@ -826,6 +848,21 @@
   }
 }
 
+inline int launch_csr_row_mask(const void *plan, size_t plan_bytes, int B, int L, long E_, int row_len, uint32_t *mask, hipStream_t s,
+                               const char *what) {
+  const int E = (int)E_;
+  if (B == 0) return 0;
+  if (!plan || plan_bytes < CsrPlan::bytes(B, L, E) || !aligned16(plan)) {
+    set_error("%s: plan missing, misaligned or too small (%zu bytes needed)", what, CsrPlan::bytes(B, L, E));
+    return PVCNN_ERR_INVALID_ARGUMENT;
+  }
+  CsrPlan pl;
+  pl.carve(const_cast<void *>(plan), B, L, E);
+  const int rows = L / row_len, words = ceil_div(rows, 32);
+  hipLaunchKernelGGL(csr_row_mask_kernel, dim3(ceil_div(rows, 256), B), dim3(256), 0, s, pl.start, L, row_len, rows, mask, words);
+  return check_launch(what);
+}
+
 template <class EP>
 int launch_csr_scatter(const EP &ep, const float *src, float *dst, int B, int C, int L, int J, long E,
                        int32_t *cnt_out, void *workspace, size_t workspace_bytes, hipStream_t s, const char *what,
diff --git a/pvcnn_amd/csrc/devoxelize.hip b/pvcnn_amd/csrc/devoxelize.hip
--- a/pvcnn_amd/csrc/devoxelize.hip
+++ b/pvcnn_amd/csrc/devoxelize.hip
@@ -148,3 +148,32 @@
   return launch_csr_apply(grad_y, plan, plan_bytes, grad_x, B, C, S, N, 8L * N, static_cast<hipStream_t>(stream),
                           "trilinear_devox_bwd_apply", grad_y_batch_stride);
 }
+
+extern "C" int pvcnn_trilinear_devox_bwd_row_mask(const void *plan, size_t plan_bytes, int B, int N, int R, void *row_mask,
+                                                  void *stream) {
+  PVCNN_REQUIRE(B >= 0 && N >= 0 && R > 0, "negative size");
+  PVCNN_REQUIRE((long)R * R * R <= 0x7fffffffL / 4, "resolution too large");
+  if (B == 0) return 0;
+  PVCNN_REQUIRE(row_mask && (reinterpret_cast<uintptr_t>(row_mask) & 3) == 0, "row_mask missing or not 4-byte aligned");
+  PVCNN_REQUIRE(B <= 65535, "batch > 65535");
+  const int S = R * R * R;
+  PVCNN_REQUIRE(csr_supported(S, 8L * N), "grid too large for a plan");
+  return launch_csr_row_mask(plan, plan_bytes, B, S, 8L * N, R, static_cast<uint32_t *>(row_mask),
+                             static_cast<hipStream_t>(stream), "trilinear_devox_bwd_row_mask");
+}
+
+extern "C" int pvcnn_trilinear_devox_bwd_apply_rows(const float *grad_y, long grad_y_batch_stride, const void *plan, size_t plan_bytes,
+                                                    const void *row_mask, int B, int C, int N, int R, float *grad_x, void *stream) {
+  PVCNN_REQUIRE(B >= 0 && C >= 0 && N >= 0 && R > 0, "negative size");
+  PVCNN_REQUIRE((long)R * R * R <= 0x7fffffffL / 4, "resolution too large");
+  PVCNN_REQUIRE(R % 4 == 0, "rows mode: R must be a multiple of 4 (a 16-byte store lies in one row)");
+  PVCNN_REQUIRE(row_mask && (reinterpret_cast<uintptr_t>(row_mask) & 3) == 0, "rows mode: row_mask missing or not 4-byte aligned");
+  PVCNN_REQUIRE(aligned16(grad_x), "rows mode: grad_x must be 16-byte aligned");
+  if (B == 0 || C == 0) return 0;
+  PVCNN_REQUIRE(grad_x && (N == 0 || grad_y), "null pointer");
+  PVCNN_REQUIRE(B <= 65535, "batch > 65535");
+  PVCNN_REQUIRE(grad_y_batch_stride >= (long)C * N, "grad_y batch stride smaller than one cloud");
+  const int S = R * R * R;
+  return launch_csr_apply(grad_y, plan, plan_bytes, grad_x, B, C, S, N, 8L * N, static_cast<hipStream_t>(stream),
+                          "trilinear_devox_bwd_apply_rows", grad_y_batch_stride, static_cast<const uint32_t *>(row_mask), R);
+}
diff --git a/pvcnn_amd/modules/functional/backend.py b/pvcnn_amd/modules/functional/backend.py
--- a/pvcnn_amd/modules/functional/backend.py
+++ b/pvcnn_amd/modules/functional/backend.py
@@ -419,14 +419,27 @@
              plan, plan.numel(), scratch, scratch.numel())
         return plan
 
-    def trilinear_devoxelize_backward_apply(self, grad_y, plan, r):
+    def trilinear_devoxelize_backward_apply(self, grad_y, plan, r, row_mask=None, out=None):
         gy_bstride = _f32_rows(grad_y, 'grad_y')
         b, c, n = grad_y.shape
         r = int(r)
-        grad_x = torch.empty((b, c, r * r * r), dtype=torch.float32, device=grad_y.device)
+        grad_x = out if out is not None else torch.empty((b, c, r * r * r), dtype=torch.float32, device=grad_y.device)
+        if row_mask is not None:
+            _run(self.lib.pvcnn_trilinear_devox_bwd_apply_rows, 'trilinear_devoxelize_backward_apply', grad_y, grad_y, gy_bstride, plan,
+                 plan.numel(), row_mask, b, c, n, r, grad_x)
+            return grad_x
         _run(self.lib.pvcnn_trilinear_devox_bwd_apply, 'trilinear_devoxelize_backward_apply', grad_y, grad_y, gy_bstride, plan, plan.numel(),
              b, c, n, r, grad_x)
         return grad_x
+
+    has_tail_rows = os.environ.get('PVCNN_TAIL_ROWS', '0') == '1'
+
+    def trilinear_devoxelize_backward_row_mask(self, plan, b, n, r):
+        r = int(r)
+        mask = torch.empty((int(b), (r * r + 31) // 32), dtype=torch.int32, device=plan.device)
+        _run(self.lib.pvcnn_trilinear_devox_bwd_row_mask, 'trilinear_devoxelize_backward_row_mask', plan, plan, plan.numel(), int(b), int(n), r,
+             mask)
+        return mask
 
     has_conv3d = True
 
@@ -1039,7 +1052,8 @@
              bc_mul, bc_add, b, c, s3, float(slope), int(bool(training)), gx, amax, int(amax_seg))
         return gx, amax
 
-    def bnact_backward(self, x, grad_y, gamma, beta, mean, rstd, slope, training, amax_seg=0, drop=None, out_w=None, out_b=None):
+    def bnact_backward(self, x, grad_y, gamma, beta, mean, rstd, slope, training, amax_seg=0, drop=None, out_w=None, out_b=None,
+                       row_mask=None, row_len=0):
         _f32(x, 'x')
         gy_bstride = _f32_rows(grad_y, 'grad_y')
         b, c, s3 = x.shape
@@ -1051,7 +1065,13 @@
         amax_seg = int(amax_seg)
         gx_amax = self.amax_buffer(b, s3, amax_seg, dev) if amax_seg > 0 else None
         tickets = self._tickets(c, dev)
-        _run(self.lib.pvcnn_bnact_bwd_strided, 'bnact_backward', x, x, grad_y, gy_bstride, gamma, beta, mean, rstd, b, c, s3, float(slope),
+        if row_mask is not None:
+            if drop:
+                raise RuntimeError('bnact_backward: rows mode has no fused dropout')
+            _run(self.lib.pvcnn_bnact_bwd_strided_rows, 'bnact_backward', x, x, grad_y, gy_bstride, gamma, beta, mean, rstd, b, c, s3,
+                 float(slope), int(bool(training)), gx, gg, gb, gx_amax, amax_seg, ws, ws.numel(), tickets, row_mask, int(row_len))
+            return (gx, gg, gb, gx_amax) if amax_seg > 0 else (gx, gg, gb)
+        _run(self.lib.pvcnn_bnact_bwd_strided,'bnact_backward', x, x, grad_y, gy_bstride, gamma, beta, mean, rstd, b, c, s3, float(slope),
              int(bool(training)), gx, gg, gb, gx_amax, amax_seg, ws, ws.numel(), drop[0] if drop else None,
              float(drop[1]) if drop else 0.0, tickets)
         return (gx, gg, gb, gx_amax) if amax_seg > 0 else (gx, gg, gb)
diff --git a/pvcnn_amd/modules/functional/bnact.py b/pvcnn_amd/modules/functional/bnact.py
--- a/pvcnn_amd/modules/functional/bnact.py
+++ b/pvcnn_amd/modules/functional/bnact.py
@@ -43,16 +43,31 @@
     return 0
 
 
-def _bnact_backward(x3, g3, w, b, mean, rstd, slope, training, shape, drop=None):
+def _bnact_backward(x3, g3, w, b, mean, rstd, slope, training, shape, drop=None, rows=None):
     be = native()
     seg = _amax_seg_for(shape, x3.is_cuda)
     dst = _gradslots.destinations(be, w, b)
+    if rows is not None:
+        assert seg and drop is None, 'rows mode rides on the amax-emitting passes'
+        dst = dict(dst, row_mask=rows[0], row_len=rows[1])
     if seg:
         gx, gw, gb, amax = be.bnact_backward(x3, g3, w, b, mean, rstd, slope, training, amax_seg=seg, **({'drop': drop} if drop else {}), **dst)
         return _cache.tag_amax(gx.view(shape), seg, amax), gw, gb
     assert drop is None, 'the fused dropout rides on the amax-emitting passes'
     gx, gw, gb = be.bnact_backward(x3, g3, w, b, mean, rstd, slope, training, **dst)
     return gx.view(shape), gw, gb
+
+
+def _tail_backward(taps, g_rows, x3, w, b, mean, rstd, slope, training, shape, rows_ok):
+    be = native()
+    seg = _amax_seg_for(shape, x3.is_cuda)
+    mask = None
+    if (rows_ok and training and getattr(be, 'has_tail_rows', False) and g_rows.is_cuda and seg > 0 and seg % 4 == 0
+            and x3.data_ptr() % 16 == 0):
+        mask = taps.row_mask(g_rows)
+    g_act = taps.backward(g_rows, **({'row_mask': mask} if mask is not None else {}))
+    return _bnact_backward(x3, g_act.view(x3.shape), w, b, mean, rstd, slope, training, shape,
+                           **({'rows': (mask, taps.r)} if mask is not None else {}))
 
 
 def _prologue(x, weight, bias):
@@ -191,13 +206,14 @@
     @staticmethod
     @amp_fwd
     def forward(ctx, grid, coords, weight, bias, running_mean, running_var, use_batch_stats, momentum, eps, slope,
-                resolution, is_training, stats_part=None, stats_shift=None, addend=None, counter=None):
+                resolution, is_training, stats_part=None, stats_shift=None, addend=None, counter=None, rows_ok=False):
         shape, x3, w, b = _prologue(grid, weight, bias)
         mean, rstd = _statistics(x3, use_batch_stats, stats_part, stats_shift, running_mean, running_var, momentum, eps, counter)
         r = int(resolution)
         pts = coords.contiguous()
         add = addend.contiguous() if addend is not None else None
         ctx.has_addend = add is not None
+        ctx.rows_ok = bool(rows_ok)
         if not is_training:
             return native().trilinear_devoxelize_bnact_forward(r, False, pts, x3, w, b, mean, rstd, slope, add)[0]
         taps = CornerTaps.of(coords, r)
@@ -211,15 +227,16 @@
     @amp_bwd
     def backward(ctx, grad_out):
         x3, w, b, mean, rstd, _, _ = ctx.saved_tensors
-        g_act = ctx.taps.backward(_rows(grad_out, grad_out.shape))
-        gx, gw, gb = _bnact_backward(x3, g_act.view(x3.shape), w, b, mean, rstd, ctx.slope, ctx.use_batch_stats, ctx.shape)
-        return (gx, None, gw if w is not None else None, gb if b is not None else None) + (None,) * 10 + (grad_out if ctx.has_addend else None, None)
+        gx, gw, gb = _tail_backward(ctx.taps, _rows(grad_out, grad_out.shape), x3, w, b, mean, rstd, ctx.slope, ctx.use_batch_stats, ctx.shape,
+                                    ctx.rows_ok)
+        return ((gx, None, gw if w is not None else None, gb if b is not None else None) + (None,) * 10
+                + (grad_out if ctx.has_addend else None, None, None))
 
 
 def batch_norm_act_devoxelize(grid, coords, bn, slope, resolution, is_training, stats_part=None, addend=None):
     use_batch_stats, momentum, rm, rv, counter, part, shift = _module_call(bn, stats_part)
     return BatchNormActDevoxelize.apply(grid, coords, bn.weight, bn.bias, rm, rv, use_batch_stats, momentum, bn.eps, slope,
-                                        resolution, is_training, part, shift, addend, counter)
+                                        resolution, is_training, part, shift, addend, counter, not torch.is_autocast_enabled())
 
 
 class BatchNormActDevoxelizePointBN(Function):
@@ -248,8 +265,7 @@
     def backward(ctx, grad_out):
         x3, w, b, mean, rstd, pre3, pw, pb, p_mean, p_rstd, _, _ = ctx.saved_tensors
         g_rows = _rows(grad_out, grad_out.shape)
-        g_act = ctx.taps.backward(g_rows)
-        gx, gw, gb = _bnact_backward(x3, g_act.view(x3.shape), w, b, mean, rstd, ctx.slope, True, ctx.shape)
+        gx, gw, gb = _tail_backward(ctx.taps, g_rows, x3, w, b, mean, rstd, ctx.slope, True, ctx.shape, True)
         gp, gpw, gpb = _bnact_backward(pre3, g_rows, pw, pb, p_mean, p_rstd, ctx.p_slope, True, ctx.p_shape)
         return ((gx, None, gw if w is not None else None, gb if b is not None else None) + (None,) * 9
                 + (gp, gpw if pw is not None else None, gpb if pb is not None else None) + (None,) * 8)
diff --git a/pvcnn_amd/modules/functional/devoxelization.py b/pvcnn_amd/modules/functional/devoxelization.py
--- a/pvcnn_amd/modules/functional/devoxelization.py
+++ b/pvcnn_amd/modules/functional/devoxelization.py
@@ -7,10 +7,10 @@
 
 
 class CornerTaps:
-    __slots__ = ('inds', 'wgts', 'plan', 'r')
+    __slots__ = ('inds', 'wgts', 'plan', 'mask', 'r')
 
     def __init__(self, r):
-        self.inds = self.wgts = self.plan = None
+        self.inds = self.wgts = self.plan = self.mask = None
         self.r = int(r)
 
     @staticmethod
@@ -26,14 +26,28 @@
             outs = run(False)[0]
         return outs
 
-    def backward(self, grad_points):
+    def _planned(self, be, grad_points):
+        if not (getattr(be, 'has_scatter_plans', False) and grad_points.is_cuda):
+            return False
+        if self.plan is None:
+            made = be.trilinear_devoxelize_backward_plan(self.inds, self.wgts, self.r)
+            self.plan = made if made is not None else False
+        return self.plan
+
+    def row_mask(self, grad_points):
         be = native()
-        if getattr(be, 'has_scatter_plans', False) and grad_points.is_cuda:
-            if self.plan is None:
-                made = be.trilinear_devoxelize_backward_plan(self.inds, self.wgts, self.r)
-                self.plan = made if made is not None else False
-            if self.plan is not False:
-                return be.trilinear_devoxelize_backward_apply(grad_points, self.plan, self.r)
+        if not getattr(be, 'has_tail_rows', False) or self.r % 4 != 0 or self._planned(be, grad_points) is False:
+            return None
+        if self.mask is None:
+            self.mask = be.trilinear_devoxelize_backward_row_mask(self.plan, grad_points.shape[0], grad_points.shape[2], self.r)
+        return self.mask
+
+    def backward(self, grad_points, row_mask=None):
+        be = native()
+        if row_mask is not None:
+            return be.trilinear_devoxelize_backward_apply(grad_points, self.plan, self.r, row_mask=row_mask)
+        if self._planned(be, grad_points) is not False:
+            return be.trilinear_devoxelize_backward_apply(grad_points, self.plan, self.r)
         return be.trilinear_devoxelize_backward(grad_points, self.inds, self.wgts, self.r)
 
 
```

After: 2506 point-clouds/s. No clear change (-0.1%).
